# iam28th/fqcomp28

Measured on AMD Instinct MI355X. Metric: encode MB/s (raw FASTQ in), higher is better.
Workload: dtype u8; 1 GPU; BASELINE configs[1]: 1024 MiB synthetic 150 bp reads (uniform ACGT, Phred~N(34,5) clipped [2,41]), -R 256 blocks, tables from the first 128 MiB, inputs resident in HBM; layout=config1, job_blocks=4, blocks_this_gpu=4, records_this_gpu=3202273, bases_this_gpu=480340950

## Files before the change

fqcomp28_amd/binding.py:

```python
import ctypes as C
import os
import subprocess

import numpy as np

HERE = os.path.dirname(os.path.abspath(__file__))
ROOT = os.path.dirname(HERE)
LIB_PATH = os.environ.get("FQGPU_LIB") or os.path.join(HERE, "libfqgpu.so")

SEQ_MODELS, SEQ_ALPHA = 256, 4
QUAL_MODELS, QUAL_ALPHA = 8192, 64
REC_DTYPE = np.dtype([("seq_off", "<u4"), ("qual_off", "<u4"), ("len", "<u4")])
SEQ_FT_DTYPE = np.dtype(
    [("norm", "<i2", (SEQ_MODELS, SEQ_ALPHA)), ("logs", "<u4", (SEQ_MODELS,)), ("max_log", "<u4")]
)
QUAL_FT_DTYPE = np.dtype(
    [("norm", "<i2", (QUAL_MODELS, QUAL_ALPHA)), ("logs", "<u4", (QUAL_MODELS,)), ("max_log", "<u4")]
)
F_WRITE_BACK_N = 1
F_DECODE_INDEX = 2
DEC_FORM_BOTH, DEC_FORM_QUAL_RESIDENT, DEC_FORM_QUAL_COMPACT, DEC_FORM_SEQ = 0x001, 0x002, 0x004, 0x008
DEC_FORM_CHUNKS_QUAL_RESIDENT, DEC_FORM_CHUNKS_QUAL_COMPACT, DEC_FORM_CHUNKS_SEQ, DEC_FORM_SNAP = 0x010, 0x020, 0x040, 0x100

ERRORS = {0: "OK", -1: "OVERFLOW", -2: "SHORT_READ", -3: "CORRUPT", -4: "ARG", -5: "NO_DEVICE",
# ... 16 lines not shown
    return LIB_PATH


def build(verbose=False):
    cmd = ["make", "-C", os.path.join(HERE, "csrc"), "-j", "6"]
    subprocess.run(cmd, check=True, stdout=None if verbose else subprocess.DEVNULL)
    return LIB_PATH


_lib = None

_PROTOS = {
    "fqgpu_device_count": (C.c_int, []),
    "fqgpu_strerror": (C.c_char_p, [C.c_int]),
    "fqgpu_version": (C.c_char_p, []),
    "fqgpu_bound_seq": (C.c_size_t, [C.c_size_t]),
    "fqgpu_bound_qual": (C.c_size_t, [C.c_size_t]),
    "fqgpu_freq_tables": (C.c_int, [C.c_int, C.c_void_p, C.c_size_t, C.c_void_p, C.c_size_t,
                                    C.c_void_p, C.c_void_p, C.c_void_p, C.c_void_p]),
    "fqgpu_tables_from_counts": (C.c_int, [C.c_int, C.c_void_p, C.c_void_p, C.c_void_p, C.c_void_p]),
    "fqgpu_ctx_create": (C.c_int, [C.c_int, C.c_void_p, C.c_void_p, C.POINTER(C.c_void_p)]),
    "fqgpu_ctx_destroy": (None, [C.c_void_p]),
    "fqgpu_ctx_set_chain_params": (C.c_int, [C.c_void_p, C.c_uint, C.c_uint]),
    "fqgpu_ctx_dump_tables": (C.c_int, [C.c_void_p, C.c_int, C.c_uint, C.c_void_p, C.c_size_t,
                                        C.c_void_p, C.c_size_t]),
    "fqgpu_encode_block": (C.c_int, [C.c_void_p, C.c_void_p, C.c_size_t, C.c_void_p, C.c_size_t,
                                     C.c_void_p, C.c_size_t, C.POINTER(C.c_size_t),
                                     C.c_void_p, C.c_size_t, C.POINTER(C.c_size_t),
                                     C.c_void_p, C.c_void_p, C.c_void_p, C.c_size_t,
                                     C.POINTER(C.c_size_t), C.c_uint]),
    "fqgpu_encode_begin": (C.c_int, [C.c_void_p, C.c_void_p, C.c_size_t, C.c_void_p, C.c_size_t, C.c_uint,
                                     C.POINTER(C.c_size_t), C.POINTER(C.c_size_t), C.POINTER(C.c_size_t)]),
    "fqgpu_encode_records": (C.c_int, [C.c_void_p, C.c_void_p, C.c_size_t]),
    "fqgpu_encode_wait": (C.c_int, [C.c_void_p, C.POINTER(C.c_size_t), C.POINTER(C.c_size_t), C.POINTER(C.c_size_t)]),
    "fqgpu_encode_cancel": (C.c_int, [C.c_void_p]),
    "fqgpu_encode_headers_begin": (C.c_int, [C.c_void_p, C.c_void_p, C.c_char_p, C.c_uint, C.c_void_p, C.c_size_t]),
    "fqgpu_encode_headers_wait": (C.c_int, [C.c_void_p, C.c_void_p, C.POINTER(C.c_size_t), C.POINTER(C.c_size_t)]),
    "fqgpu_encode_headers_end": (C.c_int, [C.c_void_p, C.c_void_p, C.c_size_t]),
    "fqgpu_encode_end": (C.c_int, [C.c_void_p, C.c_void_p, C.c_void_p, C.c_size_t, C.POINTER(C.c_size_t),
                                   C.c_void_p, C.c_size_t, C.POINTER(C.c_size_t), C.c_void_p, C.c_void_p, C.c_void_p,
                                   C.c_size_t, C.POINTER(C.c_size_t)]),
    "fqgpu_decode_block": (C.c_int, [C.c_void_p, C.c_void_p, C.c_size_t, C.c_void_p, C.c_size_t,
                                     C.c_void_p, C.c_size_t, C.c_void_p, C.c_size_t, C.c_void_p,
                                     C.c_size_t, C.c_void_p, C.c_size_t]),
    "fqgpu_encode_index": (C.c_int, [C.c_void_p, C.c_int, C.c_void_p, C.c_size_t, C.POINTER(C.c_size_t)]),
    "fqgpu_decode_block_indexed": (C.c_int, [C.c_void_p, C.c_void_p, C.c_size_t, C.c_void_p, C.c_size_t,
                                             C.c_void_p, C.c_size_t, C.c_void_p, C.c_size_t, C.c_void_p,
                                             C.c_size_t, C.c_void_p, C.c_size_t, C.c_void_p, C.c_size_t, C.c_void_p, C.c_size_t]),
    "fqgpu_decode_chunk": (C.c_int, [C.c_void_p, C.c_void_p, C.c_void_p, C.c_size_t, C.c_void_p, C.c_size_t,
                                     C.c_void_p, C.c_size_t, C.c_void_p, C.c_size_t, C.c_void_p, C.c_size_t,
                                     C.c_void_p, C.c_size_t, C.c_void_p, C.c_size_t, C.c_void_p, C.c_size_t,
                                     C.c_void_p, C.POINTER(C.c_size_t), C.POINTER(C.c_size_t)]),
    "fqgpu_decode_chunk_indexing": (C.c_int, [C.c_void_p, C.c_void_p, C.c_void_p, C.c_size_t, C.c_void_p, C.c_size_t,
                                              C.c_void_p, C.c_size_t, C.c_void_p, C.c_size_t, C.c_void_p, C.c_size_t,
                                              C.c_void_p, C.c_size_t, C.c_void_p, C.POINTER(C.c_size_t), C.POINTER(C.c_size_t)]),
    "fqgpu_decode_index": (C.c_int, [C.c_void_p, C.c_int, C.c_void_p, C.c_size_t, C.POINTER(C.c_size_t)]),
    "fqgpu_decode_chunk_range": (C.c_int, [C.c_void_p, C.c_void_p, C.c_void_p, C.c_size_t, C.c_void_p, C.c_size_t,
                                           C.c_void_p, C.c_size_t, C.c_void_p, C.c_size_t, C.c_void_p, C.c_size_t,
                                           C.c_void_p, C.c_size_t, C.c_void_p, C.c_size_t, C.c_size_t, C.c_size_t, C.c_size_t,
                                           C.c_void_p, C.c_size_t, C.POINTER(C.c_size_t), C.c_void_p,
                                           C.POINTER(C.c_size_t)]),
    "fqgpu_decode_chunk_fasta": (C.c_int, [C.c_void_p, C.c_void_p, C.c_void_p, C.c_size_t, C.c_void_p, C.c_size_t,
                                           C.c_void_p, C.c_size_t, C.c_void_p, C.c_size_t, C.c_void_p, C.c_size_t,
                                           C.c_size_t, C.c_size_t, C.c_size_t,
                                           C.c_void_p, C.c_size_t, C.POINTER(C.c_size_t), C.c_void_p,
                                           C.POINTER(C.c_size_t)]),
    "fqgpu_dblock_create": (C.c_int, [C.c_void_p, C.c_void_p, C.c_size_t, C.c_void_p, C.c_size_t,
                                      C.POINTER(C.c_void_p)]),
    "fqgpu_dblock_create_from_raw": (C.c_int, [C.c_void_p, C.c_void_p, C.c_size_t, C.POINTER(C.c_void_p)]),
    "fqgpu_dblock_records": (C.c_int, [C.c_void_p, C.c_void_p, C.c_void_p, C.c_size_t, C.POINTER(C.c_size_t),
                                       C.POINTER(C.c_size_t)]),
    "fqgpu_dblock_destroy": (None, [C.c_void_p]),
    "fqgpu_dblock_encode": (C.c_int, [C.c_void_p, C.c_void_p, C.c_uint]),
    "fqgpu_dblock_wipe": (C.c_int, [C.c_void_p, C.c_void_p]),
    "fqgpu_dblocks_decode": (C.c_int, [C.c_void_p, C.POINTER(C.c_void_p), C.c_size_t]),
    "fqgpu_dblocks_decode_indexing": (C.c_int, [C.c_void_p, C.POINTER(C.c_void_p), C.c_size_t]),
    "fqgpu_sync": (C.c_int, [C.c_void_p]),
    "fqgpu_dblock_status": (C.c_int, [C.c_void_p, C.POINTER(C.c_size_t), C.POINTER(C.c_size_t),
                                      C.POINTER(C.c_size_t), C.POINTER(C.c_size_t)]),
    "fqgpu_dblock_longest_chain": (C.c_int, [C.c_void_p, C.POINTER(C.c_uint), C.POINTER(C.c_uint)]),
    "fqgpu_dblock_qual_segment_classes": (C.c_int, [C.c_void_p, C.c_void_p, C.POINTER(C.c_size_t)]),
    "fqgpu_dblock_qual_segments": (C.c_int, [C.c_void_p, C.c_void_p, C.c_void_p, C.c_void_p, C.c_void_p, C.c_size_t,
                                             C.POINTER(C.c_size_t)]),
    "fqgpu_ctx_set_index_stride": (C.c_int, [C.c_void_p, C.c_uint]),
    "fqgpu_dblock_index_bytes": (C.c_int, [C.c_void_p, C.c_int, C.POINTER(C.c_size_t)]),
    "fqgpu_dblock_fetch_index": (C.c_int, [C.c_void_p, C.c_void_p, C.c_int, C.c_void_p, C.c_size_t]),
    "fqgpu_dblock_load_index": (C.c_int, [C.c_void_p, C.c_void_p, C.c_int, C.c_void_p, C.c_size_t]),
    "fqgpu_ctx_set_lanes": (C.c_int, [C.c_void_p, C.c_uint]),
    "fqgpu_ctx_fill_scratch": (C.c_int, [C.c_void_p, C.c_ubyte, C.POINTER(C.c_size_t), C.POINTER(C.c_size_t)]),
    "fqgpu_ctx_reserve": (C.c_int, [C.c_void_p, C.c_size_t, C.c_size_t, C.c_size_t]),
    "fqgpu_ctx_set_seq_segment": (C.c_int, [C.c_void_p, C.c_uint]),
    "fqgpu_ctx_set_seq_group": (C.c_int, [C.c_void_p, C.c_uint, C.c_uint]),
    "fqgpu_ctx_decode_forms": (C.c_int, [C.c_void_p] + [C.POINTER(C.c_uint)] * 4),
    "fqgpu_ctx_set_seq_handover": (C.c_int, [C.c_void_p, C.c_uint, C.c_uint]),
    "fqgpu_dblock_seq_handover": (C.c_int, [C.c_void_p, C.POINTER(C.c_uint), C.POINTER(C.c_uint)]),
    "fqgpu_dblock_fetch": (C.c_int, [C.c_void_p, C.c_void_p, C.c_void_p, C.c_void_p, C.c_void_p,
                                     C.c_void_p, C.c_void_p, C.c_void_p]),
    "fqgpu_dblock_load_streams": (C.c_int, [C.c_void_p, C.c_void_p, C.c_void_p, C.c_size_t,
                                            C.c_void_p, C.c_size_t, C.c_void_p, C.c_void_p, C.c_size_t]),
    "fqgpu_ctx_enable_timing": (C.c_int, [C.c_void_p, C.c_int]),
    "fqgpu_ctx_last_timing": (C.c_int, [C.c_void_p, C.POINTER(Timing)]),
    "fqgpu_ctx_timing_only": (C.c_int, [C.c_void_p, C.c_char_p]),
    "fqgpu_chunk_crc32": (C.c_int, [C.c_void_p, C.POINTER(C.c_uint32), C.POINTER(C.c_size_t)]),
    "fqgpu_dblock_crc32": (C.c_int, [C.c_void_p, C.c_void_p, C.POINTER(C.c_uint32), C.POINTER(C.c_size_t)]),
    "fqgpu_crc32_combine": (C.c_uint32, [C.c_uint32, C.c_uint32, C.c_uint64]),
    "fqgpu_ctx_set_check_only": (C.c_int, [C.c_void_p, C.c_int]),
    "fqgpu_stats_words": (C.c_size_t, [C.c_uint]),
    "fqgpu_chunk_stats": (C.c_int, [C.c_void_p, C.c_uint, C.c_void_p, C.c_size_t]),
    "fqgpu_dblock_stats": (C.c_int, [C.c_void_p, C.c_void_p, C.c_uint, C.c_void_p, C.c_size_t]),
    "fqgpu_stats_merge": (C.c_int, [C.c_void_p, C.c_size_t, C.c_void_p, C.c_size_t]),
    "fqgpu_filter_check": (C.c_int, [C.c_void_p]),
    "fqgpu_chunk_filter": (C.c_int, [C.c_void_p, C.c_void_p, C.c_void_p, C.c_size_t, C.POINTER(C.c_size_t), C.c_void_p, C.c_void_p]),
    "fqgpu_dblock_filter": (C.c_int, [C.c_void_p, C.c_void_p, C.c_void_p, C.c_void_p, C.c_size_t, C.POINTER(C.c_size_t),
                                      C.c_void_p, C.c_void_p]),
    "fqgpu_trim_check": (C.c_int, [C.c_void_p]),
    "fqgpu_chunk_trim": (C.c_int, [C.c_void_p, C.c_void_p, C.c_void_p, C.c_void_p, C.c_size_t, C.POINTER(C.c_size_t), C.c_void_p,
                                   C.c_void_p, C.c_void_p]),
    "fqgpu_dblock_trim": (C.c_int, [C.c_void_p, C.c_void_p, C.c_void_p, C.c_void_p, C.c_void_p, C.c_size_t, C.POINTER(C.c_size_t),
                                    C.c_void_p, C.c_void_p, C.c_void_p]),
    "fqgpu_adapter_check": (C.c_int, [C.c_void_p]),
    "fqgpu_chunk_clip": (C.c_int, [C.c_void_p, C.c_void_p, C.c_void_p, C.c_void_p, C.c_void_p, C.c_size_t, C.POINTER(C.c_size_t),
                                   C.c_void_p, C.c_void_p, C.c_void_p]),
    "fqgpu_dblock_clip": (C.c_int, [C.c_void_p, C.c_void_p, C.c_void_p, C.c_void_p, C.c_void_p, C.c_void_p, C.c_size_t,
                                    C.POINTER(C.c_size_t), C.c_void_p, C.c_void_p, C.c_void_p]),
    "fqgpu_tail_check": (C.c_int, [C.c_void_p]),
    "fqgpu_chunk_tailtrim": (C.c_int, [C.c_void_p, C.c_void_p, C.c_void_p, C.c_void_p, C.c_void_p, C.c_void_p, C.c_size_t,
                                       C.POINTER(C.c_size_t), C.c_void_p, C.c_void_p, C.c_void_p, C.c_void_p]),
    "fqgpu_dblock_tailtrim": (C.c_int, [C.c_void_p, C.c_void_p, C.c_void_p, C.c_void_p, C.c_void_p, C.c_void_p, C.c_void_p, C.c_size_t,
                                        C.POINTER(C.c_size_t), C.c_void_p, C.c_void_p, C.c_void_p, C.c_void_p]),
    "fqgpu_chunk_select_marked": (C.c_int, [C.c_void_p, C.c_void_p, C.c_void_p, C.c_void_p, C.c_void_p, C.c_size_t, C.c_size_t, C.c_void_p,
                                            C.c_void_p, C.c_size_t, C.POINTER(C.c_size_t), C.c_void_p, C.c_void_p, C.c_void_p, C.c_void_p]),
    "fqgpu_dblock_select_marked": (C.c_int, [C.c_void_p, C.c_void_p, C.c_void_p, C.c_void_p, C.c_void_p, C.c_void_p, C.c_size_t, C.c_size_t,
                                             C.c_void_p, C.c_void_p, C.c_size_t, C.POINTER(C.c_size_t), C.c_void_p, C.c_void_p, C.c_void_p,
                                             C.c_void_p]),
    "fqgpu_chunk_select_limited": (C.c_int, [C.c_void_p, C.c_void_p, C.c_void_p, C.c_void_p, C.c_void_p, C.c_size_t, C.c_size_t, C.c_void_p, C.c_void_p,
                                             C.c_void_p, C.c_size_t, C.POINTER(C.c_size_t), C.c_void_p, C.c_void_p, C.c_void_p, C.c_void_p]),
    "fqgpu_dblock_select_limited": (C.c_int, [C.c_void_p, C.c_void_p, C.c_void_p, C.c_void_p, C.c_void_p, C.c_void_p, C.c_size_t, C.c_size_t,
                                              C.c_void_p, C.c_void_p, C.c_void_p, C.c_size_t, C.POINTER(C.c_size_t), C.c_void_p, C.c_void_p,
                                              C.c_void_p, C.c_void_p]),
    "fqgpu_overlap_check": (C.c_int, [C.c_void_p]),
    "fqgpu_overlap_merge": (C.c_int, [C.c_void_p, C.c_size_t, C.c_void_p, C.c_size_t]),
    "fqgpu_chunk_pair_overlap": (C.c_int, [C.c_void_p, C.c_size_t, C.c_void_p, C.c_size_t, C.c_size_t, C.c_void_p, C.c_void_p, C.c_size_t,
                                           C.c_void_p, C.c_void_p, C.c_void_p]),
    "fqgpu_dblock_pair_overlap": (C.c_int, [C.c_void_p, C.c_void_p, C.c_size_t, C.c_void_p, C.c_size_t, C.c_size_t, C.c_void_p, C.c_void_p,
                                            C.c_size_t, C.c_void_p, C.c_void_p, C.c_void_p]),
    "fqgpu_correct_check": (C.c_int, [C.c_void_p]),
    "fqgpu_chunk_pair_correct": (C.c_int, [C.c_void_p, C.c_size_t, C.c_void_p, C.c_size_t, C.c_size_t, C.c_void_p, C.c_void_p, C.c_void_p,
                                           C.c_void_p, C.c_void_p]),
    "fqgpu_dblock_pair_correct": (C.c_int, [C.c_void_p, C.c_void_p, C.c_size_t, C.c_void_p, C.c_size_t, C.c_size_t, C.c_void_p, C.c_void_p,
                                            C.c_void_p, C.c_void_p, C.c_void_p]),
    "fqgpu_merge_check": (C.c_int, [C.c_void_p]),
    "fqgpu_chunk_pair_merge": (C.c_int, [C.c_void_p, C.c_size_t, C.c_void_p, C.c_size_t, C.c_size_t, C.c_void_p, C.c_void_p, C.c_void_p,
                                         C.c_void_p, C.c_size_t, C.c_void_p, C.c_void_p, C.c_void_p]),
    "fqgpu_dblock_pair_merge": (C.c_int, [C.c_void_p, C.c_void_p, C.c_size_t, C.c_void_p, C.c_size_t, C.c_size_t, C.c_void_p, C.c_void_p,
                                          C.c_void_p, C.c_void_p, C.c_size_t, C.c_void_p, C.c_void_p, C.c_void_p]),
    "fqgpu_chunk_pair_names": (C.c_int, [C.c_void_p, C.c_size_t, C.c_void_p, C.c_size_t, C.c_size_t, C.POINTER(C.c_size_t)]),
    "fqgpu_dblock_pair_names": (C.c_int, [C.c_void_p, C.c_void_p, C.c_size_t, C.c_void_p, C.c_size_t, C.c_size_t, C.POINTER(C.c_size_t)]),
    "fqgpu_read_id_len": (C.c_size_t, [C.c_void_p, C.c_size_t]),
    "fqgpu_probe_words": (C.c_size_t, [C.c_uint, C.c_uint]),
    "fqgpu_probes_check": (C.c_int, [C.c_void_p]),
    "fqgpu_chunk_probe": (C.c_int, [C.c_void_p, C.c_void_p, C.c_uint, C.c_void_p, C.c_size_t, C.c_void_p]),
    "fqgpu_dblock_probe": (C.c_int, [C.c_void_p, C.c_void_p, C.c_void_p, C.c_uint, C.c_void_p, C.c_size_t, C.c_void_p]),
    "fqgpu_probe_merge": (C.c_int, [C.c_void_p, C.c_size_t, C.c_void_p, C.c_size_t]),
    "fqgpu_host_alloc": (C.c_void_p, [C.c_size_t]),
    "fqgpu_host_free": (None, [C.c_void_p]),
    "fqgpu_host_trim": (C.c_size_t, []),
# ... 462 lines not shown
    def wipe(self):
        _check(lib().fqgpu_dblock_wipe(self.ctx.h, self.h), "dblock_wipe")

    def crc32(self, want_len=False):
        crc, n = C.c_uint32(0), C.c_size_t(0)
        _check(lib().fqgpu_dblock_crc32(self.ctx.h, self.h, C.byref(crc), C.byref(n)), "dblock_crc32")
        return (crc.value, n.value) if want_len else crc.value

    def stats(self, positions):
        rc, out = _stats_call(lib().fqgpu_dblock_stats, positions, self.ctx.h, self.h)
        _check(rc, "dblock_stats")
        return out

    def probe(self, probes, positions, want_places=True, **kw):
        return _probe_call(lib().fqgpu_dblock_probe, (self.ctx.h, self.h), probes, positions, self.n_recs, want_places, **kw)

    def filter(self, flt, **kw):
        return _select_call(lib().fqgpu_dblock_filter, (self.ctx.h, self.h), (flt,), self.n_recs, **kw)

    def trim(self, trim, flt=None, **kw):
        return _select_call(lib().fqgpu_dblock_trim, (self.ctx.h, self.h), (trim, flt), self.n_recs, more=("win",), **kw)

    def clip(self, adapter, trim=None, flt=None, **kw):
        return _select_call(lib().fqgpu_dblock_clip, (self.ctx.h, self.h), (adapter, trim, flt), self.n_recs, more=("win",), **kw)

    def tailtrim(self, adapter=None, tail=None, trim=None, flt=None, **kw):
        return _select_call(lib().fqgpu_dblock_tailtrim, (self.ctx.h, self.h), (adapter, tail, trim, flt), self.n_recs, more=("win", "places"),
                            report_words=TAIL_REPORT_WORDS, **kw)

    def select_marked(self, first, end, mark=None, adapter=None, tail=None, trim=None, flt=None, **kw):
        return _range_call(lib().fqgpu_dblock_select_marked, (self.ctx.h, self.h), (adapter, tail, trim, flt), first, end, mark, **kw)

    def select_limited(self, first, end, mark=None, limit=None, adapter=None, tail=None, trim=None, flt=None, **kw):
        return _range_call(lib().fqgpu_dblock_select_limited, (self.ctx.h, self.h), (adapter, tail, trim, flt), first, end, mark, limit, **kw)

    def pair_correct(self, first, other, other_first, count, insert, spec, **kw):
        return _correct_call(lib().fqgpu_dblock_pair_correct, (self.ctx.h, self.h, first, other.h if other is not None else None, other_first),
                             count, insert, spec, **kw)

    def pair_merge(self, first, other, other_first, count, insert, mark, spec, **kw):
        return _merge_call(lib().fqgpu_dblock_pair_merge, (self.ctx.h, self.h, first, other.h if other is not None else None, other_first),
                           count, insert, mark, spec, **kw)

    def pair_overlap(self, first, other, other_first, count, spec, **kw):
        return _overlap_call(lib().fqgpu_dblock_pair_overlap, (self.ctx.h, self.h, first, other.h if other is not None else None, other_first),
                             count, spec, **kw)

    def pair_names(self, first, other, other_first, count):
        m = C.c_size_t(7)
        rc = lib().fqgpu_dblock_pair_names(self.ctx.h, self.h, first, other.h if other is not None else None, other_first, count, C.byref(m))
        return rc, None if m.value == NO_MISMATCH else m.value

    def status(self):
        a, b, c, d = C.c_size_t(), C.c_size_t(), C.c_size_t(), C.c_size_t()
        rc = lib().fqgpu_dblock_status(self.h, C.byref(a), C.byref(b), C.byref(c), C.byref(d))
        return rc, dict(seq_len=a.value, qual_len=b.value, n_pos_len=c.value, n_bases=d.value)

    def longest_chain(self):
        a, b = C.c_uint(), C.c_uint()
        _check(lib().fqgpu_dblock_longest_chain(self.h, C.byref(a), C.byref(b)), "dblock_longest_chain")
        return a.value, b.value

    def seq_handover(self):
        a, b = C.c_uint(), C.c_uint()
        _check(lib().fqgpu_dblock_seq_handover(self.h, C.byref(a), C.byref(b)), "dblock_seq_handover")
        return a.value, b.value

    def qual_segment_classes(self):
        c = (C.c_size_t * 4)()
        _check(lib().fqgpu_dblock_qual_segment_classes(self.ctx.h, self.h, c), "dblock_qual_segment_classes")
        return dict(transparent=c[0], anchored=c[1], uniform=c[2], opaque=c[3])

    def qual_segments(self):
        n = C.c_size_t(0)
        rc = lib().fqgpu_dblock_qual_segments(self.ctx.h, self.h, None, None, None, 0, C.byref(n))
        if rc != -1:
            _check(rc, "dblock_qual_segments")
        cls, anchor, ctx = np.zeros(n.value, dtype=np.uint8), np.zeros(n.value, dtype=np.uint32), np.zeros(n.value, dtype=np.uint32)
        if n.value:
            _check(lib().fqgpu_dblock_qual_segments(self.ctx.h, self.h, _p(cls), _p(anchor), _p(ctx), n.value, C.byref(n)),
                   "dblock_qual_segments")
        return dict(cls=cls, anchor=anchor, ctx=ctx)

    def fetch(self, raw=False):
        rc, st = self.status()
        _check(rc, "dblock_status")
        seq = np.zeros(st["seq_len"], dtype=np.uint8)
        qual = np.zeros(st["qual_len"], dtype=np.uint8)
        rl = np.zeros(self.n_recs, dtype=np.uint16)
        nc = np.zeros(self.n_recs, dtype=np.uint16)
        npos = np.zeros(st["n_pos_len"], dtype=np.uint16)
        rw = np.zeros(self.raw_len, dtype=np.uint8) if raw else None
        _check(lib().fqgpu_dblock_fetch(self.ctx.h, self.h, _p(seq), _p(qual), _p(rl), _p(nc), _p(npos),
                                        _p(rw)), "dblock_fetch")
        return dict(seq=seq, qual=qual, readlens=rl, n_count=nc, n_pos=npos, raw=rw)

    def fetch_raw(self):
        rw = np.zeros(self.raw_len, dtype=np.uint8)
        _check(lib().fqgpu_dblock_fetch(self.ctx.h, self.h, None, None, None, None, None, _p(rw)),
               "dblock_fetch")
        return rw

    def load_streams(self, seq, qual, n_count, n_pos):
        seq = np.ascontiguousarray(seq, dtype=np.uint8)
        qual = np.ascontiguousarray(qual, dtype=np.uint8)
        n_count = np.ascontiguousarray(n_count, dtype=np.uint16)
        n_pos = np.ascontiguousarray(n_pos, dtype=np.uint16)
        _check(lib().fqgpu_dblock_load_streams(self.ctx.h, self.h, _p(seq), seq.size, _p(qual), qual.size,
                                               _p(n_count), _p(n_pos), n_pos.size), "load_streams")


class _HeaderStreams(C.Structure):
    _fields_ = [("field_types", C.c_void_p), ("separators", C.c_char_p), ("n_fields", C.c_uint),
                ("first_header", C.c_void_p), ("first_header_len", C.c_size_t), ("sizes", C.c_void_p),
                ("streams", C.POINTER(C.c_void_p))]


class Context:

    def __init__(self, seq_ft, qual_ft, device=0):
        self.seq_ft = np.ascontiguousarray(seq_ft)
        self.qual_ft = np.ascontiguousarray(qual_ft)
        assert self.seq_ft.nbytes == SEQ_FT_DTYPE.itemsize and self.qual_ft.nbytes == QUAL_FT_DTYPE.itemsize
        h = C.c_void_p()
        _check(lib().fqgpu_ctx_create(device, _p(self.seq_ft), _p(self.qual_ft), C.byref(h)), "ctx_create")
        self.h = h
        self.device = device

    def close(self):
        if getattr(self, "h", None):
            lib().fqgpu_ctx_destroy(self.h)
            self.h = None

    __del__ = close

    def set_chain_params(self, segment=0, seq_generic=False, seq_segment=None, seq_group=None):
        flags = 1 if seq_generic else 0
        if seq_segment is not None:
            _check(lib().fqgpu_ctx_set_seq_segment(self.h, seq_segment), "set_seq_segment")
        if seq_group is not None:
            q, g = seq_group if isinstance(seq_group, tuple) else (seq_group, 0)
            _check(lib().fqgpu_ctx_set_seq_group(self.h, q, g), "set_seq_group")
        _check(lib().fqgpu_ctx_set_chain_params(self.h, segment, flags), "set_chain_params")

    def set_seq_handover(self, cap, prefix_segments=1):
        _check(lib().fqgpu_ctx_set_seq_handover(self.h, cap, prefix_segments), "set_seq_handover")

    def set_index_stride(self, symbols):
        _check(lib().fqgpu_ctx_set_index_stride(self.h, symbols), "set_index_stride")

    def set_lanes(self, lanes):
        _check(lib().fqgpu_ctx_set_lanes(self.h, lanes), "set_lanes")

    def sync(self):
        _check(lib().fqgpu_sync(self.h), "sync")

    def fill_scratch(self, byte):
        n, nb = C.c_size_t(0), C.c_size_t(0)
        _check(lib().fqgpu_ctx_fill_scratch(self.h, byte, C.byref(n), C.byref(nb)), "fill_scratch")
        return n.value, nb.value

    def decode_forms(self):
        f, c, s, n = C.c_uint(0), C.c_uint(0), C.c_uint(0), C.c_uint(0)
        _check(lib().fqgpu_ctx_decode_forms(self.h, C.byref(f), C.byref(c), C.byref(s), C.byref(n)), "decode_forms")
        return dict(forms=f.value, qual_chains=c.value, qual_strides=s.value, n_cus=n.value)

# ... 268 lines not shown
```

fqcomp28_amd/csrc/api.hip:

```cpp
#include "fqgpu_internal.h"

#include <algorithm>
#include <cstdio>
#include <cstdlib>
#include <cstring>
#include <initializer_list>
#include <new>
#include <string>
#include <map>
#include <memory>
#include <mutex>
#include <vector>

__attribute__((constructor)) static void fq_ask_for_hw_queues() {
  if (getenv("FQGPU_KEEP_HW_QUEUES")) return;
  if (const char *have = getenv("GPU_MAX_HW_QUEUES")) {
    char *end = nullptr;
    const long n = strtol(have, &end, 10);
    if (end == have || *end != 0 || n < 1 || n >= 16) return;
  }
  setenv("GPU_MAX_HW_QUEUES", "16", 1);
}

static thread_local char g_hip_msg[256] = "";

int fq_hip_error(hipError_t e, const char *file, int line) {
  snprintf(g_hip_msg, sizeof(g_hip_msg), "HIP error %d (%s) at %s:%d", (int)e, hipGetErrorString(e), file, line);
  if (getenv("FQGPU_VERBOSE")) fprintf(stderr, "fqgpu: %s\n", g_hip_msg);
  return (e == hipErrorOutOfMemory) ? FQGPU_E_NOMEM
         : (e == hipErrorNoDevice || e == hipErrorInvalidDevice) ? FQGPU_E_NO_DEVICE
                                                                 : FQGPU_E_HIP;
}

extern "C" const char *fqgpu_strerror(int code) {
  switch (code) {
  case FQGPU_OK: return "ok";
  case FQGPU_E_OVERFLOW: return "compressed stream exceeds the reference capacity bound";
  case FQGPU_E_SHORT_READ: return "read shorter than 3 bases (undefined in the reference coder)";
  case FQGPU_E_CORRUPT: return "corrupt stream (end mark / leftover bits / N table)";
  case FQGPU_E_ARG: return "bad argument or symbol outside the model alphabet";
  case FQGPU_E_NO_DEVICE: return "no usable MI355X / HIP device (there is no CPU fallback)";
  case FQGPU_E_NOMEM: return "out of device or host memory";
  case FQGPU_E_HIP: return g_hip_msg[0] ? g_hip_msg : "HIP runtime error";
  case FQGPU_E_HEADER: return "read header the field coder cannot code (numeric field not an int32 / string field of 255 or more bytes)";
  default: return "unknown fqgpu error";
  }
}

extern "C" const char *fqgpu_version(void) { return "fqgpu 0.1 (gfx950)"; }

extern "C" int fqgpu_device_count(void) {
  int n = 0;
  if (hipGetDeviceCount(&n) != hipSuccess) return 0;
  return n;
}

extern "C" size_t fqgpu_bound_seq(size_t n) {
  if (n < 1024) return (size_t)1024 * FQGPU_SEQ_MODELS;
  return n / 4 + 1024;
}
extern "C" size_t fqgpu_bound_qual(size_t n) {
  const size_t a = (size_t)1024 * FQGPU_QUAL_MODELS, b = n * 7 / 8 + 1024;
  return a > b ? a : b;
}

static int use_device(int device) {
  int n = 0;
  if (hipGetDeviceCount(&n) != hipSuccess || n <= 0) return FQGPU_E_NO_DEVICE;
  if (device < 0 || device >= n) return FQGPU_E_NO_DEVICE;
  FQ_HIP(hipSetDevice(device));
  return FQGPU_OK;
}

namespace {
struct HostHdr { uint64_t magic, pinned, size, pad[5]; };
constexpr uint64_t HOST_MAGIC = 0x46514850494E4E44ull;
constexpr size_t PIN_MIN = 64 << 10;
struct PinCache {
  std::mutex mutex;
  std::multimap<size_t, void *> blocks;
  size_t bytes = 0;
};
PinCache &pin_cache() {
// ... 262 lines not shown
  return l;
}

static int normalize_to_host(hipStream_t st, const uint32_t *counts_dev, int stream, void *ft_out) {
  const FtLayout l = ft_layout(stream);
  uint8_t *dev = fq_dev_alloc<uint8_t>(l.total + 8);
  if (!dev) return FQGPU_E_NOMEM;
  int rc = FQGPU_OK;
  uint32_t err = 0;
  do {
    if (hipMemsetAsync(dev, 0, l.total + 8, st) != hipSuccess) { rc = FQGPU_E_HIP; break; }
    uint32_t *err_dev = reinterpret_cast<uint32_t *>(dev + ((l.total + 3) & ~(size_t)3));
    rc = fq_normalize_counts(st, counts_dev, l.n_models, l.alpha, reinterpret_cast<int16_t *>(dev),
                             reinterpret_cast<uint32_t *>(dev + l.logs_off),
                             reinterpret_cast<uint32_t *>(dev + l.maxlog_off), err_dev);
    if (rc) break;
    if (hipMemcpyAsync(ft_out, dev, l.total, hipMemcpyDeviceToHost, st) != hipSuccess ||
        hipMemcpyAsync(&err, err_dev, 4, hipMemcpyDeviceToHost, st) != hipSuccess ||
        hipStreamSynchronize(st) != hipSuccess) { rc = FQGPU_E_HIP; break; }
    if (err) rc = FQGPU_E_ARG;
  } while (0);
  (void)hipFree(dev);
  return rc;
}

extern "C" int fqgpu_tables_from_counts(int device, const uint32_t *seq_counts, const uint32_t *qual_counts,
                                        void *seq_ft_out, void *qual_ft_out) {
  int rc = use_device(device);
  if (rc) return rc;
  if (!seq_counts || !qual_counts || !seq_ft_out || !qual_ft_out) return FQGPU_E_ARG;
  const size_t ns = (size_t)FQGPU_SEQ_MODELS * FQGPU_SEQ_ALPHA, nq = (size_t)FQGPU_QUAL_MODELS * FQGPU_QUAL_ALPHA;
  uint32_t *dev = fq_dev_alloc<uint32_t>(ns + nq);
  if (!dev) return FQGPU_E_NOMEM;
  hipStream_t st = nullptr;
  if (hipMemcpy(dev, seq_counts, ns * 4, hipMemcpyHostToDevice) != hipSuccess ||
      hipMemcpy(dev + ns, qual_counts, nq * 4, hipMemcpyHostToDevice) != hipSuccess) rc = FQGPU_E_HIP;
  if (!rc) rc = normalize_to_host(st, dev, 0, seq_ft_out);
  if (!rc) rc = normalize_to_host(st, dev + ns, 1, qual_ft_out);
  (void)hipFree(dev);
  return rc;
}

extern "C" int fqgpu_freq_tables(int device, const uint8_t *raw, size_t raw_len, const fqgpu_rec *recs,
                                 size_t n_recs, void *seq_ft_out, void *qual_ft_out,
                                 uint32_t *seq_counts_out, uint32_t *qual_counts_out) {
  int rc = use_device(device);
  if (rc) return rc;
  if (!raw || !recs || !seq_ft_out || !qual_ft_out) return FQGPU_E_ARG;
  size_t n_bases = 0;
  unsigned min_len = 0xFFFFFFFFu;
  for (size_t i = 0; i < n_recs; i++) {
    if ((size_t)recs[i].seq_off + recs[i].len > raw_len || (size_t)recs[i].qual_off + recs[i].len > raw_len)
      return FQGPU_E_ARG;
    n_bases += recs[i].len;
    if (recs[i].len < min_len || recs[i].len > 65535u) min_len = recs[i].len > 65535u ? 0u : recs[i].len;
  }
  const size_t ns = (size_t)FQGPU_SEQ_MODELS * FQGPU_SEQ_ALPHA, nq = (size_t)FQGPU_QUAL_MODELS * FQGPU_QUAL_ALPHA;
  uint8_t *raw_dev = fq_dev_alloc<uint8_t>(raw_len + 64);
  fqgpu_rec *recs_dev = fq_dev_alloc<fqgpu_rec>(n_recs + 1);
  uint32_t *cnt = fq_dev_alloc<uint32_t>(ns + nq + 1);
  hipStream_t st = nullptr;
  uint32_t err = 0;
  if (!raw_dev || !recs_dev || !cnt) rc = FQGPU_E_NOMEM;
  do {
    if (rc) break;
    if (hipMemcpy(raw_dev, raw, raw_len, hipMemcpyHostToDevice) != hipSuccess ||
        hipMemcpy(recs_dev, recs, n_recs * sizeof(fqgpu_rec), hipMemcpyHostToDevice) != hipSuccess ||
        hipMemset(cnt + ns + nq, 0, 4) != hipSuccess) { rc = FQGPU_E_HIP; break; }
    if ((rc = fq_build_freq_tables(device, st, raw_dev, recs_dev, n_recs, cnt, cnt + ns, n_bases, min_len))) break;
    if (hipMemcpy(&err, cnt + ns + nq, 4, hipMemcpyDeviceToHost) != hipSuccess) { rc = FQGPU_E_HIP; break; }
    if (err) { rc = FQGPU_E_ARG; break; }
    if (seq_counts_out && hipMemcpy(seq_counts_out, cnt, ns * 4, hipMemcpyDeviceToHost) != hipSuccess) { rc = FQGPU_E_HIP; break; }
    if (qual_counts_out && hipMemcpy(qual_counts_out, cnt + ns, nq * 4, hipMemcpyDeviceToHost) != hipSuccess) { rc = FQGPU_E_HIP; break; }
    if ((rc = normalize_to_host(st, cnt, 0, seq_ft_out))) break;
    if ((rc = normalize_to_host(st, cnt + ns, 1, qual_ft_out))) break;
  } while (0);
  if (raw_dev) (void)hipFree(raw_dev);
  if (recs_dev) (void)hipFree(recs_dev);
  if (cnt) (void)hipFree(cnt);
  return rc;
}

static void free_tables(DevTables &t) {
  void *ps[] = {t.norm, t.logs, t.log_prefix, t.ct, t.ct_off, t.dt, t.dt_off, t.next1, t.next2, t.reset_mask,
                t.seq_pow[0], t.seq_pow[1], t.seq_pow[2], t.seq_pow[3]};
  for (void *p : ps) if (p) (void)hipFree(p);
  t = DevTables();
}

static int upload_tables(fqgpu_ctx *ctx, int stream, const void *ft) {
  const FtLayout l = ft_layout(stream);
  DevTables &t = ctx->tab[stream];
  const uint8_t *p = static_cast<const uint8_t *>(ft);
  const uint32_t *logs = reinterpret_cast<const uint32_t *>(p + l.logs_off);
  const int16_t *norm = reinterpret_cast<const int16_t *>(p);
  uint32_t max_log = 0;
  for (int i = 0; i < l.n_models; i++) {
    if (logs[i] < 5 || logs[i] > 12) return FQGPU_E_ARG;
    if (logs[i] > max_log) max_log = logs[i];
    uint32_t sum = 0;
    for (int s = 0; s < l.alpha; s++) {
      const int n = norm[(size_t)i * l.alpha + s];
      if (n < -1) return FQGPU_E_ARG;
      sum += n == -1 ? 1u : (uint32_t)n;
    }
    if (sum != (1u << logs[i])) return FQGPU_E_ARG;
  }
  t.max_log = max_log;
  t.norm = fq_dev_alloc<int16_t>((size_t)l.n_models * l.alpha);
  t.logs = fq_dev_alloc<uint32_t>(l.n_models);
  uint32_t *err_dev = fq_dev_alloc<uint32_t>(1);
  if (!t.norm || !t.logs || !err_dev) return FQGPU_E_NOMEM;
  FQ_HIP(hipMemcpyAsync(t.norm, p, l.norm_bytes, hipMemcpyHostToDevice, ctx->stream));
  FQ_HIP(hipMemcpyAsync(t.logs, logs, (size_t)l.n_models * 4, hipMemcpyHostToDevice, ctx->stream));
  FQ_HIP(hipMemsetAsync(err_dev, 0, 4, ctx->stream));
  int rc = fq_build_tables(ctx->stream, t, l.n_models, l.alpha, err_dev);
  uint32_t err = 0;
  if (!rc) {
    FQ_HIP(hipMemcpyAsync(&err, err_dev, 4, hipMemcpyDeviceToHost, ctx->stream));
    FQ_HIP(hipStreamSynchronize(ctx->stream));
    if (err) rc = FQGPU_E_ARG;
  }
  (void)hipFree(err_dev);
  return rc;
}

extern "C" int fqgpu_ctx_create(int device, const void *seq_ft, const void *qual_ft, fqgpu_ctx **out) {
  if (!out) return FQGPU_E_ARG;
  *out = nullptr;
  int rc = use_device(device);
  if (rc) return rc;
  if (!seq_ft || !qual_ft) return FQGPU_E_ARG;
  fqgpu_ctx *ctx = new (std::nothrow) fqgpu_ctx();
  if (!ctx) return FQGPU_E_NOMEM;
  ctx->device = device;
  {
    int cus = 0;
    if (hipDeviceGetAttribute(&cus, hipDeviceAttributeMultiprocessorCount, device) == hipSuccess && cus > 0) ctx->n_cus = (unsigned)cus;
  }
  if (hipStreamCreateWithFlags(&ctx->stream, hipStreamNonBlocking) != hipSuccess) {
    delete ctx;
    return FQGPU_E_HIP;
  }
  rc = fq_probe_lds_atomic_order(ctx->stream, &ctx->lds_atomics_ordered);
  if (!rc) rc = fq_encode_init_device();
  if (getenv("FQGPU_NO_LDS_ATOMIC_RANK")) ctx->lds_atomics_ordered = false;
  if (getenv("FQGPU_SLOT_PARTITION")) ctx->tile_sorted = false;
  if (const char *e = getenv("FQGPU_SETFUNC_WGS")) ctx->setfunc_wgs = (unsigned)atoi(e);
  if (const char *e = getenv("FQGPU_SEQ_GROUP")) ctx->seq_group = (unsigned)atoi(e);
  if (const char *e = getenv("FQGPU_SEQ_GROUP_MIN")) ctx->seq_group_min = (unsigned)atoi(e);
  if (const char *e = getenv("FQGPU_SEQ_CAND_CAP")) ctx->seq_cand_cap = std::min((unsigned)atoi(e), 64u);
  if (const char *e = getenv("FQGPU_SEQ_CAND_PREFIX")) ctx->seq_cand_prefix = std::max((unsigned)atoi(e), 1u);
  if (!rc) rc = upload_tables(ctx, 0, seq_ft);
  if (!rc) rc = upload_tables(ctx, 1, qual_ft);
  if (rc) { fqgpu_ctx_destroy(ctx); return rc; }
  *out = ctx;
  return FQGPU_OK;
}

#ifdef FQGPU_EXPERIMENTS
void fq_ts_prof_dump();
#endif

extern "C" void fqgpu_ctx_destroy(fqgpu_ctx *ctx) {
  if (!ctx) return;
  (void)hipSetDevice(ctx->device);
  (void)fqgpu_sync(ctx);
// ... 293 lines not shown
  return rc;
}

extern "C" int fqgpu_dblock_longest_chain(const fqgpu_dblock *b, unsigned *seq_segments, unsigned *qual_segments) {
  if (!b) return FQGPU_E_ARG;
  (void)hipSetDevice(b->device);
  BlockResult tmp;
  FQ_HIP(hipMemcpy(&tmp, b->result, sizeof(tmp), hipMemcpyDeviceToHost));
  if (seq_segments) *seq_segments = tmp.s[0].refixed;
  if (qual_segments) *qual_segments = tmp.s[1].refixed;
  return FQGPU_OK;
}

extern "C" int fqgpu_dblock_seq_handover(const fqgpu_dblock *b, unsigned *handed_over, unsigned *kept) {
  if (!b) return FQGPU_E_ARG;
  (void)hipSetDevice(b->device);
  if (b->last_op && !b->result_pulled && b->owner) {
    const int rc = fqgpu_sync(b->owner);
    if (rc) return rc;
  }
  BlockResult tmp;
  FQ_HIP(hipMemcpy(&tmp, b->result, sizeof(tmp), hipMemcpyDeviceToHost));
  if (handed_over) *handed_over = tmp.seq_groups_handed;
  if (kept) *kept = tmp.seq_groups_kept;
  return FQGPU_OK;
}

extern "C" int fqgpu_ctx_decode_forms(const fqgpu_ctx *ctx, unsigned *forms, unsigned *qual_chains, unsigned *qual_strides, unsigned *n_cus) {
  if (!ctx) return FQGPU_E_ARG;
  if (forms) *forms = ctx->dec_forms;
  if (qual_chains) *qual_chains = ctx->dec_qual_chains;
  if (qual_strides) *qual_strides = ctx->dec_qual_strides;
  if (n_cus) *n_cus = ctx->n_cus;
  return FQGPU_OK;
}

static int diag_lane(fqgpu_ctx *ctx, const fqgpu_dblock *b, const EncLane **lane_out, uint32_t *n_out) {
  if (int rc = fqgpu_sync(ctx)) return rc;
  if (b->owner != ctx || !b->diag_stamp || b->home_lane < 0 || b->home_lane >= FQ_MAX_LANES) return FQGPU_E_ARG;
  const EncLane &lane = ctx->lanes[b->home_lane];
  if (lane.diag_stamp != b->diag_stamp || !lane.diag_cls || !lane.diag_anchor || !lane.diag_n_segs) return FQGPU_E_ARG;
  FQ_HIP(hipMemcpy(n_out, lane.diag_n_segs, 4, hipMemcpyDeviceToHost));
  *lane_out = &lane;
  return FQGPU_OK;
}

extern "C" int fqgpu_dblock_qual_segment_classes(fqgpu_ctx *ctx, const fqgpu_dblock *b, size_t counts[4]) {
  if (!ctx || !b || !counts) return FQGPU_E_ARG;
  counts[0] = counts[1] = counts[2] = counts[3] = 0;
  const EncLane *lane = nullptr;
  uint32_t n = 0;
  if (int rc = diag_lane(ctx, b, &lane, &n)) return rc;
  if (!n) return FQGPU_OK;
  uint8_t *cls = static_cast<uint8_t *>(malloc(n));
  if (!cls) return FQGPU_E_NOMEM;
  const hipError_t he = hipMemcpy(cls, lane->diag_cls, n, hipMemcpyDeviceToHost);
  if (he == hipSuccess)
    for (uint32_t i = 0; i < n; i++) counts[cls[i] == 1 ? 0 : cls[i] == 0xFF ? 2 : cls[i] == 0 ? 3 : 1]++;
  free(cls);
  return he == hipSuccess ? FQGPU_OK : fq_hip_error(he, __FILE__, __LINE__);
}

extern "C" int fqgpu_dblock_qual_segments(fqgpu_ctx *ctx, const fqgpu_dblock *b, uint8_t *cls_out, uint32_t *anchor_out,
                                          uint32_t *ctx_out, size_t cap, size_t *n_out) {
  if (!ctx || !b || !n_out || (cap && (!cls_out || !anchor_out || !ctx_out))) return FQGPU_E_ARG;
  *n_out = 0;
  const EncLane *lane = nullptr;
  uint32_t n = 0;
  if (int rc = diag_lane(ctx, b, &lane, &n)) return rc;
  *n_out = n;
  if (n > cap) return FQGPU_E_OVERFLOW;
  if (!n) return FQGPU_OK;
  constexpr unsigned B = FQGPU_QUAL_MODELS;
  uint32_t *seg_base = static_cast<uint32_t *>(malloc((size_t)(B + 1) * 4));
  if (!seg_base) return FQGPU_E_NOMEM;
  hipError_t he = hipMemcpy(seg_base, lane->diag_n_segs - B, (size_t)(B + 1) * 4, hipMemcpyDeviceToHost);
  if (he == hipSuccess) he = hipMemcpy(cls_out, lane->diag_cls, n, hipMemcpyDeviceToHost);
  if (he == hipSuccess) he = hipMemcpy(anchor_out, lane->diag_anchor, (size_t)n * 4, hipMemcpyDeviceToHost);
  if (he == hipSuccess)
    for (unsigned c = 0; c < B; c++)
      for (uint32_t s = seg_base[c]; s < seg_base[c + 1] && s < n; s++) ctx_out[s] = c;
  free(seg_base);
  return he == hipSuccess ? FQGPU_OK : fq_hip_error(he, __FILE__, __LINE__);
}

extern "C" int fqgpu_dblock_fetch(fqgpu_ctx *ctx, const fqgpu_dblock *b, uint8_t *seq_out, uint8_t *qual_out,
                                  uint16_t *readlens_out, uint16_t *n_count_out, uint16_t *n_pos_out,
                                  uint8_t *raw_out) {
  if (!ctx || !b) return FQGPU_E_ARG;
  int rc = fqgpu_sync(ctx);
  if (rc) return rc;
  if (b->last_op && !b->result_pulled && (rc = pull_result(const_cast<fqgpu_dblock *>(b), b->last_op == 1))) return rc;
  if (seq_out && b->seq_len) FQ_HIP(hipMemcpy(seq_out, b->seq, b->seq_len, hipMemcpyDeviceToHost));
  if (qual_out && b->qual_len) FQ_HIP(hipMemcpy(qual_out, b->qual, b->qual_len, hipMemcpyDeviceToHost));
  if (readlens_out) FQ_HIP(hipMemcpy(readlens_out, b->readlens, b->n_recs * 2, hipMemcpyDeviceToHost));
  if (n_count_out) FQ_HIP(hipMemcpy(n_count_out, b->n_count, b->n_recs * 2, hipMemcpyDeviceToHost));
  if (n_pos_out && b->n_pos_len) FQ_HIP(hipMemcpy(n_pos_out, b->n_pos, b->n_pos_len * 2, hipMemcpyDeviceToHost));
  if (raw_out) FQ_HIP(hipMemcpy(raw_out, b->raw, b->raw_len, hipMemcpyDeviceToHost));
  return FQGPU_OK;
}

extern "C" int fqgpu_dblock_load_streams(fqgpu_ctx *ctx, fqgpu_dblock *b, const uint8_t *seq, size_t seq_len,
                                         const uint8_t *qual, size_t qual_len, const uint16_t *n_count,
                                         const uint16_t *n_pos, size_t n_pos_len) {
  if (!ctx || !b || !seq || !qual || !n_count || (!n_pos && n_pos_len)) return FQGPU_E_ARG;
  int rc = fqgpu_sync(ctx);
  if (rc) return rc;
  if (b->seq.grow(seq_len + 64) || b->qual.grow(qual_len + 64) || b->n_pos.grow(n_pos_len + 16)) return FQGPU_E_NOMEM;
  if (n_pos_len > b->n_pos_cap) b->n_pos_cap = n_pos_len;
  FQ_HIP(hipMemset(b->seq + seq_len, 0, 16));
  FQ_HIP(hipMemset(b->qual + qual_len, 0, 16));
  FQ_HIP(hipMemcpy(b->seq, seq, seq_len, hipMemcpyHostToDevice));
  FQ_HIP(hipMemcpy(b->qual, qual, qual_len, hipMemcpyHostToDevice));
  FQ_HIP(hipMemcpy(b->n_count, n_count, b->n_recs * 2, hipMemcpyHostToDevice));
  if (n_pos_len) FQ_HIP(hipMemcpy(b->n_pos, n_pos, n_pos_len * 2, hipMemcpyHostToDevice));
  b->seq_len = seq_len; b->qual_len = qual_len; b->n_pos_len = n_pos_len;
  b->drop_results();
  return FQGPU_OK;
}

static int dblocks_decode(fqgpu_ctx *ctx, fqgpu_dblock *const *blocks, size_t n_blocks, bool build_index) {
  if (!ctx || (!blocks && n_blocks)) return FQGPU_E_ARG;
  int rc = use_device(ctx->device);
  if (rc) return rc;
  for (size_t i = 0; i < n_blocks; i++)
    if (!blocks[i] || blocks[i]->device != ctx->device) return FQGPU_E_ARG;
  bool synced = false;
  for (size_t i = 0; i < n_blocks; i++) {
    fqgpu_dblock *b = blocks[i];
    if (b->last_op == 1 && !b->result_pulled) {
      if (!synced && (rc = fqgpu_sync(ctx))) return rc;
      synced = true;
      if ((rc = pull_result(b, true))) return rc;
    }
    if (!b->seq_len || !b->qual_len) return FQGPU_E_ARG;
  }
  for (size_t i = 0; i < n_blocks; i++) blocks[i]->launched(2);
  return fq_decode_launch(ctx, blocks, n_blocks, nullptr, build_index);
}

extern "C" int fqgpu_dblocks_decode(fqgpu_ctx *ctx, fqgpu_dblock *const *blocks, size_t n_blocks) {
  return dblocks_decode(ctx, blocks, n_blocks, false);
}

extern "C" int fqgpu_dblocks_decode_indexing(fqgpu_ctx *ctx, fqgpu_dblock *const *blocks, size_t n_blocks) {
  int rc = dblocks_decode(ctx, blocks, n_blocks, true);
  if (rc) {
    for (size_t i = 0; blocks && i < n_blocks; i++)
      if (blocks[i]) blocks[i]->index_bytes[0] = blocks[i]->index_bytes[1] = 0;
    return rc;
  }
  if ((rc = fqgpu_sync(ctx))) return rc;
  for (size_t i = 0; i < n_blocks; i++) {
    const int brc = pull_result(blocks[i], false);
    if (brc) blocks[i]->index_bytes[0] = blocks[i]->index_bytes[1] = 0;
    if (brc && brc != FQGPU_E_CORRUPT && brc != FQGPU_E_ARG) return brc;
  }
  return FQGPU_OK;
}

template <class A> static bool hp_room(A &a, size_t need) { return a.grow(need, need / 8) == FQGPU_OK; }

static int hp_block_acquire(fqgpu_ctx *ctx, size_t raw_len, size_t n_recs, size_t n_bases, size_t seq_cap,
                            size_t qual_cap, size_t n_pos_cap, fqgpu_dblock **out) {
  if (!ctx->hp.block && !(ctx->hp.block = dblock_new(ctx).release())) return FQGPU_E_NOMEM;
  fqgpu_dblock *b = ctx->hp.block;
// ... 885 lines not shown
```

fqcomp28_amd/csrc/enc_chains_generic.h:

```cpp

constexpr unsigned SEG_NONE = 0xFFFFFFFFu;
constexpr unsigned SEG_CLS_OPAQUE = 0, SEG_CLS_UNIFORM = 0xFF;

struct SegArrays {
  uint32_t *anchor;
  uint32_t *usym;
  uint16_t *entry_state;
  uint16_t *cand_exit;
  uint8_t *cls;
};

template <class M>
__device__ __forceinline__ unsigned seg_ctx_of(const uint32_t *__restrict__ base, unsigned v) {
  unsigned lo = 0, hi = M::B - 1;
  while (lo < hi) {
    const unsigned mid = lo + ((hi - lo + 1) >> 1);
    if (base[mid] <= v) lo = mid; else hi = mid - 1;
  }
  return lo;
}

template <class M>
__global__ void __launch_bounds__(256)
k_seg_scan(const uint8_t *__restrict__ sorted_sym, const uint32_t *__restrict__ arrays,
// ... 78 lines not shown
__device__ __forceinline__ bool seg_wants_setfunc(const SegArrays &sa, unsigned seg, unsigned k, unsigned nseg) {
  if (k + 1 >= nseg) return false;
  const unsigned cls = sa.cls[seg];
  return cls == SEG_CLS_OPAQUE || (seg_is_cand(cls) && !seg_entry_known(k, k ? (unsigned)sa.cls[seg - 1] : 1u));
}

template <class M, unsigned PER0>
__device__ __forceinline__ void seg_pow_table(uint32_t *lds, const uint32_t *__restrict__ tbl, unsigned s, unsigned S,
                                              uint16_t *__restrict__ f) {
  const unsigned log = tbl[0] & 0xFFFFu, size = 1u << log, lane = fq_lane(), per = max(size >> 6, 1u);
  const uint16_t *st = reinterpret_cast<const uint16_t *>(tbl) + 2;
  const uint32_t *tt = tbl + 1 + (size >> 1);
  const int dfs = (int)tt[2 * s];
  const unsigned dnb = tt[2 * s + 1];
  uint16_t *base = reinterpret_cast<uint16_t *>(lds);
  unsigned acc[PER0], tmp[PER0];
#pragma unroll
  for (unsigned j = 0; j < PER0; j++) {
    const unsigned i = (lane + 64u * j) & (size - 1);
    acc[j] = i;
    if (j < per) {
      const unsigned x = size + i, nb = (x + dnb) >> 16;
      base[i] = (uint16_t)(st[(int)(x >> nb) + dfs] - size);
    }
  }
  fq_lds_wave_sync();
  for (unsigned e = S; e; e >>= 1) {
    if (e & 1u) {
#pragma unroll
      for (unsigned j = 0; j < PER0; j++)
        if (j < per) acc[j] = base[acc[j]];
    }
    if (e > 1u) {
#pragma unroll
      for (unsigned j = 0; j < PER0; j++)
        if (j < per) tmp[j] = base[base[(lane + 64u * j) & (size - 1)]];
      fq_lds_wave_sync();
#pragma unroll
      for (unsigned j = 0; j < PER0; j++)
        if (j < per) base[(lane + 64u * j) & (size - 1)] = (uint16_t)tmp[j];
      fq_lds_wave_sync();
    }
  }
#pragma unroll
  for (unsigned j = 0; j < PER0; j++) {
    const unsigned i = lane + 64u * j;
    if (j < per && i < size) f[i] = (uint16_t)(size + acc[j]);
  }
}

template <class M>
__device__ __forceinline__ unsigned seg_walk_range(const LdsCTable &t, const uint8_t *__restrict__ sym,
                                                   uint16_t *__restrict__ out, unsigned i, unsigned end, unsigned x) {
  while (i < end && (i & 15u)) {
    out[i] = (uint16_t)chain_step(t, x, sym[i] & (unsigned)(M::A - 1));
    i++;
  }
  if (i + 16 <= end) {
    const uint4 *sym16 = reinterpret_cast<const uint4 *>(sym);
    uint4 *out16v = reinterpret_cast<uint4 *>(out);
    uint4 cur = sym16[i >> 4];
    while (i + 16 <= end) {
      const uint4 nxt = i + 32 <= end ? sym16[(i >> 4) + 1] : cur;
      const unsigned w[4] = {cur.x, cur.y, cur.z, cur.w};
      unsigned o[8];
#pragma unroll
      for (int j = 0; j < 16; j++) {
        const unsigned v = chain_step(t, x, (w[j >> 2] >> (8 * (j & 3))) & (unsigned)(M::A - 1));
        if (j & 1) o[j >> 1] |= v << 16; else o[j >> 1] = v;
      }
      out16v[i >> 3] = make_uint4(o[0], o[1], o[2], o[3]);
      out16v[(i >> 3) + 1] = make_uint4(o[4], o[5], o[6], o[7]);
      i += 16;
      cur = nxt;
    }
  }
  while (i < end) {
    out[i] = (uint16_t)chain_step(t, x, sym[i] & (unsigned)(M::A - 1));
    i++;
  }
  return x;
}

template <class M, int PASS>
__device__ __forceinline__ void seg_walk_role(uint32_t *lds, unsigned item, const uint8_t *__restrict__ sorted_sym,
                                              uint16_t *__restrict__ out16, const uint32_t *__restrict__ arrays,
                                              const uint32_t *__restrict__ ct, const uint32_t *__restrict__ ct_off,
                                              uint16_t *__restrict__ final_state, unsigned S, const SegArrays &sa, StreamResult *res) {
  constexpr unsigned B = M::B;
  const uint32_t *ctx_count = arrays, *ctx_start = arrays + B, *seg_base = ctx_start + B + 1,
                 *item_base = seg_base + B + 1;
  if (item >= item_base[B]) return;
  const unsigned c = seg_ctx_of<M>(item_base, item);
  const unsigned n = ctx_count[c];
  const unsigned nseg = seg_base[c + 1] - seg_base[c];
  const unsigned k = (item - item_base[c]) * 64 + fq_lane();
  const LdsCTable t = stage_ctable<M>(lds, ct + ct_off[c]);
  if (k >= nseg) return;
  const unsigned seg = seg_base[c] + k;
  const uint8_t *sym = sorted_sym + ctx_start[c];
  uint16_t *out = out16 + ctx_start[c];
  const unsigned begin = k * S, end = min(n, begin + S);
  const bool reset = sa.cls[seg] == 1;
  const unsigned fr = sa.anchor[seg];
  unsigned x, i0, i1;
  if (PASS == 1) {
    if (!reset) return;
    i0 = begin + fr + 1; i1 = end;
    x = reset_state(t, sym[begin + fr] & (unsigned)(M::A - 1));
  } else {
    i0 = begin; i1 = reset ? begin + fr + 1 : end;
    x = sa.entry_state[seg];
  }
  x = seg_walk_range<M>(t, sym, out, i0, i1, x);
  if (PASS == 1 && k + 1 < nseg) sa.entry_state[seg + 1] = (uint16_t)x;
  if (k == nseg - 1 && (PASS == 1 || !reset)) final_state[c] = (uint16_t)x;
  if (PASS == 2 && fq_lane() == 0) atomicMax(&res->refixed, min(S, n));
}

template <class M, int PASS>
__global__ void __launch_bounds__(64)
k_seg_walk(const uint8_t *__restrict__ sorted_sym, uint16_t *__restrict__ out16,
           const uint32_t *__restrict__ arrays, const uint32_t *__restrict__ ct,
           const uint32_t *__restrict__ ct_off, uint16_t *__restrict__ final_state, unsigned S,
           SegArrays sa, StreamResult *res) {
  extern __shared__ uint32_t lds[];
  seg_walk_role<M, PASS>(lds, blockIdx.x, sorted_sym, out16, arrays, ct, ct_off, final_state, S, sa, res);
}

template <class M>
__device__ __forceinline__ unsigned seg_state_range(const LdsCTable &t, const uint8_t *__restrict__ sym, unsigned i,
                                                    unsigned end, unsigned x) {
  auto step = [&](unsigned s) {
    const int dfs = (int)t.tt[2 * s];
    const unsigned nb = (x + t.tt[2 * s + 1]) >> 16;
    x = t.state_table[(int)(x >> nb) + dfs];
  };
  while (i < end && (i & 15u)) { step(sym[i] & (unsigned)(M::A - 1)); i++; }
  if (i + 16 <= end) {
    const uint4 *sym16 = reinterpret_cast<const uint4 *>(sym);
    uint4 cur = sym16[i >> 4];
    while (i + 16 <= end) {
      const uint4 nxt = i + 32 <= end ? sym16[(i >> 4) + 1] : cur;
      const unsigned w[4] = {cur.x, cur.y, cur.z, cur.w};
#pragma unroll
      for (int j = 0; j < 16; j++) step((w[j >> 2] >> (8 * (j & 3))) & (unsigned)(M::A - 1));
      i += 16;
      cur = nxt;
    }
  }
  while (i < end) { step(sym[i] & (unsigned)(M::A - 1)); i++; }
  return x;
}

template <class M, bool HEADS>
__device__ __forceinline__ void seg_cand_role(uint32_t *lds, unsigned w_first, unsigned w_step, const uint8_t *__restrict__ sorted_sym,
                                              const uint32_t *__restrict__ arrays, const uint32_t *__restrict__ ct,
                                              const uint32_t *__restrict__ ct_off, unsigned S, unsigned fstride, const SegArrays &sa,
                                              uint16_t *__restrict__ fbuf) {
  constexpr unsigned B = M::B, PER = 64 / SEG_SLOT;
  const uint32_t *ctx_count = arrays, *ctx_start = arrays + B, *seg_base = ctx_start + B + 1;
  const unsigned n_segs = seg_base[B];
  const unsigned lane = fq_lane(), slot = lane / SEG_SLOT, j = lane % SEG_SLOT;
  for (unsigned w = w_first; w * PER < n_segs; w += w_step) {
    const unsigned seg = w * PER + slot;
    unsigned cls = 0, c = 0, k = 0, pred = 1;
    bool want = false;
    if (seg < n_segs) {
      cls = sa.cls[seg];
      if (seg_is_cand(cls)) {
        c = seg_ctx_of<M>(seg_base, seg);
        k = seg - seg_base[c];
        pred = k ? (unsigned)sa.cls[seg - 1] : 1u;
        want = k + 1 < seg_base[c + 1] - seg_base[c] && (!HEADS || seg_entry_known(k, pred));
      }
    }
    unsigned long long todo = __ballot(want);
    while (todo) {
      const unsigned cc = (unsigned)__shfl((int)c, __ffsll((long long)todo) - 1);
      const bool mine = want && c == cc;
      todo &= ~__ballot(mine);
      fq_lds_wave_sync();
      const LdsCTable t = stage_ctable<M>(lds, ct + ct_off[cc]);
      if (!mine) continue;
      const unsigned size = 1u << t.log;
      const unsigned n = ctx_count[c], begin = k * S, end = min(n, begin + S);
      const uint8_t *sym = sorted_sym + ctx_start[c];
      const unsigned r = begin + sa.anchor[seg];
      const unsigned s = sym[r] & (unsigned)(M::A - 1);
      const int dfs = (int)t.tt[2 * s];
      const unsigned n_cand = HEADS ? pred : cls;
      for (unsigned cand = j; cand < n_cand; cand += SEG_SLOT) {
        if (!HEADS) {
          unsigned x = t.state_table[dfs + (int)cls + (int)cand];
          x = seg_state_range<M>(t, sym, r + 1, end, x);
          sa.cand_exit[(size_t)seg * SEG_MAX_CAND + cand] = (uint16_t)x;
        } else {
          const unsigned entry = pred == 1 ? (unsigned)sa.entry_state[seg] : (unsigned)sa.cand_exit[(size_t)(seg - 1) * SEG_MAX_CAND + cand];
          const unsigned x = seg_state_range<M>(t, sym, begin, r, entry);
          const unsigned nb = (x + t.tt[2 * s + 1]) >> 16;
          const unsigned u = (x >> nb) - cls;
          fbuf[(size_t)seg * fstride + (entry - size)] = sa.cand_exit[(size_t)seg * SEG_MAX_CAND + u];
        }
      }
    }
  }
}

template <class M>
__global__ void __launch_bounds__(64)
// ... 61 lines not shown
  const LdsCTable t = stage_ctable<M>(lds, ct + ct_off[c]);
  const unsigned log = t.log, size = 1u << log, lane = fq_lane();
  const unsigned per = max(size >> 6, 1u), nw = max(size >> 5, 1u);
  const uint4 *gseg = reinterpret_cast<const uint4 *>(sorted_sym + ctx_start[c] + (size_t)k * S);
  const unsigned nblk = S / SETS_BLOCK, w_end = S / 4;

  unsigned x0[PER0];
#pragma unroll
  for (unsigned j = 0; j < PER0; j++) x0[j] = size + ((lane + 64u * j) & (size - 1));
  unsigned level = 0, n = size, n1 = 0;
  unsigned w = 0, stop = 1;
  uint4 cur = gseg[lane];
  for (unsigned blk = 0; blk < nblk; blk++) {
    const uint4 nxt = blk + 1 < nblk ? gseg[(size_t)(blk + 1) * 64 + lane] : cur;
    const unsigned wb_end = (blk + 1) * (SETS_BLOCK / 4);
    while (w < wb_end) {
      const unsigned w1 = min(stop, wb_end);
      if (level == 0) {
        for (; w < w1; w++) {
          const unsigned word = sets_word(cur, w);
#pragma unroll
          for (int i = 0; i < 4; i++) {
            const unsigned s = (word >> (8 * i)) & (unsigned)(M::A - 1);
            const int dfs = (int)t.tt[2 * s];
            const unsigned dnb = t.tt[2 * s + 1];
#pragma unroll
            for (unsigned j = 0; j < PER0; j++)
              if (j < per) { const unsigned nb = (x0[j] + dnb) >> 16; x0[j] = t.state_table[(int)(x0[j] >> nb) + dfs]; }
          }
        }
      } else {
        switch ((n + 63) / 64) {
          case 1: seg_sets_walk<M, 1>(L, n, t, cur, w, w1); break;
          case 2: seg_sets_walk<M, 2>(L, n, t, cur, w, w1); break;
          case 3: seg_sets_walk<M, 3>(L, n, t, cur, w, w1); break;
          case 4: seg_sets_walk<M, 4>(L, n, t, cur, w, w1); break;
          case 5: seg_sets_walk<M, 5>(L, n, t, cur, w, w1); break;
          case 6: seg_sets_walk<M, 6>(L, n, t, cur, w, w1); break;
          case 7: seg_sets_walk<M, 7>(L, n, t, cur, w, w1); break;
          default: seg_sets_walk<M, 8>(L, n, t, cur, w, w1); break;
        }
        w = w1;
      }
      if (w != stop || w >= w_end) continue;
      stop = stop == 1 ? 4 : stop == 4 ? 12 : stop == 12 ? 32 : stop * 4;
      if (level == 0) {
        sets_clear(L);
#pragma unroll
        for (unsigned j = 0; j < PER0; j++)
          if (j < per) { const unsigned xi = x0[j] - size; atomicOr(&L.bm[xi >> 5], 1u << (xi & 31u)); }
        fq_lds_wave_sync();
        const unsigned nn = sets_count(L, nw);
        if (nn <= SETS_MAX_CLASSES) {
#pragma unroll
          for (unsigned j = 0; j < PER0; j++)
            if (j < per) {
              const unsigned r = sets_rank(L, x0[j] - size);
              L.list[r] = (uint16_t)x0[j];
              x0[j] = r;
            }
          for (unsigned i = lane; i < nn; i += 64) L.m[i] = (uint16_t)i;
          fq_lds_wave_sync();
          level = 1; n = n1 = nn;
        }
      } else if (n > 64) {
        n = sets_merge<false>(L, n, n1, nw, size);
      }
    }
    cur = nxt;
  }
  uint16_t *f = fbuf + (size_t)seg * fstride;
#pragma unroll
  for (unsigned j = 0; j < PER0; j++) {
    const unsigned xi = lane + 64u * j;
    if (j < per && xi < size) f[xi] = level == 0 ? (uint16_t)x0[j] : L.list[L.m[x0[j]]];
  }
}

template <class M, unsigned PER0>
__global__ void __launch_bounds__(64)
k_seg_stage1(const uint8_t *__restrict__ sorted_sym, uint16_t *__restrict__ out16, const uint32_t *__restrict__ arrays,
             const uint32_t *__restrict__ ct, const uint32_t *__restrict__ ct_off, uint16_t *__restrict__ final_state,
             unsigned S, unsigned n_walk, unsigned n_cand, unsigned pbase, unsigned fstride, SegArrays sa,
             uint16_t *__restrict__ fbuf, StreamResult *res) {
  extern __shared__ uint32_t lds[];
  __shared__ SetsWaveLds L;
  if (blockIdx.x < n_walk)
    seg_walk_role<M, 1>(lds, blockIdx.x, sorted_sym, out16, arrays, ct, ct_off, final_state, S, sa, res);
  else if (blockIdx.x < n_walk + n_cand)
    seg_cand_role<M, false>(lds, blockIdx.x - n_walk, n_cand, sorted_sym, arrays, ct, ct_off, S, fstride, sa, fbuf);
  else
    seg_setfunc_role<M, PER0>(lds, L, blockIdx.x - n_walk - n_cand, sorted_sym, arrays, ct, ct_off, S, pbase, fstride, sa, fbuf);
}

struct ItemArrays {
  uint16_t *g;
  uint32_t *has_g;
  uint16_t *item_entry;
};

template <class M, unsigned PER0>
__global__ void __launch_bounds__(64)
k_seg_compose(const uint32_t *__restrict__ arrays, const uint32_t *__restrict__ logs,
              const uint16_t *__restrict__ fbuf, unsigned pbase, unsigned fstride, SegArrays sa, ItemArrays ia) {
  constexpr unsigned B = M::B;
  const uint32_t *seg_base = arrays + B + (B + 1), *item_base = seg_base + B + 1;
  const unsigned item = blockIdx.x, lane = fq_lane();
  if (item >= item_base[B]) return;
  const unsigned c = seg_ctx_of<M>(item_base, item);
  const unsigned nseg = seg_base[c + 1] - seg_base[c];
  const unsigned k0 = (item - item_base[c]) * 64, n_here = min(64u, nseg - k0);
  const unsigned seg0 = seg_base[c] + k0;
  const unsigned slot = lane < n_here ? seg_fslot(sa, seg0 + lane, k0 + lane, nseg, c, pbase) : SEG_NONE;
  const unsigned long long opaque = __ballot(slot != SEG_NONE);
  if (lane == 0) ia.has_g[item] = opaque != 0ull;
  if (!opaque) return;
  const unsigned exit_state = lane < n_here && slot == SEG_NONE && k0 + lane + 1 < nseg ? sa.entry_state[seg0 + lane + 1] : 0u;
  const unsigned size = 1u << logs[c], per = max(size >> 6, 1u);
  unsigned x[PER0];
#pragma unroll
  for (unsigned j = 0; j < PER0; j++) x[j] = size + ((lane + 64u * j) & (size - 1));
  for (unsigned t = 0; t < n_here; t++) {
    const unsigned sl = (unsigned)__shfl((int)slot, (int)t);
    if (sl == SEG_NONE) {
      if (k0 + t + 1 >= nseg) break;
      const unsigned e = (unsigned)__shfl((int)exit_state, (int)t);
#pragma unroll
      for (unsigned j = 0; j < PER0; j++) x[j] = e;
    } else {
      const uint16_t *f = fbuf + (size_t)sl * fstride;
#pragma unroll
      for (unsigned j = 0; j < PER0; j++)
        if (j < per) x[j] = size | ((unsigned)f[x[j] - size] & (size - 1));
    }
  }
  uint16_t *g = ia.g + (size_t)item * fstride;
#pragma unroll
  for (unsigned j = 0; j < PER0; j++) {
    const unsigned xi = lane + 64u * j;
    if (j < per && xi < size) g[xi] = (uint16_t)x[j];
  }
}

template <class M>
__global__ void __launch_bounds__(256)
k_seg_resolve2(const uint32_t *__restrict__ arrays, const uint32_t *__restrict__ logs, unsigned fstride,
               SegArrays sa, ItemArrays ia) {
  constexpr unsigned B = M::B;
  const unsigned c = blockIdx.x * blockDim.x + threadIdx.x;
  if (c >= B) return;
  const uint32_t *seg_base = arrays + B + (B + 1), *item_base = seg_base + B + 1;
  const unsigned i0 = item_base[c], ni = item_base[c + 1] - i0;
  const unsigned size = 1u << logs[c];
  unsigned x = size;
  for (unsigned i = 0; i < ni; i++) {
    ia.item_entry[i0 + i] = (uint16_t)x;
    if (i + 1 == ni) break;
    x = ia.has_g[i0 + i] ? ia.g[(size_t)(i0 + i) * fstride + (x - size)]
                         : sa.entry_state[seg_base[c] + (i + 1) * 64];
  }
}

template <class M>
__global__ void __launch_bounds__(256)
k_seg_resolve3(const uint32_t *__restrict__ arrays, const uint32_t *__restrict__ logs,
               const uint16_t *__restrict__ fbuf, unsigned pbase, unsigned fstride, SegArrays sa, ItemArrays ia) {
  constexpr unsigned B = M::B;
  const uint32_t *seg_base = arrays + B + (B + 1), *item_base = seg_base + B + 1;
  const unsigned item = blockIdx.x * blockDim.x + threadIdx.x;
  if (item >= item_base[B] || !ia.has_g[item]) return;
  const unsigned c = seg_ctx_of<M>(item_base, item);
// ... 14 lines not shown
```

fqcomp28_amd/csrc/enc_plan.h:

```cpp
#pragma once

#include <stddef.h>
#include <stdint.h>

#include <algorithm>

#include "../../include/fqgpu.h"

constexpr unsigned TILE_SEQ = 32768;
constexpr unsigned TILE_QUAL = 65536;
constexpr unsigned TS_TILE = 32768;
constexpr unsigned GROUP_TILES = 64;
constexpr unsigned PACK_TILE = 4096;
constexpr unsigned CTX_PAD = 16;
constexpr unsigned SC_BATCH_SEQ = 8192;
constexpr unsigned SETS_WAVES = 8;
constexpr unsigned SETS_WAVES2 = 16;
constexpr unsigned SETS_ROUNDS = 4;
constexpr unsigned SETS_MAX_GROUP = 16;
constexpr unsigned SETS_BLOCK = 1024;
constexpr unsigned SEQ_CAND_MAX = 64;
constexpr unsigned SEGPLAN_WORDS = 5 * (FQGPU_SEQ_MODELS + 1) + 4;
constexpr unsigned SEQ_ITEM_GROUPS = 64;
constexpr unsigned SEG_MAX_CAND = 64;
constexpr unsigned SEG_SLOT = 16;

struct EncSpan {
  size_t off = 0, bytes = 0;
};
struct EncCarve {
  size_t total = 0;
  EncSpan take(size_t bytes, size_t align = 1) {
    EncSpan s;
    s.off = (total + align - 1) & ~(align - 1);
    s.bytes = bytes;
    total = s.off + bytes;
    return s;
  }
};

struct EncBytes {
  size_t slot_of = 0;
  size_t keys = 0;
  size_t sorted_sym = 0;
  size_t out16 = 0;
  size_t tile_hist = 0;
  size_t tile_base = 0;
  size_t group_sum = 0;
  size_t ctx_arrays = 0;
  size_t seg_state = 0;
  size_t seg_arrays = 0;
  size_t seq_plan = 0;
  size_t seq_fbuf = 0;
  size_t seq_cbuf = 0;
  size_t seq_cand = 0;
  size_t seq_bdesc = 0;
  size_t tile_bits = 0;
  size_t tile_bit_base = 0;
  size_t tile_runs = 0;
  size_t tile_sync = 0;
};

struct EncShape {
  unsigned n_sym = 0, R = 0, B = 0, T = 0;
  unsigned n_tiles = 0, n_groups = 0, n_ptiles = 0;
  size_t n_pad = 0;
  size_t padded = 0;
  size_t lpos16_bytes = 0, tile_runs_bytes = 0;
  EncBytes bytes;
  EncSpan ckey, csym;
  EncSpan ctx_count, ctx_start, seg_base;

  EncShape() = default;
  EncShape(unsigned n_sym_, unsigned R_, unsigned B_, unsigned T_) : n_sym(n_sym_), R(R_), B(B_), T(T_) {
    n_tiles = (n_sym + T - 1) / T;
    n_groups = (n_tiles + GROUP_TILES - 1) / GROUP_TILES;
    n_ptiles = (n_sym + PACK_TILE - 1) / PACK_TILE;
    n_pad = ((size_t)n_sym + SC_BATCH_SEQ + 15) & ~(size_t)15;
    padded = (size_t)n_sym + (size_t)CTX_PAD * B + 64;
    lpos16_bytes = n_pad * 2;
    tile_runs_bytes = (size_t)n_tiles * std::min(B, TS_TILE) * 8;
    EncCarve k, a;
    ckey = k.take(n_pad * 2);
    csym = k.take(n_pad);
    bytes.keys = k.total;
    bytes.sorted_sym = padded;
    bytes.tile_hist = bytes.tile_base = (size_t)n_tiles * B * 4;
    bytes.group_sum = (size_t)n_groups * B * 4;
    ctx_count = a.take((size_t)B * 4);
    ctx_start = a.take((size_t)(B + 1) * 4);
    seg_base = a.take((size_t)(B + 1) * 4);
    a.take((size_t)(B + 1) * 4);
    bytes.ctx_arrays = a.total;
  }
};

struct EncPlanIn {
  unsigned n_sym = 0, R = 0;
  int stream = 0;
  unsigned B = 0, A = 0, max_log = 0;
  bool two_sym = false;
  bool tile_path = false, serial_seq = false;
  unsigned seg_len = 0, seq_segment = 0, seq_group = 0, seq_group_min = 0, seq_cand_cap = 0, seq_cand_prefix = 0, n_cus = 0;
};

struct EncPlan : EncShape {
  bool tile_path = false, serial_seq = false, two_sym = false;
  unsigned max_log = 0;
  unsigned S = 0;
  unsigned seq_S = 0;
  unsigned max_items = 0, gen_max_segs = 0, seq_max_segs = 0;
  unsigned fstride = 0;
  unsigned next_stride = 0;
  unsigned gen_pbase = 0;
  unsigned cand_grid = 0;
  unsigned cand_cap = 0, cand_W = 0, cand_P = 0;
  unsigned wpg = 0, Q = 0, gmin = 0, rounds = 0;
  unsigned max_fitems = 0, max_eitems = 0, max_citems = 0;
  unsigned lds_ct = 0;

  EncSpan sa_anchor, sa_usym, sa_entry, sa_cand, sa_cls;
  EncSpan ia_has_g, ia_entry, ia_g;
  EncSpan sp_fitem, sp_seg, sp_work, sp_entry;
  EncSpan cb_func, cb_item_entry;
  EncSpan cand0, cand;
  EncSpan bd_start, bd_pre;
  EncSpan ts_status, ts_counter, ts_run_count, ts_edges;

  EncPlan() = default;
  explicit EncPlan(const EncPlanIn &in)
      : EncShape(in.n_sym, in.R, in.B, in.tile_path ? TS_TILE : in.stream == 0 ? TILE_SEQ : TILE_QUAL),
        tile_path(in.tile_path), serial_seq(in.serial_seq), two_sym(in.two_sym), max_log(in.max_log) {
    const auto whole_blocks = [](unsigned s) { return (unsigned)std::min(((size_t)s + SETS_BLOCK - 1) / SETS_BLOCK * SETS_BLOCK, (size_t)1 << 30); };
    S = whole_blocks(in.seg_len ? in.seg_len : n_sym >= (24u << 20) ? 4096u : n_sym >= (4u << 20) ? 2048u : 1024u);
    seq_S = whole_blocks(in.seq_segment ? in.seq_segment : n_sym >= (48u << 20) ? 4096u : n_sym >= (4u << 20) ? 2048u : 1024u);
    max_items = (unsigned)((size_t)n_sym / ((size_t)S * 64) + B + 1);
    gen_max_segs = n_sym / S + B + 1;
    seq_max_segs = n_sym / seq_S + B + 1;
    fstride = 1u << max_log;
    next_stride = 4u << max_log;
    gen_pbase = gen_max_segs;
    cand_grid = std::min(gen_max_segs / (64 / SEG_SLOT) + 1, 32u * in.n_cus);
    cand_cap = serial_seq && two_sym ? std::min(in.seq_cand_cap, SEQ_CAND_MAX) : 0u;
    cand_W = cand_cap == 0 ? 0u : cand_cap <= 16 ? 16u : cand_cap <= 32 ? 32u : 64u;
    cand_P = std::min(std::max(in.seq_cand_prefix, 1u), SETS_MAX_GROUP);
    wpg = two_sym ? SETS_WAVES2 : SETS_WAVES;
    Q = std::min(std::max(in.seq_group, 1u), SETS_MAX_GROUP);
    gmin = std::max(in.seq_group_min, 1u);
    rounds = std::max(SETS_ROUNDS / Q, 1u);
    max_fitems = seq_max_segs / (wpg * rounds) + B + 1;
    max_eitems = seq_max_segs / 64 + B + 1;
    max_citems = seq_max_segs / SEQ_ITEM_GROUPS + B + 1;
    lds_ct = (1u + (1u << (max_log - 1)) + 2u * in.A) * 4u;

    bytes.slot_of = tile_path ? lpos16_bytes : n_pad * 4;
    bytes.out16 = padded * 2;
    bytes.seg_state = (size_t)B * 2 + (size_t)B * 8;
    bytes.tile_bits = (size_t)n_ptiles * 4;
    bytes.tile_bit_base = (size_t)(n_ptiles + 1) * 8;

    const size_t gs = gen_max_segs;
    EncCarve g;
    sa_anchor = g.take(gs * 4, 16);
    sa_usym = g.take((size_t)B * 4, 16);
    sa_entry = g.take(gs * 2, 16);
    sa_cand = g.take(gs * SEG_MAX_CAND * 2, 16);
    sa_cls = g.take(gs, 16);
    ia_has_g = g.take((size_t)max_items * 4, 16);
    ia_entry = g.take((size_t)max_items * 2, 16);
    ia_g = g.take((size_t)max_items * fstride * 2, 16);
    g.take(64);
    EncCarve sp, cb, cd, bd, ts;
    const size_t base_bytes = (size_t)(FQGPU_SEQ_MODELS + 1) * 4;
    sp_fitem = sp.take(2 * base_bytes);
    sp_seg = sp.take(3 * base_bytes);
    sp_work = sp.take(16);
    sp_entry = sp.take((size_t)seq_max_segs * 2);
    sp.take(64);
    cb_func = cb.take((size_t)max_citems * fstride * 2);
    cb_item_entry = cb.take((size_t)max_citems * 2);
    cb.take(64);
    cand0 = cd.take((size_t)seq_max_segs * cand_W * 2);
    cand = cd.take((size_t)seq_max_segs * cand_W * 2);
    cd.take(64);
    bd_start = bd.take((size_t)(n_ptiles + 1) * FQGPU_SEQ_MODELS * 4);
    bd_pre = bd.take((size_t)(n_ptiles + 1) * FQGPU_SEQ_MODELS * 2);
    bd.take(64);
    ts_status = ts.take((size_t)n_tiles * 8);
    ts_counter = ts.take(16);
    ts_run_count = ts.take((size_t)n_tiles * 4);
    ts_edges = ts.take((size_t)n_tiles * 16, 16);
    if (serial_seq) {
      bytes.seq_plan = sp.total;
      bytes.seq_fbuf = (size_t)seq_max_segs * fstride * 2 + 64;
      bytes.seq_cand = cand_W ? cd.total : 0;
      bytes.seq_cbuf = cb.total;
      bytes.seq_bdesc = bd.total;
    } else {
      bytes.seg_arrays = g.total;
      bytes.seq_fbuf = ((size_t)gen_max_segs + B) * fstride * 2 + 64;
    }
    if (tile_path) {
      bytes.tile_runs = tile_runs_bytes;
      bytes.tile_sync = ts.total;
    }
  }
};

struct EncLanePlan {
  size_t rec_start = 0;
  size_t n_cnt32 = 0;
  size_t n_off = 0;
  size_t first_sym = 0;
  size_t tile_first = 0;
  size_t scan_tmp = 0;
  EncSpan n_cnt, lens;
  EncSpan first_sym_of[2];

  EncLanePlan(unsigned R, size_t n_bases) {
    EncCarve c, f;
    rec_start = n_off = (size_t)(R + 1) * 4;
    n_cnt = c.take((size_t)R * 4);
    lens = c.take((size_t)R * 4);
    n_cnt32 = c.total;
    first_sym_of[0] = f.take(R);
    first_sym_of[1] = f.take(R);
    f.take(16);
    first_sym = f.total;
    tile_first = (n_bases + TS_TILE - 1) / TS_TILE * 4;
    scan_tmp = ((size_t)R / 1024 + 64) * 16;
  }
};
```

fqcomp28_amd/csrc/enc_records_hist.h:

```cpp


struct __attribute__((packed)) FqBytes16 { uint32_t w[4]; };
__global__ void __launch_bounds__(256)
k_readlens_ncount(const uint8_t *__restrict__ raw, const fqgpu_rec *__restrict__ recs, unsigned R,
                  uint16_t *__restrict__ readlens, uint16_t *__restrict__ n_count,
                  uint32_t *__restrict__ n_cnt32, uint32_t *__restrict__ lens32, BlockResult *res) {
  if (res != nullptr && blockIdx.x == 0 && threadIdx.x < sizeof(BlockResult) / 4) reinterpret_cast<uint32_t *>(res)[threadIdx.x] = 0u;
  const unsigned waves = (gridDim.x * blockDim.x) >> 6;
  const unsigned lane = fq_lane(), sub = lane >> 4, l = lane & 15u;
  for (unsigned r0 = ((blockIdx.x * blockDim.x + threadIdx.x) >> 6) * 4; r0 < R; r0 += waves * 4) {
    const unsigned r = r0 + sub;
    const bool on = r < R;
    const fqgpu_rec rec = recs[on ? r : R - 1];
    const unsigned len = on ? rec.len : 0u;
    const uint8_t *s = raw + rec.seq_off;
    unsigned cnt = 0;
    for (unsigned off = l * 16; off < len; off += 256) {
      const FqBytes16 v = *reinterpret_cast<const FqBytes16 *>(s + off);
      const unsigned live = min(16u, len - off);
#pragma unroll
      for (unsigned i = 0; i < 16; i++)
        cnt += (i < live && ((v.w[i >> 2] >> (8 * (i & 3))) & 0xFFu) == 'N') ? 1u : 0u;
    }
#pragma unroll
// ... 448 lines not shown
        }
        if (n & 1u) {
          const unsigned o = n & 2u;
          ckey_seq[e_first + o] = (uint8_t)(o ? kb >> 16 : kb);
          ckey_qual[e_first + o] = (uint16_t)(o ? cq23 : cq01);
        }
        if (cut) {
#pragma unroll
          for (unsigned i = 0; i < 4; i++)
            if ((valid >> i) & 1u) {
              ckey_seq[e_first + i] = (uint8_t)k16[i];
              ckey_qual[e_first + i] = (uint16_t)cq[i];
            }
        }
#pragma unroll
        for (unsigned i = 0; i < 4; i++) {
          const unsigned one = (valid >> i) & 1u;
          atomicAdd(&hist_s[k16[i] & 0xFFu], one);
          atomicAdd(&hist_q[cq[i] >> 1], one << (16u * (cq[i] & 1u)));
        }
      };
#pragma unroll
      for (int d = 0; d < K1Q_DEPTH - 1; d++)
        if ((unsigned)d < nch) fetch(d, (unsigned)d);
      unsigned c = 0;
      for (; c + 2u * (K1Q_DEPTH - 1) < nch; c += K1Q_DEPTH) {
#pragma unroll
        for (int d = 0; d < K1Q_DEPTH; d++) {
          fetch((d + K1Q_DEPTH - 1) % K1Q_DEPTH, c + d + (K1Q_DEPTH - 1));
          consume(d);
        }
      }
      for (; c < nch; c += K1Q_DEPTH) {
#pragma unroll
        for (int d = 0; d < K1Q_DEPTH; d++) {
          const unsigned cur = c + d;
          if (cur < nch) {
            if (cur + (K1Q_DEPTH - 1) < nch) fetch((d + K1Q_DEPTH - 1) % K1Q_DEPTH, cur + (K1Q_DEPTH - 1));
            consume(d);
          }
        }
      }
      if (covered >= we || r0 + 64u >= R) break;
      r0 += 64u;
    }
  }
  if (bad_s) atomicOr(&res->s[0].bad_symbol, 1u);
  if (bad_q) atomicOr(&res->s[1].bad_symbol, 1u);
  __syncthreads();
  for (unsigned c = threadIdx.x; c < BS; c += blockDim.x) tile_hist_seq[(size_t)tile * BS + c] = (uint16_t)hist_s[c];
  uint32_t *rowq = reinterpret_cast<uint32_t *>(tile_hist_qual + (size_t)tile * BQ);
  for (unsigned c = threadIdx.x; c < BQ / 2; c += blockDim.x) rowq[c] = hist_q[c];
}

template <class HT>
__global__ void __launch_bounds__(256)
k_group_sum(const HT *__restrict__ tile_hist, unsigned n_tiles, unsigned B,
            uint32_t *__restrict__ group_sum) {
  const unsigned c = blockIdx.x * blockDim.x + threadIdx.x;
  const unsigned g = blockIdx.y;
  if (c >= B) return;
  const unsigned t0 = g * GROUP_TILES, t1 = min(t0 + GROUP_TILES, n_tiles);
  uint32_t acc = 0;
  for (unsigned t = t0; t < t1; t++) acc += tile_hist[(size_t)t * B + c];
  group_sum[(size_t)g * B + c] = acc;
}

__global__ void __launch_bounds__(256)
k_group_prefix(uint32_t *__restrict__ group_sum, unsigned n_groups, unsigned B, uint32_t *__restrict__ ctx_count) {
  const unsigned c = blockIdx.x * blockDim.x + threadIdx.x;
  if (c >= B) return;
  uint32_t acc = 0;
  for (unsigned g0 = 0; g0 < n_groups; g0 += 8) {
    uint32_t v[8];
#pragma unroll
    for (unsigned k = 0; k < 8; k++) v[k] = g0 + k < n_groups ? group_sum[(size_t)(g0 + k) * B + c] : 0u;
#pragma unroll
    for (unsigned k = 0; k < 8; k++)
      if (g0 + k < n_groups) { group_sum[(size_t)(g0 + k) * B + c] = acc; acc += v[k]; }
  }
  ctx_count[c] = acc;
}

__global__ void __launch_bounds__(1024)
k_ctx_layout(unsigned B, unsigned S, uint32_t *__restrict__ arrays, uint32_t *__restrict__ fill_none) {
  if (fill_none)
    for (unsigned c = threadIdx.x; c < B; c += blockDim.x) fill_none[c] = 0xFFFFFFFFu;
  __shared__ unsigned part[3][1024];
  uint32_t *ctx_count = arrays, *ctx_start = arrays + B, *seg_base = ctx_start + B + 1,
           *item_base = seg_base + B + 1;
  const unsigned per = (B + blockDim.x - 1) / blockDim.x;
  const unsigned c0 = threadIdx.x * per, c1 = min(c0 + per, B);
  unsigned a0 = 0, a1 = 0, a2 = 0;
  for (unsigned c = c0; c < c1; c++) {
    const unsigned n = ctx_count[c];
    const unsigned nseg = (n + S - 1) / S;
    a0 += (n + CTX_PAD - 1) & ~(CTX_PAD - 1);
    a1 += nseg;
    a2 += (nseg + 63) >> 6;
  }
  part[0][threadIdx.x] = a0; part[1][threadIdx.x] = a1; part[2][threadIdx.x] = a2;
  __syncthreads();
  if (threadIdx.x < 3) {
    unsigned run = 0;
    for (unsigned i = 0; i < blockDim.x; i++) {
      const unsigned v = part[threadIdx.x][i];
      part[threadIdx.x][i] = run;
      run += v;
    }
  }
  __syncthreads();
  a0 = part[0][threadIdx.x]; a1 = part[1][threadIdx.x]; a2 = part[2][threadIdx.x];
  for (unsigned c = c0; c < c1; c++) {
    const unsigned n = ctx_count[c];
    const unsigned nseg = (n + S - 1) / S;
    ctx_start[c] = a0; seg_base[c] = a1; item_base[c] = a2;
    a0 += (n + CTX_PAD - 1) & ~(CTX_PAD - 1);
    a1 += nseg;
    a2 += (nseg + 63) >> 6;
  }
  if (c1 == B && c0 < B) { ctx_start[B] = a0; seg_base[B] = a1; item_base[B] = a2; }
}

template <class HT>
__global__ void __launch_bounds__(256)
k_tile_base(const HT *__restrict__ tile_hist, const uint32_t *__restrict__ group_sum,
            const uint32_t *__restrict__ ctx_start, unsigned n_tiles, unsigned B,
            uint32_t *__restrict__ tile_base) {
  const unsigned c = blockIdx.x * blockDim.x + threadIdx.x;
  const unsigned g = blockIdx.y;
  if (c >= B) return;
  const unsigned t0 = g * GROUP_TILES, t1 = min(t0 + GROUP_TILES, n_tiles);
  uint32_t acc = ctx_start[c] + group_sum[(size_t)g * B + c];
  for (unsigned t = t0; t < t1; t++) {
    tile_base[(size_t)t * B + c] = acc;
    acc += tile_hist[(size_t)t * B + c];
  }
}
```

fqcomp28_amd/csrc/encode.hip:

```cpp
#include "fqgpu_internal.h"
#include "enc_plan.h"

#include <cstdio>
#include <cstdlib>
#include <cstring>
#include <type_traits>

#ifdef FQGPU_EXPERIMENTS
__device__ unsigned long long g_ts_prof[48];
void fq_ts_prof_dump() {
  unsigned long long h[48];
  if (hipMemcpyFromSymbol(h, HIP_SYMBOL(g_ts_prof), sizeof(h)) != hipSuccess) return;
  const char *names[4] = {"partition<Qual>", "partition<Seq>", "gather_pack<Qual>", "gather_pack<Seq>"};
  for (int k = 0; k < 4; k++)
    fprintf(stderr, "ts_prof %-18s phase ticks (100 MHz, summed over workgroups): %llu %llu %llu %llu | ranker alone %llu | K3: store wait %llu patch %llu run map %llu\n",
            names[k], h[8 * k], h[8 * k + 1], h[8 * k + 2], h[8 * k + 3], h[8 * k + 4], h[8 * k + 5], h[8 * k + 6], h[8 * k + 7]);
  for (int k = 0; k < 2; k++)
    fprintf(stderr, "ts_prof %-18s loader thread 64, ticks summed over workgroups: wait for the requested batch (taken in front of finish) %llu | finish %llu | deposit %llu | request %llu | barrier %llu\n",
            names[k], h[32 + 8 * k], h[33 + 8 * k], h[34 + 8 * k], h[35 + 8 * k], h[36 + 8 * k]);
}
#endif

namespace {

// ... 43 lines not shown
  return ctx->lds_atomics_ordered && ctx->tile_sorted && !ctx->seq_generic && !fq_debug_skip() && !fq_debug_k1();
}
static bool dbg_no_alias() {
  static const bool on = fq_debug_flag("FQGPU_DEBUG_NO_ALIAS");
  return on;
}

struct EncStage {
  fqgpu_ctx *ctx;
  hipStream_t st;
  bool off;
  EncStage(fqgpu_ctx *c, hipStream_t s, const char *span, unsigned mask = 0, unsigned bit = 0, const char *skipk = nullptr)
      : ctx(c), st(s), off((mask & bit) != 0 || (skipk && fq_debug_skipk(skipk))) { fq_timer_span_begin(ctx, span, st); }
  ~EncStage() { fq_timer_span_end(ctx, st); }
  EncStage(const EncStage &) = delete;
};
#define FQ_SPAN(x) (M::STREAM ? "qual." x : "seq." x)

template <class M>
EncPlan make_plan(const fqgpu_ctx *ctx, const fqgpu_dblock *b) {
  const DevTables &tab = ctx->tab[M::STREAM];
  EncPlanIn in;
  in.n_sym = (unsigned)b->n_bases;
  in.R = (unsigned)b->n_recs;
  in.stream = M::STREAM; in.B = M::B; in.A = M::A;
  in.max_log = tab.max_log;
  in.two_sym = tab.next2 != nullptr;
  in.serial_seq = M::STREAM == 0 && !ctx->seq_generic;
  in.tile_path = ctx->lds_atomics_ordered && ctx->tile_sorted && (M::STREAM == 1 || in.serial_seq);
  in.seg_len = ctx->seg_len; in.seq_segment = ctx->seq_segment;
  in.seq_group = ctx->seq_group; in.seq_group_min = ctx->seq_group_min;
  in.seq_cand_cap = ctx->seq_cand_cap; in.seq_cand_prefix = ctx->seq_cand_prefix;
  in.n_cus = ctx->n_cus;
  return EncPlan(in);
}
static_assert(TILE_SEQ % SEQ_BATCH == 0 && SEQ_BATCH % PACK_TILE == 0 && TILE_QUAL % PACK_TILE == 0, "a packing tile lies inside one partition tile");
static_assert(ts_run_stride<SeqModel>() == (unsigned)SeqModel::B && ts_run_stride<QualModel>() == (unsigned)QualModel::B, "EncPlan sizes tile_runs by min(B, TS_TILE)");

static int reserve_k1(EncScratch &sc, const EncShape &sh) {
  int rc;
  if ((rc = sc.keys.reserve(sh.bytes.keys))) return rc;
  return sc.tile_hist.reserve(sh.bytes.tile_hist);
}
static int reserve(EncScratch &sc, const EncPlan &p) {
  const EncBytes &n = p.bytes;
  const struct { DevBuf &buf; size_t bytes; } want[] = {
      {sc.slot_of, n.slot_of}, {sc.keys, n.keys}, {sc.sorted_sym, n.sorted_sym}, {sc.out16, n.out16}, {sc.tile_hist, n.tile_hist},
      {sc.tile_base, n.tile_base}, {sc.group_sum, n.group_sum}, {sc.ctx_arrays, n.ctx_arrays}, {sc.seg_state, n.seg_state},
      {sc.seg_arrays, n.seg_arrays}, {sc.seq_plan, n.seq_plan}, {sc.seq_fbuf, n.seq_fbuf}, {sc.seq_cand, n.seq_cand},
      {sc.seq_cbuf, n.seq_cbuf}, {sc.seq_bdesc, n.seq_bdesc}, {sc.tile_bits, n.tile_bits}, {sc.tile_bit_base, n.tile_bit_base},
      {sc.tile_runs, n.tile_runs}, {sc.tile_sync, n.tile_sync}, {sc.dbg_enc16, dbg_no_alias() ? p.n_pad * 2 : 0}};
  for (const auto &w : want)
    if (int rc = w.bytes ? w.buf.reserve(w.bytes) : FQGPU_OK) return rc;
  return FQGPU_OK;
}
static int reserve(EncLane &lane, const EncLanePlan &lp) {
  int rc;
  if ((rc = lane.rec_start.reserve(lp.rec_start)) || (rc = lane.n_cnt32.reserve(lp.n_cnt32)) || (rc = lane.n_off.reserve(lp.n_off)) ||
      (rc = lane.first_sym.reserve(lp.first_sym)))
    return rc;
  return lane.tile_first.reserve(lp.tile_first);
}

template <class T> T *at(const DevBuf &b, const EncSpan &s) { return b.p ? reinterpret_cast<T *>(b.as<uint8_t>() + s.off) : nullptr; }

struct EncViews {
  const uint32_t *rec_start;
  StreamResult *res;
  uint16_t *ckey;
  uint8_t *csym;
  uint16_t *enc16;
  uint32_t *arrays, *ctx_start, *seg_base;
  uint16_t *final_state;
  uint16_t *lpos16;
  SeqBatchDesc bd;
  unsigned long long *ts_status;
  unsigned *ts_counter;
  uint32_t *ts_run_count;
  uint4 *ts_edges;
  const uint8_t *first_sym;
  const uint32_t *tile_first;
  SegArrays sa;
  ItemArrays ia;
  uint32_t *plan, *plan_work, *plan_seg_base;
  uint16_t *entry, *fbuf, *cbuf, *item_entry;
  SeqHandover hand;
};

template <class M>
EncViews make_views(EncLane &lane, const EncPlan &p, const EncLanePlan &lp, fqgpu_dblock *b, bool fused) {
  EncScratch &sc = lane.enc[M::STREAM];
  EncViews v{};
  v.rec_start = lane.rec_start.as<uint32_t>();
  v.res = &b->result->s[M::STREAM];
  v.ckey = at<uint16_t>(sc.keys, p.ckey);
  v.csym = at<uint8_t>(sc.keys, p.csym);
  v.enc16 = dbg_no_alias() ? sc.dbg_enc16.as<uint16_t>() : v.ckey;
  v.arrays = at<uint32_t>(sc.ctx_arrays, p.ctx_count);
  v.ctx_start = at<uint32_t>(sc.ctx_arrays, p.ctx_start);
  v.seg_base = at<uint32_t>(sc.ctx_arrays, p.seg_base);
  v.final_state = sc.seg_state.as<uint16_t>();
  v.lpos16 = sc.slot_of.as<uint16_t>();
  v.bd.start = at<uint32_t>(sc.seq_bdesc, p.bd_start);
  v.bd.pre = at<uint16_t>(sc.seq_bdesc, p.bd_pre);
  v.ts_status = at<unsigned long long>(sc.tile_sync, p.ts_status);
  v.ts_counter = at<unsigned>(sc.tile_sync, p.ts_counter);
  v.ts_run_count = at<uint32_t>(sc.tile_sync, p.ts_run_count);
  v.ts_edges = at<uint4>(sc.tile_sync, p.ts_edges);
  if (fused) {
    v.first_sym = at<uint8_t>(lane.first_sym, lp.first_sym_of[M::STREAM]);
    v.tile_first = lane.tile_first.as<uint32_t>();
  }
  v.fbuf = sc.seq_fbuf.as<uint16_t>();
  if (p.serial_seq) {
    v.plan = at<uint32_t>(sc.seq_plan, p.sp_fitem);
    v.plan_work = at<uint32_t>(sc.seq_plan, p.sp_work);
    v.plan_seg_base = at<uint32_t>(sc.seq_plan, p.sp_seg);
    v.entry = at<uint16_t>(sc.seq_plan, p.sp_entry);
    v.cbuf = at<uint16_t>(sc.seq_cbuf, p.cb_func);
    v.item_entry = at<uint16_t>(sc.seq_cbuf, p.cb_item_entry);
    v.hand.W = p.cand_W; v.hand.cap = p.cand_cap; v.hand.P = p.cand_P;
    if (p.cand_W) {
      v.hand.cand0 = at<uint16_t>(sc.seq_cand, p.cand0);
      v.hand.cand = at<uint16_t>(sc.seq_cand, p.cand);
      v.hand.counts = &b->result->seq_groups_handed;
    }
  } else {
    v.sa.anchor = at<uint32_t>(sc.seg_arrays, p.sa_anchor);
    v.sa.usym = at<uint32_t>(sc.seg_arrays, p.sa_usym);
    v.sa.entry_state = at<uint16_t>(sc.seg_arrays, p.sa_entry);
    v.sa.cand_exit = at<uint16_t>(sc.seg_arrays, p.sa_cand);
    v.sa.cls = at<uint8_t>(sc.seg_arrays, p.sa_cls);
    v.ia.has_g = at<uint32_t>(sc.seg_arrays, p.ia_has_g);
    v.ia.item_entry = at<uint16_t>(sc.seg_arrays, p.ia_entry);
    v.ia.g = at<uint16_t>(sc.seg_arrays, p.ia_g);
  }
  return v;
}

template <class F> void with_hist_type(bool tile_path, F &&f) {
  if (tile_path) f((uint16_t *)nullptr); else f((uint32_t *)nullptr);
}
#define FQ_HIST_TYPE(h) std::remove_pointer_t<decltype(h)>
template <class F> void with_log_width(unsigned max_log, F &&f) {
  if (max_log <= 11) f(std::integral_constant<unsigned, 32>()); else f(std::integral_constant<unsigned, 64>());
}
template <class F> void with_cand_width(unsigned W, F &&f) {
  if (W == 16) f(std::integral_constant<unsigned, 16>());
  else if (W == 32) f(std::integral_constant<unsigned, 32>());
  else f(std::integral_constant<unsigned, 64>());
}

template <class M>
void launch_hist(EncScratch &sc, const EncPlan &p, const EncViews &v, hipStream_t st, const fqgpu_dblock *b) {
  with_hist_type(p.tile_path, [&](auto *h) {
    using H = FQ_HIST_TYPE(h);
    hipLaunchKernelGGL((k_tile_hist<M, H>), dim3(p.n_tiles), dim3(256), 0, st, b->raw, b->recs, v.rec_start, p.R, p.n_sym, p.T,
                       sc.tile_hist.as<H>(), v.ckey, v.csym, v.res, fq_debug_k1());
  });
}

static void launch_layout(EncScratch &sc, const EncShape &sh, bool tile_path, unsigned S, uint32_t *usym, hipStream_t st) {
  const unsigned B = sh.B;
  const dim3 grid((B + 255) / 256, sh.n_groups);
  uint32_t *arrays = at<uint32_t>(sc.ctx_arrays, sh.ctx_count), *group_sum = sc.group_sum.as<uint32_t>();
  with_hist_type(tile_path, [&](auto *h) {
    using H = FQ_HIST_TYPE(h);
    hipLaunchKernelGGL(k_group_sum<H>, grid, dim3(256), 0, st, sc.tile_hist.as<H>(), sh.n_tiles, B, group_sum);
    hipLaunchKernelGGL(k_group_prefix, dim3((B + 255) / 256), dim3(256), 0, st, group_sum, sh.n_groups, B, arrays);
    hipLaunchKernelGGL(k_ctx_layout, dim3(1), dim3(1024), 0, st, B, S, arrays, usym);
    hipLaunchKernelGGL(k_tile_base<H>, grid, dim3(256), 0, st, sc.tile_hist.as<H>(), group_sum, at<uint32_t>(sc.ctx_arrays, sh.ctx_start),
                       sh.n_tiles, B, sc.tile_base.as<uint32_t>());
  });
}

template <class M, bool FUSED>
void launch_tile_partition(EncScratch &sc, const EncShape &sh, hipStream_t st, const uint16_t *ckey, const uint8_t *csym, uint32_t *run_count,
                           unsigned long long *status, unsigned *counter, const uint32_t *rec_start, const uint8_t *first_sym, const uint32_t *tile_first) {
  hipLaunchKernelGGL((k_tile_partition<M, FUSED>), dim3(sh.n_tiles), dim3(TS_THREADS), 0, st, ckey, csym, sh.n_sym, sc.tile_hist.as<uint16_t>(),
                     sc.tile_base.as<uint32_t>(), sc.sorted_sym.as<uint8_t>(), sc.slot_of.as<uint16_t>(), sc.tile_runs.as<uint2>(), run_count, status, counter,
                     rec_start, sh.R, first_sym, tile_first);
}

template <class M>
void launch_partition(const fqgpu_ctx *ctx, EncScratch &sc, const EncPlan &p, const EncViews &v, hipStream_t st, bool fused) {
  const bool ordered = ctx->lds_atomics_ordered;
  if (p.tile_path) {
    if (fused) launch_tile_partition<M, true>(sc, p, st, v.ckey, v.csym, v.ts_run_count, v.ts_status, v.ts_counter, v.rec_start, v.first_sym, v.tile_first);
    else launch_tile_partition<M, false>(sc, p, st, v.ckey, v.csym, v.ts_run_count, v.ts_status, v.ts_counter, v.rec_start, v.first_sym, v.tile_first);
  } else if (p.serial_seq) {
    if (ordered)
      hipLaunchKernelGGL(k_scatter_seq<true>, dim3(p.n_tiles), dim3(64), 0, st, v.ckey, p.n_sym, p.T, sc.tile_base.as<uint32_t>(),
                         sc.sorted_sym.as<uint8_t>(), v.lpos16, v.bd, fq_debug_no_sym(0));
    else
      hipLaunchKernelGGL(k_scatter_seq<false>, dim3(p.n_tiles), dim3(64), 0, st, v.ckey, p.n_sym, p.T, sc.tile_base.as<uint32_t>(),
                         sc.sorted_sym.as<uint8_t>(), v.lpos16, v.bd, fq_debug_no_sym(0));
  } else if (ordered) {
    hipLaunchKernelGGL((k_scatter<M, true>), dim3(p.n_tiles), dim3(64), 0, st, v.ckey, v.csym, p.n_sym, p.T, sc.tile_base.as<uint32_t>(),
                       sc.sorted_sym.as<uint8_t>(), sc.slot_of.as<uint32_t>(), fq_debug_no_sym(M::STREAM));
  } else {
    hipLaunchKernelGGL((k_scatter<M, false>), dim3(p.n_tiles), dim3(64), 0, st, v.ckey, v.csym, p.n_sym, p.T, sc.tile_base.as<uint32_t>(),
                       sc.sorted_sym.as<uint8_t>(), sc.slot_of.as<uint32_t>(), fq_debug_no_sym(M::STREAM));
  }
}

static void launch_seq_chains(fqgpu_ctx *ctx, EncScratch &sc, const EncPlan &p, const EncViews &v, hipStream_t st, unsigned mask) {
  const DevTables &tab = ctx->tab[0];
  const uint8_t *sym = sc.sorted_sym.as<uint8_t>();
  const uint16_t *pow = nullptr;
  for (unsigned i = 0; i < FQ_SEQ_POW_SETS; i++)
    if (tab.seq_pow[i] && tab.seq_pow_S[i] == p.seq_S) pow = tab.seq_pow[i];
  const SeqHandover no_hand{};
  const unsigned log_size = 1u << tab.max_log;
  if (EncStage s{ctx, st, "seq.plan", mask, 8u}; !s.off)
    hipLaunchKernelGGL(k_seq_segplan, dim3(1), dim3(256), 0, st, v.arrays, p.seq_S, p.Q, p.gmin, p.wpg * p.rounds, v.plan);
  const bool dbg_skip = fq_debug_flag("FQGPU_DEBUG_SKIP_SEQ_CHAIN");
  if (EncStage s{ctx, st, "seq.setfunc", mask, 8u, "setfunc"}; s.off || dbg_skip) {
  } else if (p.two_sym) {
    hipLaunchKernelGGL((k_seq_setfunc<32, true>), dim3(min(p.max_fitems, ctx->setfunc_wgs ? ctx->setfunc_wgs : ctx->n_cus)), dim3(SETS_WAVES2 * 64),
                       32 * log_size + SETS_WAVES2 * sizeof(SetsWaveLds11) + 16, st, sym, v.arrays, v.plan, tab.logs, tab.next2,
                       4 * p.next_stride, pow, p.next_stride, p.seq_S, p.Q, p.gmin, p.rounds, p.fstride, v.fbuf, v.plan_work, 32 * log_size, v.hand);
  } else {
    hipLaunchKernelGGL((k_seq_setfunc<64, false>), dim3(min(p.max_fitems, 2 * ctx->n_cus)), dim3(SETS_WAVES * 64),
                       8 * log_size + SETS_WAVES * sizeof(SetsWaveLds) + 16, st, sym, v.arrays, v.plan, tab.logs, tab.next1,
                       p.next_stride, pow, p.next_stride, p.seq_S, p.Q, p.gmin, p.rounds, p.fstride, v.fbuf, v.plan_work, 8 * log_size, no_hand);
  }
  if (dbg_skip) return;
  if (p.cand_W) {
    const unsigned clds = 32u << tab.max_log;
    if (EncStage s{ctx, st, "seq.candwalk", mask, 8u, "candwalk"}; !s.off)
      with_cand_width(p.cand_W, [&](auto w) {
        hipLaunchKernelGGL(k_seq_candwalk<decltype(w)::value>, dim3(p.max_fitems), dim3(CANDW_WAVES * 64), clds, st, sym, v.arrays, v.plan, tab.logs,
                           tab.next2, 4 * p.next_stride, p.seq_S, p.Q, p.gmin, p.rounds, v.hand);
      });
  }
  if (EncStage s{ctx, st, "seq.resolve", mask, 8u, "resolve"}; !s.off)
    with_log_width(tab.max_log, [&](auto w) {
      constexpr unsigned W = decltype(w)::value;
      hipLaunchKernelGGL(k_seq_resolve<W>, dim3(1), dim3(SEQ_RESOLVE_THREADS), 0, st, v.plan, tab.logs, v.fbuf, p.fstride, p.Q, p.gmin, v.cbuf,
                         v.item_entry, v.entry, W == 32 ? v.hand : no_hand);
    });
  if (EncStage s{ctx, st, "seq.chains", mask, 8u, "emit"}; !s.off)
    hipLaunchKernelGGL(k_seq_emit, dim3(p.max_eitems), dim3(64), 8 * log_size, st, sym, sc.out16.as<uint16_t>(), v.arrays, v.plan, tab.ct, tab.ct_off,
                       tab.next1, p.next_stride, p.seq_S, v.entry, v.final_state, v.res);
}

template <class M>
void launch_generic_chains(fqgpu_ctx *ctx, EncScratch &sc, const EncPlan &p, const EncViews &v, hipStream_t st, unsigned mask) {
  const DevTables &tab = ctx->tab[M::STREAM];
  constexpr unsigned B = M::B;
  const uint8_t *sym = sc.sorted_sym.as<uint8_t>();
  uint16_t *out16 = sc.out16.as<uint16_t>();
  if (EncStage s{ctx, st, FQ_SPAN("scan"), mask, 8u, "scan"}; !s.off)
    hipLaunchKernelGGL(k_seg_scan<M>, dim3((p.gen_max_segs + 3) / 4), dim3(256), 0, st, sym, v.arrays, tab.reset_mask, tab.norm, tab.logs, p.S, v.sa);
  if (EncStage s{ctx, st, FQ_SPAN("stage1"), mask, 8u, "stage1"}; !s.off)
    with_log_width(tab.max_log, [&](auto w) {
      hipLaunchKernelGGL((k_seg_stage1<M, decltype(w)::value>), dim3(p.max_items + p.cand_grid + p.gen_pbase + B), dim3(64), p.lds_ct, st, sym, out16,
                         v.arrays, tab.ct, tab.ct_off, v.final_state, p.S, p.max_items, p.cand_grid, p.gen_pbase, p.fstride, v.sa, v.fbuf, v.res);
    });
  if (EncStage s{ctx, st, FQ_SPAN("heads"), mask, 8u, "heads"}; !s.off)
    hipLaunchKernelGGL(k_seg_heads<M>, dim3(p.cand_grid), dim3(64), p.lds_ct, st, sym, v.arrays, tab.ct, tab.ct_off, p.S, p.fstride, v.sa, v.fbuf);
  if (EncStage s{ctx, st, FQ_SPAN("resolve"), mask, 8u, "qresolve"}; !s.off) {
    with_log_width(tab.max_log, [&](auto w) {
      hipLaunchKernelGGL((k_seg_compose<M, decltype(w)::value>), dim3(p.max_items), dim3(64), 0, st, v.arrays, tab.logs, v.fbuf, p.gen_pbase, p.fstride, v.sa, v.ia);
    });
    hipLaunchKernelGGL(k_seg_resolve2<M>, dim3((B + 255) / 256), dim3(256), 0, st, v.arrays, tab.logs, p.fstride, v.sa, v.ia);
    hipLaunchKernelGGL(k_seg_resolve3<M>, dim3((p.max_items + 255) / 256), dim3(256), 0, st, v.arrays, tab.logs, v.fbuf, p.gen_pbase, p.fstride, v.sa, v.ia);
  }
  if (EncStage s{ctx, st, FQ_SPAN("walk2"), mask, 8u, "walk2"}; !s.off)
    hipLaunchKernelGGL((k_seg_walk<M, 2>), dim3(p.max_items), dim3(64), p.lds_ct, st, sym, out16, v.arrays, tab.ct, tab.ct_off, v.final_state, p.S, v.sa, v.res);
}

template <class M>
void launch_pack(fqgpu_ctx *ctx, EncScratch &sc, const EncPlan &p, const EncViews &v, hipStream_t st, unsigned mask, uint8_t *out_dev, size_t cap) {
  const DevTables &tab = ctx->tab[M::STREAM];
  uint16_t *out16 = sc.out16.as<uint16_t>();
  uint32_t *out = reinterpret_cast<uint32_t *>(out_dev);
  unsigned long long *bit_base = sc.tile_bit_base.as<unsigned long long>();
  if (p.tile_path) {
    if (EncStage s{ctx, st, FQ_SPAN("gatherpack"), mask, 16u, M::STREAM ? "k6q" : "k6s"}; !s.off)
      hipLaunchKernelGGL(k_tile_gather_pack<M>, dim3(p.n_tiles), dim3(TS_GP_THREADS), 0, st, v.lpos16, sc.tile_runs.as<uint2>(), v.ts_run_count, out16,
                         p.n_sym, p.n_tiles, v.ts_status, v.ts_counter, tab.log_prefix, (unsigned long long)cap, out, v.res, bit_base, v.ts_edges);
    return;
  }
  if (EncStage s{ctx, st, FQ_SPAN("bitcount"), mask, 16u}; s.off) {
  } else if (p.serial_seq) {
    hipLaunchKernelGGL(k_bitcount_seq, dim3((p.n_sym + SEQ_BATCH - 1) / SEQ_BATCH), dim3(PACK_THREADS), 0, st, v.lpos16, v.bd, out16, p.n_sym,
                       sc.tile_bits.as<uint32_t>(), v.enc16);
  } else {
    hipLaunchKernelGGL(k_bitcount, dim3(p.n_ptiles), dim3(PACK_THREADS), 0, st, sc.slot_of.as<uint32_t>(), out16, p.n_sym, sc.tile_bits.as<uint32_t>(), v.enc16);
  }
  if (EncStage s{ctx, st, FQ_SPAN("bitscan"), mask, 32u}; !s.off)
    hipLaunchKernelGGL(k_bitscan, dim3(1), dim3(1024), 0, st, sc.tile_bits.as<uint32_t>(), p.n_ptiles, bit_base, tab.log_prefix, p.B, (unsigned long long)cap, out, v.res);
  if (EncStage s{ctx, st, FQ_SPAN("pack"), mask, 64u}; !s.off)
    hipLaunchKernelGGL(k_pack, dim3(p.n_ptiles), dim3(PACK_THREADS), 0, st, v.enc16, p.n_sym, bit_base, out, v.res);
}

template <class M>
int launch_index(fqgpu_ctx *ctx, EncScratch &sc, const EncPlan &p, const EncViews &v, hipStream_t st, fqgpu_dblock *b) {
  const DevTables &tab = ctx->tab[M::STREAM];
  const unsigned stride = ctx->index_stride;
  const unsigned n_snap = fq_index_n_snap(p.n_sym, stride);
  const size_t bytes = fq_index_bytes(n_snap, M::B);
  if (int rc = b->index[M::STREAM].grow(bytes + 64, 0, true)) return rc;
  {
    EncStage s{ctx, st, FQ_SPAN("index")};
    hipLaunchKernelGGL(k_index_meta<M>, dim3(n_snap / 256 + 1), dim3(256), 0, st, b->raw, b->recs, v.rec_start, p.R, p.n_sym, stride,
                       sc.tile_bit_base.as<unsigned long long>(), p.tile_path ? TS_TILE : PACK_TILE, b->index[M::STREAM]);
    if (n_snap)
      hipLaunchKernelGGL(k_index_states<M>, dim3(M::B, (n_snap + 63) / 64), dim3(64), p.lds_ct, st, sc.sorted_sym.as<uint8_t>(), v.arrays,
                         sc.tile_base.as<uint32_t>(), p.T, p.n_sym, stride, p.serial_seq ? v.plan_seg_base : v.seg_base,
                         p.serial_seq ? v.entry : v.sa.entry_state, p.serial_seq ? 1 : 0, p.serial_seq ? p.seq_S : p.S, tab.ct, tab.ct_off,
                         v.final_state, b->index[M::STREAM]);
  }
  b->index_bytes[M::STREAM] = bytes;
  return FQGPU_OK;
}

template <class M>
int encode_stream(fqgpu_ctx *ctx, EncLane &lane, const EncPlan &p, const EncLanePlan &lp, hipStream_t st, fqgpu_dblock *b,
                  uint8_t *out_dev, size_t cap, unsigned flags) {
  EncScratch &sc = lane.enc[M::STREAM];
  const DevTables &tab = ctx->tab[M::STREAM];
  unsigned mask = fq_debug_skip();
  if ((mask & 256u) && M::STREAM == 1) mask = 0;
  if ((mask & 512u) && M::STREAM == 0) mask = 0;
  const bool fused = fused_k1(ctx);
  if (int rc = reserve(sc, p)) return rc;
  const EncViews v = make_views<M>(lane, p, lp, b, fused);
  if (M::STREAM == 1) {
    lane.diag_cls = v.sa.cls;
    lane.diag_anchor = v.sa.anchor;
    lane.diag_n_segs = v.seg_base + M::B;
  }

  if (EncStage s{ctx, st, FQ_SPAN("tile_hist"), mask, 1u}; !s.off && !fused) launch_hist<M>(sc, p, v, st, b);
  if (EncStage s{ctx, st, FQ_SPAN("layout"), mask, 2u, M::STREAM ? "k2q" : "k2s"}; !s.off) launch_layout(sc, p, p.tile_path, p.S, v.sa.usym, st);
  if (EncStage s{ctx, st, FQ_SPAN("scatter"), mask, 4u, M::STREAM ? "k3q" : "k3s"}; !s.off) launch_partition<M>(ctx, sc, p, v, st, fused);
  if (p.serial_seq) launch_seq_chains(ctx, sc, p, v, st, mask);
  else launch_generic_chains<M>(ctx, sc, p, v, st, mask);
  launch_pack<M>(ctx, sc, p, v, st, mask, out_dev, cap);
  if (EncStage s{ctx, st, FQ_SPAN("epilogue"), mask, 128u}; !s.off)
    hipLaunchKernelGGL(k_epilogue<M>, dim3(1), dim3(256), 0, st, v.arrays, v.final_state, tab.logs, tab.log_prefix, reinterpret_cast<uint32_t *>(out_dev),
                       v.res, p.tile_path ? v.ts_edges : (const uint4 *)nullptr, p.n_tiles);
  b->index_bytes[M::STREAM] = 0;
  if ((flags & FQGPU_F_DECODE_INDEX) && !mask)
    if (int rc = launch_index<M>(ctx, sc, p, v, st, b)) return rc;
  FQ_HIP(hipGetLastError());
  return FQGPU_OK;
}

#undef FQ_SPAN
#undef FQ_HIST_TYPE

}

int fq_encode_init_device() {
  FQ_HIP(hipFuncSetAttribute(reinterpret_cast<const void *>(&k_seq_setfunc<32, true>), hipFuncAttributeMaxDynamicSharedMemorySize, 160 * 1024));
  FQ_HIP(hipFuncSetAttribute(reinterpret_cast<const void *>(&k_seq_setfunc<64, false>), hipFuncAttributeMaxDynamicSharedMemorySize, 160 * 1024));
  return FQGPU_OK;
}

namespace {
__global__ void __launch_bounds__(256)
k_probe_lds_atomic_order(unsigned iters, unsigned *__restrict__ bad) {
  __shared__ unsigned cnt[4][1024];
  const unsigned wave = threadIdx.x >> 6, lane = fq_lane();
  unsigned s = (blockIdx.x * blockDim.x + threadIdx.x) * 40503u + 12345u;
  unsigned nbad = 0;
  for (unsigned it = 0; it < iters; it++) {
    for (unsigned c = lane; c < 1024; c += 64) cnt[wave][c] = 0;
    fq_lds_wave_sync();
    s ^= s << 13; s ^= s >> 17; s ^= s << 5;
    const unsigned range = 1u << ((it % 6) * 2);
    const unsigned key = (s >> 8) % range;
    const bool active = (s & 15u) != 0;
    const bool packed = (it & 1u) != 0;
    unsigned got = 0;
    if (active) {
      if (packed) got = (atomicAdd(&cnt[wave][key >> 1], 1u << (16 * (key & 1u))) >> (16 * (key & 1u))) & 0xFFFFu;
      else got = atomicAdd(&cnt[wave][key], 1u);
    }
    unsigned ref = 0;
    for (int l = 0; l < 64; l++) {
      const unsigned k2 = (unsigned)__shfl((int)key, l);
      const int a2 = __shfl((int)active, l);
      if ((unsigned)l < lane && a2 && k2 == key) ref++;
    }
    if (active && got != ref) nbad++;
    fq_lds_wave_sync();
  }
  if (nbad) atomicAdd(bad, nbad);
}

}

int fq_probe_lds_atomic_order(hipStream_t st, bool *ordered) {
  unsigned *bad = fq_dev_alloc<unsigned>(1);
  if (!bad) return FQGPU_E_NOMEM;
  unsigned h = 1;
  hipError_t e = hipMemsetAsync(bad, 0, 4, st);
  if (e == hipSuccess) {
    hipLaunchKernelGGL(k_probe_lds_atomic_order, dim3(512), dim3(256), 0, st, 96u, bad);
    e = hipMemcpyAsync(&h, bad, 4, hipMemcpyDeviceToHost, st);
  }
  if (e == hipSuccess) e = hipStreamSynchronize(st);
  (void)hipFree(bad);
  if (e != hipSuccess) return FQGPU_E_HIP;
  *ordered = h == 0;
  return FQGPU_OK;
}

namespace {
__global__ void __launch_bounds__(256)
k_hist_sorted_qual(const uint8_t *__restrict__ sorted_sym, const uint32_t *__restrict__ arrays, unsigned S,
                   uint32_t *__restrict__ counts) {
  constexpr unsigned B = QualModel::B, A = QualModel::A;
  __shared__ uint32_t s_bins[4][A];
  const uint32_t *ctx_count = arrays, *ctx_start = arrays + B, *seg_base = ctx_start + B + 1;
  const unsigned wave = threadIdx.x >> 6, lane = fq_lane(), seg = blockIdx.x * 4 + wave;
  if (seg >= seg_base[B]) return;
  const unsigned c = seg_ctx_of<QualModel>(seg_base, seg), k = seg - seg_base[c];
  const unsigned n = ctx_count[c], begin = k * S, end = min(n, begin + S);
  const uint8_t *sym = sorted_sym + ctx_start[c];
  uint32_t *bins = s_bins[wave];
  bins[lane] = 0;
  fq_lds_wave_sync();
  for (unsigned p0 = begin; p0 < end; p0 += 1024) {
    const unsigned p = p0 + 16 * lane;
    uint4 v = make_uint4(0, 0, 0, 0);
    if (p < end) v = *reinterpret_cast<const uint4 *>(sym + p);
    const unsigned w[4] = {v.x, v.y, v.z, v.w};
#pragma unroll
    for (int j = 0; j < 16; j++) {
      const unsigned s = (w[j >> 2] >> (8 * (j & 3))) & (A - 1);
      bool on = p + j < end;
      const unsigned long long live = __ballot(on);
      if (!live) break;
      const unsigned lead = (unsigned)__ffsll((long long)live) - 1u;
      const unsigned s_lead = (unsigned)__shfl((int)s, (int)lead);
      const unsigned long long same = __ballot(on && s == s_lead);
      if (lane == lead) atomicAdd(&bins[s_lead], (unsigned)__popcll(same));
      if (on && s != s_lead) atomicAdd(&bins[s], 1u);
    }
  }
  fq_lds_wave_sync();
  if (bins[lane]) atomicAdd(&counts[(size_t)c * A + lane], bins[lane]);
}
}

namespace {
void launch_hist2(EncLane &lane, const EncLanePlan &lp, hipStream_t st, const uint8_t *raw, const fqgpu_rec *recs, unsigned R, unsigned n_sym,
                  BlockResult *res) {
  hipLaunchKernelGGL(k_tile_hist2, dim3((n_sym + TS_TILE - 1) / TS_TILE), dim3(256), 0, st, raw, recs, lane.rec_start.as<uint32_t>(), R, n_sym, TS_TILE,
                     lane.enc[0].tile_hist.as<uint16_t>(), lane.enc[0].keys.as<uint8_t>(), lane.enc[1].tile_hist.as<uint16_t>(),
                     lane.enc[1].keys.as<uint16_t>(), at<uint8_t>(lane.first_sym, lp.first_sym_of[0]), at<uint8_t>(lane.first_sym, lp.first_sym_of[1]),
                     lane.tile_first.as<uint32_t>(), at<uint32_t>(lane.n_cnt32, lp.n_cnt), res);
}
}

int fq_qual_counts_sorted(hipStream_t st, const uint8_t *raw_dev, const fqgpu_rec *recs_dev, size_t n_recs, size_t n_bases,
                          uint32_t *counts_dev, uint32_t *err_dev) {
  constexpr unsigned S = 4096;
  const unsigned R = (unsigned)n_recs, n_sym = (unsigned)n_bases;
  const EncShape shq(n_sym, R, QualModel::B, TS_TILE), shs(n_sym, R, SeqModel::B, TS_TILE);
  const EncLanePlan lp(R, n_bases);
  const unsigned max_segs = n_sym / S + shq.B + 1;
  EncLane lane;
  EncScratch &sq = lane.enc[1], &ss = lane.enc[0];
  DevBuf readlens, result;
  int rc = FQGPU_OK;
  do {
    if ((rc = lane.rec_start.reserve(lp.rec_start)) || (rc = lane.n_cnt32.reserve(lp.n_cnt32)) ||
        (rc = readlens.reserve((size_t)R * 2)) || (rc = result.reserve(sizeof(BlockResult))) || (rc = lane.first_sym.reserve(lp.first_sym)) ||
        (rc = lane.tile_first.reserve(lp.tile_first)) || (rc = reserve_k1(ss, shs)) || (rc = reserve_k1(sq, shq)) ||
        (rc = sq.slot_of.reserve(shq.lpos16_bytes)) || (rc = sq.sorted_sym.reserve(shq.bytes.sorted_sym)) || (rc = sq.tile_base.reserve(shq.bytes.tile_base)) ||
        (rc = sq.group_sum.reserve(shq.bytes.group_sum)) || (rc = sq.ctx_arrays.reserve(shq.bytes.ctx_arrays)) ||
        (rc = sq.tile_runs.reserve(shq.tile_runs_bytes)) || (rc = sq.tile_sync.reserve((size_t)shq.n_tiles * 4 + 64)))
      break;
    uint32_t *n_cnt32 = at<uint32_t>(lane.n_cnt32, lp.n_cnt), *lens32 = at<uint32_t>(lane.n_cnt32, lp.lens), *rec_start = lane.rec_start.as<uint32_t>();
    BlockResult *res = result.as<BlockResult>();
    if (hipMemsetAsync(res, 0, sizeof(BlockResult), st) != hipSuccess) { rc = FQGPU_E_HIP; break; }
    hipLaunchKernelGGL(k_readlens, dim3((unsigned)min((size_t)(R + 255) / 256, (size_t)2048)), dim3(256), 0, st, recs_dev, R,
                       readlens.as<uint16_t>(), n_cnt32, lens32, (BlockResult *)nullptr);
    if ((rc = fq_scan_u32_to_u32(st, lens32, R, rec_start, lane.scan_tmp))) break;
    launch_hist2(lane, lp, st, raw_dev, recs_dev, R, n_sym, res);
    launch_layout(sq, shq, true, S, nullptr, st);
    launch_tile_partition<QualModel, true>(sq, shq, st, sq.keys.as<uint16_t>(), nullptr, sq.tile_sync.as<uint32_t>(), nullptr, nullptr, rec_start,
                                           at<uint8_t>(lane.first_sym, lp.first_sym_of[1]), lane.tile_first.as<uint32_t>());
    hipLaunchKernelGGL(k_hist_sorted_qual, dim3((max_segs + 3) / 4), dim3(256), 0, st, sq.sorted_sym.as<uint8_t>(), sq.ctx_arrays.as<uint32_t>(), S, counts_dev);
    BlockResult h;
    if (hipMemcpyAsync(&h, res, sizeof(h), hipMemcpyDeviceToHost, st) != hipSuccess || hipStreamSynchronize(st) != hipSuccess ||
        hipGetLastError() != hipSuccess) { rc = FQGPU_E_HIP; break; }
    if (h.s[0].bad_symbol || h.s[1].bad_symbol) {
      uint32_t one = 1;
      if (hipMemcpy(err_dev, &one, 4, hipMemcpyHostToDevice) != hipSuccess) rc = FQGPU_E_HIP;
    }
  } while (0);
  (void)hipStreamSynchronize(st);
  readlens.release();
  result.release();
  fq_release_bufs(lane);
  fq_release_bufs(ss);
  fq_release_bufs(sq);
  return rc;
}

namespace {
int launch_record_scan(EncLane &lane, const EncLanePlan &lp, hipStream_t st, const fqgpu_dblock *b, int mode) {
  const unsigned R = (unsigned)b->n_recs, rscan_chunks = (R + RSCAN_CHUNK - 1) / RSCAN_CHUNK;
  const size_t need = (size_t)rscan_chunks * 8 + 16;
  if (need > lane.rscan.cap) {
    int rr = lane.rscan.reserve(need);
    if (rr) return rr;
    FQ_HIP(hipMemsetAsync(lane.rscan.p, 0, lane.rscan.cap, st));
    lane.rscan_tickets = 0;
  }
  lane.rscan_epoch = (lane.rscan_epoch + 1u) & 0xFFFFFFu;
  if (lane.rscan_epoch == 0u) {
    FQ_HIP(hipMemsetAsync(lane.rscan.p, 0, lane.rscan.cap, st));
    lane.rscan_tickets = 0;
    lane.rscan_epoch = 1u;
  }
  unsigned *ticket = lane.rscan.as<unsigned>();
  unsigned long long *status = reinterpret_cast<unsigned long long *>(lane.rscan.as<uint8_t>() + 16);
  uint32_t *n_cnt32 = at<uint32_t>(lane.n_cnt32, lp.n_cnt);
  if (mode == 0)
    hipLaunchKernelGGL(k_record_scan<0>, dim3(rscan_chunks), dim3(RSCAN_THREADS), 0, st, b->recs, n_cnt32, R, b->readlens, lane.rec_start.as<uint32_t>(),
                       status, ticket, lane.rscan_tickets, lane.rscan_epoch, b->result);
  else
    hipLaunchKernelGGL(k_record_scan<1>, dim3(rscan_chunks), dim3(RSCAN_THREADS), 0, st, b->recs, n_cnt32, R, b->n_count, lane.n_off.as<uint32_t>(),
                       status, ticket, lane.rscan_tickets, lane.rscan_epoch, b->result);
  lane.rscan_tickets += rscan_chunks;
  return FQGPU_OK;
}
}

int fq_encode_reserve(fqgpu_ctx *ctx, const fqgpu_dblock *b) {
  if (b->n_recs == 0 || b->n_bases == 0) return FQGPU_E_ARG;
  EncLane *lane = fq_next_lane(ctx, b->n_bases);
  if (!lane) return FQGPU_E_NOMEM;
  const EncLanePlan lp((unsigned)b->n_recs, b->n_bases);
  const EncPlan seq = make_plan<SeqModel>(ctx, b), qual = make_plan<QualModel>(ctx, b);
  lane->forget_diag();
  int rc;
  if ((rc = reserve(*lane, lp))) return rc;
  if (fused_k1(ctx) && ((rc = reserve_k1(lane->enc[0], seq)) || (rc = reserve_k1(lane->enc[1], qual)))) return rc;
  if ((rc = lane->scan_tmp.reserve(lp.scan_tmp)) || (rc = reserve(lane->enc[1], qual))) return rc;
  return reserve(lane->enc[0], seq);
}

int fq_encode_launch(fqgpu_ctx *ctx, fqgpu_dblock *b, unsigned flags, hipEvent_t wait, hipStream_t *done) {
  const unsigned R = (unsigned)b->n_recs, n_sym = (unsigned)b->n_bases;
  if (R == 0 || b->n_bases == 0) return FQGPU_E_ARG;
  EncLane *lanep = fq_next_lane(ctx, b->n_bases, b);
  if (!lanep) return FQGPU_E_NOMEM;
  EncLane &lane = *lanep;
  hipStream_t st = lane.st_seq;
  if (done) *done = st;
  int rc;
  if (wait) FQ_HIP(hipStreamWaitEvent(st, wait, 0));
  if (b->ev_encoded) FQ_HIP(hipStreamWaitEvent(st, b->ev_encoded, 0));
  lane.forget_diag();
  lane.diag_stamp = ++ctx->encodes;
  b->diag_stamp = b->owner == ctx ? lane.diag_stamp : 0;
  const bool fused = fused_k1(ctx);
  const EncLanePlan lp(R, b->n_bases);
  const EncPlan seq = make_plan<SeqModel>(ctx, b), qual = make_plan<QualModel>(ctx, b);
  if ((rc = reserve(lane, lp))) return rc;
  uint32_t *n_cnt32 = at<uint32_t>(lane.n_cnt32, lp.n_cnt), *lens32 = at<uint32_t>(lane.n_cnt32, lp.lens);
// ... 34 lines not shown
```

fqcomp28_amd/csrc/fqgpu_internal.h:

```cpp
#pragma once

#include <hip/hip_runtime.h>
#include <stdint.h>
#include <stddef.h>

#include <new>

#include "../../include/fqgpu.h"

#define FQ_WAVE 64

struct SeqModel {
  static constexpr int B = FQGPU_SEQ_MODELS;
  static constexpr int A = FQGPU_SEQ_ALPHA;
  static constexpr int KEYBITS = 8;
  static constexpr int STREAM = 0;
};
struct QualModel {
  static constexpr int B = FQGPU_QUAL_MODELS;
  static constexpr int A = FQGPU_QUAL_ALPHA;
  static constexpr int KEYBITS = 13;
  static constexpr int STREAM = 1;
};

#define FQ_DENTRY(new_state, sym, nb) ((((uint32_t)(new_state)) << 18) | ((uint32_t)(nb) << 9) | ((uint32_t)(sym) << 3))
#define FQ_DENTRY_TO_ZSTD(w) ((((uint32_t)(w)) >> 18) | (((((uint32_t)(w)) >> 3) & 63u) << 16) | (((((uint32_t)(w)) >> 9) & 15u) << 24))

struct DevTables {
  int16_t *norm = nullptr;
  uint32_t *logs = nullptr;
  uint32_t *log_prefix = nullptr;
  uint32_t *ct = nullptr;
  uint32_t *ct_off = nullptr;
  uint32_t *dt = nullptr;
  uint32_t *dt_off = nullptr;
  unsigned long long *reset_mask = nullptr;
  uint16_t *next1 = nullptr;
  uint16_t *next2 = nullptr;
  uint16_t *seq_pow[4] = {nullptr, nullptr, nullptr, nullptr};
  unsigned seq_pow_S[4] = {0, 0, 0, 0};
  uint32_t max_log = 0;
  size_t ct_words = 0, dt_words = 0;
};
#define FQ_SEQ_POW_SETS 4
#ifndef FQ_SEQ_CAND_CAP_DEFAULT
#define FQ_SEQ_CAND_CAP_DEFAULT 32u
#endif
#ifndef FQ_SEQ_CAND_PREFIX_DEFAULT
#define FQ_SEQ_CAND_PREFIX_DEFAULT 1u
#endif

struct StreamResult {
  unsigned long long total_bits;
  unsigned long long len;
  unsigned int overflow;
  unsigned int bad_symbol;
  unsigned int refixed;
  unsigned int corrupt;
};

struct BlockResult {
  StreamResult s[2];
  unsigned long long n_pos_len;
  unsigned int seq_groups_handed;
  unsigned int seq_groups_kept;
};

#define FQ_HIP(call)                                                 \
  do {                                                               \
    hipError_t e_ = (call);                                          \
    if (e_ != hipSuccess) return fq_hip_error(e_, __FILE__, __LINE__); \
  } while (0)

int fq_hip_error(hipError_t e, const char *file, int line);

template <class T> static inline T *fq_dev_alloc(size_t n) {
  void *p = nullptr;
  if (hipMalloc(&p, (n ? n : 1) * sizeof(T)) != hipSuccess) return nullptr;
  return reinterpret_cast<T *>(p);
}

template <class T> struct DevArray {
  T *p = nullptr;
  size_t n = 0;
  operator T *() const { return p; }
  T *operator->() const { return p; }
  size_t bytes() const { return n * sizeof(T); }
  int grow(size_t need, size_t slack = 0, bool check_free = false) {
    if (p && need <= n) return FQGPU_OK;
    const hipError_t e = release();
    if (check_free) FQ_HIP(e);
    if (!(p = fq_dev_alloc<T>(need + slack))) return FQGPU_E_NOMEM;
    n = need + slack;
    return FQGPU_OK;
  }
  hipError_t release() {
    const hipError_t e = p ? hipFree(p) : hipSuccess;
    p = nullptr;
    n = 0;
    return e;
  }
};

struct DevBuf {
  void *p = nullptr;
  size_t cap = 0;
  int reserve(size_t bytes) {
    if (bytes <= cap) return FQGPU_OK;
    if (p) (void)hipFree(p);
    p = nullptr;
    cap = 0;
    const size_t want = bytes + bytes / 8 + 256;
    if (hipMalloc(&p, want) != hipSuccess) { p = nullptr; return FQGPU_E_NOMEM; }
    cap = want;
    return FQGPU_OK;
  }
  void release() { if (p) (void)hipFree(p); p = nullptr; cap = 0; }
  template <class T> T *as() const { return reinterpret_cast<T *>(p); }
};

template <class T> struct FqBufOf { const char *name; DevBuf T::*m; };
#define FQ_B(T, m) {#m, &T::m}
#define FQ_SCRATCH_BUFS(T, ...)                                                      \
  inline constexpr FqBufOf<T> fq_bufs_##T[] = {__VA_ARGS__};                         \
  template <class F> static inline void fq_each_buf(T &s, F &&f) {                   \
    for (const FqBufOf<T> &e : fq_bufs_##T) f(e.name, s.*(e.m));                     \
  }
template <class T> static inline void fq_release_bufs(T &s) { fq_each_buf(s, [](const char *, DevBuf &b) { b.release(); }); }

struct KernelTimer;

struct ParseScratch {
  DevBuf cnt, base, sum, nl_pos, scan_tmp;
  size_t total_nl = 0;
};
FQ_SCRATCH_BUFS(ParseScratch, FQ_B(ParseScratch, cnt), FQ_B(ParseScratch, base), FQ_B(ParseScratch, sum), FQ_B(ParseScratch, nl_pos),
                FQ_B(ParseScratch, scan_tmp))

struct HdrResult {
  unsigned long long first_error;
  unsigned long long total;
  unsigned long long off[3 * FQGPU_HDR_MAX_FIELDS];
  uint32_t size[3 * FQGPU_HDR_MAX_FIELDS];
};
struct HdrScratch {
  DevBuf wg_sum, wg_base, out, first, res;
  HdrResult *host_res = nullptr;
  uint8_t *host_first = nullptr;
  unsigned n_fields = 0;
  size_t bound = 0;
  bool pending = false;
  bool collected = false;
  void release_host() {
    if (host_res) (void)hipHostFree(host_res);
    if (host_first) (void)hipHostFree(host_first);
    host_res = nullptr; host_first = nullptr; pending = collected = false;
  }
};
FQ_SCRATCH_BUFS(HdrScratch, FQ_B(HdrScratch, wg_sum), FQ_B(HdrScratch, wg_base), FQ_B(HdrScratch, out), FQ_B(HdrScratch, first),
                FQ_B(HdrScratch, res))

struct EncScratch {
  DevBuf slot_of, keys, sorted_sym, out16, tile_hist, tile_base, group_sum, ctx_arrays, seg_state, seg_arrays;
  DevBuf seq_bdesc, seq_plan, seq_fbuf, seq_cbuf, seq_cand, tile_bits, tile_bit_base, tile_runs, tile_sync;
  DevBuf dbg_enc16;
};
FQ_SCRATCH_BUFS(EncScratch, FQ_B(EncScratch, slot_of), FQ_B(EncScratch, keys), FQ_B(EncScratch, sorted_sym), FQ_B(EncScratch, out16),
                FQ_B(EncScratch, tile_hist), FQ_B(EncScratch, tile_base), FQ_B(EncScratch, group_sum), FQ_B(EncScratch, ctx_arrays),
                FQ_B(EncScratch, seg_state), FQ_B(EncScratch, seg_arrays), FQ_B(EncScratch, seq_bdesc), FQ_B(EncScratch, seq_plan),
                FQ_B(EncScratch, seq_fbuf), FQ_B(EncScratch, seq_cbuf), FQ_B(EncScratch, seq_cand), FQ_B(EncScratch, tile_bits),
                FQ_B(EncScratch, tile_bit_base), FQ_B(EncScratch, dbg_enc16), FQ_B(EncScratch, tile_runs), FQ_B(EncScratch, tile_sync))

struct EncLane {
  hipStream_t st_seq = nullptr, st_qual = nullptr;
  hipEvent_t ev_fork = nullptr, ev_join = nullptr;
  DevBuf rec_start;
  DevBuf n_cnt32;
  DevBuf n_off;
  DevBuf first_sym;
  DevBuf tile_first;
  DevBuf rscan;
  unsigned rscan_epoch = 0, rscan_tickets = 0;
  DevBuf scan_tmp;
  EncScratch enc[2];
  const uint8_t *diag_cls = nullptr;
  const uint32_t *diag_anchor = nullptr;
  const uint32_t *diag_n_segs = nullptr;
  unsigned long long diag_stamp = 0;
  void forget_diag() { diag_cls = nullptr; diag_anchor = nullptr; diag_n_segs = nullptr; diag_stamp = 0; }
};
FQ_SCRATCH_BUFS(EncLane, FQ_B(EncLane, rec_start), FQ_B(EncLane, n_cnt32), FQ_B(EncLane, n_off), FQ_B(EncLane, first_sym),
                FQ_B(EncLane, tile_first), FQ_B(EncLane, rscan), FQ_B(EncLane, scan_tmp))

struct FqChunkField {
  unsigned long long flags, content, lengths;
  uint32_t n_flags, n_content, n_lengths;
  uint32_t first_off, first_len;
  int32_t first_val;
  uint32_t type;
  uint32_t sep;
};
struct FqChunkFmt {
  uint32_t n_fields, n_recs, n_tiles, pad;
  unsigned long long raw_len, stage_len, readlens, first;
  FqChunkField f[FQGPU_HDR_MAX_FIELDS];
};
struct FqChunkResult {
  unsigned long long bad;
  unsigned long long total;
};
struct ChunkScratch {
  DevBuf stage, agg, cls, clp, hlen, tlen, toff, res, scan_tmp;
  DevBuf pick;
  uint8_t *host = nullptr;
  size_t host_cap = 0, stage_len = 0;
  unsigned n_fields = 0, n_tiles = 0;
  bool host_grow(size_t n) {
    if (n <= host_cap) return true;
    delete[] host;
    host = new (std::nothrow) uint8_t[n + n / 8];
    host_cap = host ? n + n / 8 : 0;
    return host != nullptr;
  }
  void release_host() {
    delete[] host;
    host = nullptr;
    host_cap = 0;
  }
};
FQ_SCRATCH_BUFS(ChunkScratch, FQ_B(ChunkScratch, stage), FQ_B(ChunkScratch, agg), FQ_B(ChunkScratch, cls), FQ_B(ChunkScratch, clp),
                FQ_B(ChunkScratch, hlen), FQ_B(ChunkScratch, tlen), FQ_B(ChunkScratch, toff), FQ_B(ChunkScratch, res),
                FQ_B(ChunkScratch, scan_tmp), FQ_B(ChunkScratch, pick))

struct CrcScratch {
  DevBuf tab, rem, res, chk, clen, coff, flat, scan_tmp;
  uint32_t *host = nullptr;
  bool tab_built = false;
  void release_host();
};
FQ_SCRATCH_BUFS(CrcScratch, FQ_B(CrcScratch, tab), FQ_B(CrcScratch, rem), FQ_B(CrcScratch, res), FQ_B(CrcScratch, chk),
                FQ_B(CrcScratch, clen), FQ_B(CrcScratch, coff), FQ_B(CrcScratch, flat), FQ_B(CrcScratch, scan_tmp))

struct StatsScratch {
  DevBuf out, slabs, bad;
  unsigned *host_bad = nullptr;
  bool attr_set = false;
  void release_host();
};
FQ_SCRATCH_BUFS(StatsScratch, FQ_B(StatsScratch, out), FQ_B(StatsScratch, slabs), FQ_B(StatsScratch, bad))

struct SelectResult;
struct SelectScratch {
  DevBuf ksize, hstart, win, clip, places, keep, koff, dst, res, scan_tmp;
  DevBuf probe_out, probe_places;
  DevBuf mark, limit;
  DevBuf overlap_out, overlap_pairs;
  DevBuf correct_in, correct_fixed;
  DevBuf merge_in, merge_size, merge_bits, merge_out;
  void *host = nullptr;
  void release_host();
  int begin(hipStream_t st);
  int finish(hipStream_t st, const SelectResult *&result);
};
FQ_SCRATCH_BUFS(SelectScratch, FQ_B(SelectScratch, ksize), FQ_B(SelectScratch, hstart), FQ_B(SelectScratch, win), FQ_B(SelectScratch, clip),
                FQ_B(SelectScratch, places), FQ_B(SelectScratch, keep), FQ_B(SelectScratch, koff), FQ_B(SelectScratch, dst),
                FQ_B(SelectScratch, res), FQ_B(SelectScratch, scan_tmp), FQ_B(SelectScratch, probe_out), FQ_B(SelectScratch, probe_places),
                FQ_B(SelectScratch, mark), FQ_B(SelectScratch, limit), FQ_B(SelectScratch, overlap_out), FQ_B(SelectScratch, overlap_pairs),
                FQ_B(SelectScratch, correct_in), FQ_B(SelectScratch, correct_fixed), FQ_B(SelectScratch, merge_in),
                FQ_B(SelectScratch, merge_size), FQ_B(SelectScratch, merge_bits), FQ_B(SelectScratch, merge_out))

#define FQ_MAX_LANES 8
#define FQ_RECENT_BLOCKS 8
// ... 345 lines not shown
```

fqcomp28_amd/csrc/tables.hip:

```cpp
#include "fqgpu_internal.h"

namespace {

__global__ void __launch_bounds__(256)
k_hist_seq(const uint8_t *__restrict__ raw, const fqgpu_rec *__restrict__ recs, unsigned R,
           uint32_t *__restrict__ counts, uint32_t *__restrict__ err) {
  __shared__ uint32_t hist[FQGPU_SEQ_MODELS * FQGPU_SEQ_ALPHA];
  for (unsigned i = threadIdx.x; i < FQGPU_SEQ_MODELS * FQGPU_SEQ_ALPHA; i += blockDim.x) hist[i] = 0;
  __syncthreads();
  const unsigned waves = (gridDim.x * blockDim.x) >> 6;
  const unsigned lane = fq_lane();
  bool bad = false;
  for (unsigned r = (blockIdx.x * blockDim.x + threadIdx.x) >> 6; r < R; r += waves) {
    const fqgpu_rec rec = recs[r];
    const uint8_t *s = raw + rec.seq_off;
    unsigned carry = 0xD7u;
    for (unsigned base = 0; base < rec.len; base += 64) {
      const unsigned i = base + lane;
      const unsigned ch = i < rec.len ? s[i] : 'N';
      const bool keep = i < rec.len && ch != 'N';
      const unsigned code = fq_base_code(ch);
      bad |= fq_base_sym(ch) > 3u;
      const unsigned long long km = __ballot(keep);
      unsigned long long m = km & ((1ull << lane) - 1ull);
      const unsigned avail = (unsigned)__popcll(m);
      unsigned ctx = 0;
#pragma unroll
      for (int k = 1; k <= 4; k++) {
        const int src = m ? 63 - __clzll(m) : 0;
        const unsigned from_wave = (unsigned)__shfl((int)code, src);
        const unsigned back = (unsigned)k > avail ? (unsigned)k - avail : 1u;
        const unsigned from_carry = (carry >> (2 * (4 - back))) & 3u;
        const unsigned c = (unsigned)k <= avail ? from_wave : from_carry;
        ctx |= c << (2 * (4 - k));
        if (m) m &= ~(1ull << src);
      }
      if (keep) atomicAdd(&hist[ctx * 4 + code], 1u);
      const unsigned kept = (unsigned)__popcll(km);
      if (kept) {
        const int lastl = 63 - __clzll(km);
        const unsigned ctx_last = (unsigned)__shfl((int)ctx, lastl);
        const unsigned code_last = (unsigned)__shfl((int)code, lastl);
        carry = (ctx_last >> 2) + (code_last << 6);
      }
    }
  }
  if (bad) atomicOr(err, 1u);
  __syncthreads();
  for (unsigned i = threadIdx.x; i < FQGPU_SEQ_MODELS * FQGPU_SEQ_ALPHA; i += blockDim.x)
    if (hist[i]) atomicAdd(&counts[i], hist[i]);
}

__global__ void __launch_bounds__(256)
k_hist_qual(const uint8_t *__restrict__ raw, const fqgpu_rec *__restrict__ recs, unsigned R,
            uint32_t *__restrict__ counts, uint32_t *__restrict__ err) {
  const unsigned waves = (gridDim.x * blockDim.x) >> 6;
  const unsigned lane = fq_lane();
  bool bad = false;
  for (unsigned r = (blockIdx.x * blockDim.x + threadIdx.x) >> 6; r < R; r += waves) {
    const fqgpu_rec rec = recs[r];
    const uint8_t *qs = raw + rec.qual_off;
    for (unsigned base = 0; base < rec.len; base += 64) {
      const unsigned i = base + lane;
      bool active = i < rec.len;
      unsigned cell = 0;
      if (active) {
        const unsigned q = (unsigned)qs[i] - 33u;
        const unsigned a = i >= 1 ? (unsigned)qs[i - 1] - 33u : 0u;
        const unsigned b = i >= 2 ? (unsigned)qs[i - 2] - 33u : 0u;
        const unsigned c = i >= 3 ? (unsigned)qs[i - 3] - 33u : 0u;
        if (q >= FQGPU_QUAL_ALPHA) { bad = true; active = false; }
        cell = fq_qual_ctx(a & 63u, b & 63u, c & 63u) * FQGPU_QUAL_ALPHA + (q & 63u);
      }
      for (int round = 0; round < 2; round++) {
        const unsigned long long am = __ballot(active);
        if (!am) break;
        const int lead = __ffsll((long long)am) - 1;
        const unsigned lead_cell = (unsigned)__shfl((int)cell, lead);
        const bool same = active && cell == lead_cell;
        const unsigned long long sm = __ballot(same);
        if ((int)lane == lead) atomicAdd(&counts[lead_cell], (unsigned)__popcll(sm));
        if (same) active = false;
      }
// ... 84 lines not shown
  unsigned long long total = cnt;
#pragma unroll
  for (int d = 32; d > 0; d >>= 1) total += __shfl_xor(total, d);
  if (total == 0 || total > 0xFFFFFFFFull) { if (lane == 0) atomicOr(err, 2u); return; }
  const unsigned t = optimal_table_log(total, A - 1);
  const unsigned long long scale = 62 - t;
  const unsigned long long step = (1ull << 62) / (unsigned)total;
  const unsigned long long vstep = 1ull << (scale - 20);
  const unsigned low_thr = (unsigned)(total >> t);
  int p = 0;
  if (__ballot(on && (unsigned long long)cnt == total)) {
    if (lane == 0) atomicOr(err, 4u);
    return;
  }
  if (on && cnt != 0) {
    if (cnt <= low_thr) {
      p = -1;
    } else {
      p = (int)(short)(((unsigned long long)cnt * step) >> scale);
      if (p < 8) {
        const unsigned long long to_beat = vstep * rtb[p];
        p += (((unsigned long long)cnt * step) - ((unsigned long long)p << scale)) > to_beat;
      }
    }
  }
  int used = p == -1 ? 1 : p;
#pragma unroll
  for (int d = 32; d > 0; d >>= 1) used += __shfl_xor(used, d);
  const int still = (1 << (int)t) - used;
  int best = p > 0 ? p : 0;
#pragma unroll
  for (int d = 32; d > 0; d >>= 1) { const int o = __shfl_xor(best, d); best = o > best ? o : best; }
  const unsigned long long at_best = __ballot(on && p > 0 && p == best);
  const unsigned largest = at_best ? (unsigned)__ffsll((long long)at_best) - 1u : 0u;
  const int norm_largest = __shfl(p, (int)largest);
  if (-still >= (norm_largest >> 1)) {
    s_cnt[lane] = cnt;
    __syncthreads();
    if (lane == 0 && normalize_m2(s_norm, t, s_cnt, total, A - 1) != 0) atomicOr(err, 8u);
    __syncthreads();
    p = s_norm[lane];
  } else if (lane == largest) {
    p += still;
  }
  if (on) norm_out[(size_t)ctx * A + lane] = (int16_t)p;
  if (lane == 0) { logs[ctx] = t; atomicMax(max_log, t); }
}

__global__ void __launch_bounds__(1024)
k_log_prefix(const uint32_t *__restrict__ logs, unsigned B, uint32_t *__restrict__ prefix,
             uint32_t *__restrict__ ct_off, uint32_t *__restrict__ dt_off, unsigned A,
             uint32_t *__restrict__ totals) {
  __shared__ unsigned part[3][1024];
  const unsigned per = (B + blockDim.x - 1) / blockDim.x;
  const unsigned c0 = threadIdx.x * per, c1 = min(c0 + per, B);
  unsigned a = 0, b = 0, d = 0;
  for (unsigned c = c0; c < c1; c++) {
    const unsigned t = logs[c];
    a += t;
    b += 1u + (1u << (t - 1)) + 2u * A;
    d += 1u + (1u << t);
  }
  part[0][threadIdx.x] = a; part[1][threadIdx.x] = b; part[2][threadIdx.x] = d;
  __syncthreads();
  if (threadIdx.x < 3) {
    unsigned run = 0;
    for (unsigned i = 0; i < blockDim.x; i++) {
      const unsigned v = part[threadIdx.x][i];
      part[threadIdx.x][i] = run;
      run += v;
    }
    totals[threadIdx.x] = run;
  }
  __syncthreads();
  a = part[0][threadIdx.x]; b = part[1][threadIdx.x]; d = part[2][threadIdx.x];
  for (unsigned c = c0; c < c1; c++) {
    const unsigned t = logs[c];
    prefix[c] = a; ct_off[c] = b; dt_off[c] = d;
    a += t; b += 1u + (1u << (t - 1)) + 2u * A; d += 1u + (1u << t);
  }
  if (c1 == B && c0 < B) prefix[B] = a;
}

template <int A, int ABITS>
__global__ void __launch_bounds__(64)
k_build_tables(const int16_t *__restrict__ norm, const uint32_t *__restrict__ logs,
               const uint32_t *__restrict__ ct_off, const uint32_t *__restrict__ dt_off,
               uint32_t *__restrict__ ct_pool, uint32_t *__restrict__ dt_pool,
               uint32_t *__restrict__ err) {
  __shared__ uint8_t cell[1 << 12];
  __shared__ uint32_t cum_pos[65];
  __shared__ uint32_t cumul[65];
  __shared__ uint32_t next_rank[64];
  const unsigned ctx = blockIdx.x, lane = threadIdx.x;
  const unsigned t = logs[ctx];
  if (t < 5 || t > 12) { if (lane == 0) atomicOr(err, 16u); return; }
  const unsigned size = 1u << t, mask = size - 1;
  const unsigned step = (size >> 1) + (size >> 3) + 3;
  const bool on = lane < (unsigned)A;
  const int n = on ? (int)norm[(size_t)ctx * A + lane] : 0;
  uint32_t *ct = ct_pool + ct_off[ctx];
  uint32_t *dt = dt_pool + dt_off[ctx];

  const unsigned pos_n = n > 0 ? (unsigned)n : 0u;
  const unsigned any_n = n == -1 ? 1u : pos_n;
  unsigned inc_pos = pos_n, inc_any = any_n;
#pragma unroll
  for (int d = 1; d < 64; d <<= 1) {
    const unsigned o1 = __shfl_up(inc_pos, d), o2 = __shfl_up(inc_any, d);
    if (lane >= (unsigned)d) { inc_pos += o1; inc_any += o2; }
  }
  const unsigned sum_any = __shfl(inc_any, 63);
  if (sum_any != size) { if (lane == 0) atomicOr(err, 32u); return; }
  cum_pos[lane + 1] = inc_pos;
  cumul[lane + 1] = inc_any;
  if (lane == 0) { cum_pos[0] = 0; cumul[0] = 0; }
  next_rank[lane] = 0;
  const unsigned long long low_mask = __ballot(n == -1);
  const unsigned n_low = (unsigned)__popcll(low_mask);
  const unsigned high = size - 1 - n_low;
  if (n == -1) cell[size - 1 - fq_mbcnt(low_mask)] = (uint8_t)lane;
  __syncthreads();

  unsigned seen = 0;
  for (unsigned jb = 0; jb < size; jb += 64) {
    const unsigned j = jb + lane;
    const unsigned pos = (j * step) & mask;
    const bool ok = j < size && pos <= high;
    const unsigned long long okm = __ballot(ok);
    if (ok) {
      const unsigned k = seen + fq_mbcnt(okm);
      unsigned lo = 0, hi = A - 1;
      while (lo < hi) {
        const unsigned mid = lo + ((hi - lo + 1) >> 1);
        if (cum_pos[mid] <= k) lo = mid; else hi = mid - 1;
      }
      cell[pos] = (uint8_t)lo;
    }
    seen += (unsigned)__popcll(okm);
  }
  __syncthreads();

  if (lane == 0) {
    ct[0] = t | ((unsigned)(A - 1) << 16);
    unsigned fast = 1;
    for (int s = 0; s < A; s++) if ((int)norm[(size_t)ctx * A + s] >= (int)(size >> 1)) fast = 0;
    dt[0] = t | (fast << 16);
  }
  uint16_t *state_table = reinterpret_cast<uint16_t *>(ct) + 2;
  for (unsigned ub = 0; ub < size; ub += 64) {
    const unsigned u = ub + lane;
    const bool valid = u < size;
    const unsigned s = valid ? cell[u] : 0u;
    const unsigned long long grp = fq_match_any<ABITS>(s, valid);
    const unsigned r = next_rank[s] + fq_mbcnt(grp);
    __syncthreads();
    if (valid) {
      if (fq_mbcnt(grp) == 0) next_rank[s] = r + (unsigned)__popcll(grp);
      state_table[cumul[s] + r] = (uint16_t)(size + u);
      const unsigned ns = cumul[s + 1] - cumul[s];
      const unsigned x = ns + r;
      const unsigned nb = t - hb32(x);
      dt[1 + u] = FQ_DENTRY(((x << nb) - size) & 0x3FFFu, s, nb);
    }
    __syncthreads();
  }
// ... 62 lines not shown
  uint16_t *next = next1 + (size_t)blockIdx.x * stride;
  for (unsigned e = threadIdx.x; e < 4 * size; e += 256) {
    const unsigned s = e >> log, x = size + (e & (size - 1));
    const unsigned nb = (x + tt[2 * s + 1]) >> 16;
    next[e] = (uint16_t)(((unsigned)st[(int)(x >> nb) + (int)tt[2 * s]] - size) * 2u);
  }
}

__global__ void __launch_bounds__(256)
k_build_seq_next2(const uint32_t *__restrict__ logs, const uint16_t *__restrict__ next1, unsigned stride1,
                  unsigned stride2, uint16_t *__restrict__ next2) {
  const unsigned log = logs[blockIdx.x], size = 1u << log;
  const uint16_t *n1 = next1 + (size_t)blockIdx.x * stride1;
  uint16_t *n2 = next2 + (size_t)blockIdx.x * stride2;
  for (unsigned e = threadIdx.x; e < 16 * size; e += 256) {
    const unsigned xi = e & (size - 1), pc = e >> log, s1 = pc & 3u, s2 = pc >> 2;
    n2[e] = n1[(s2 << log) + ((unsigned)n1[(s1 << log) + xi] >> 1)];
  }
}

__global__ void __launch_bounds__(256)
k_build_seq_pow(const uint32_t *__restrict__ logs, const uint16_t *__restrict__ next1, unsigned stride, unsigned S,
                uint16_t *__restrict__ pow) {
  __shared__ uint16_t base[1 << 12], acc[1 << 12], tmp[1 << 12];
  const unsigned c = blockIdx.x, s = blockIdx.y;
  const unsigned log = logs[c], size = 1u << log;
  const uint16_t *n1 = next1 + (size_t)c * stride + ((size_t)s << log);
  for (unsigned i = threadIdx.x; i < size; i += blockDim.x) { base[i] = (uint16_t)(n1[i] >> 1); acc[i] = (uint16_t)i; }
  __syncthreads();
  for (unsigned e = S; e; e >>= 1) {
    if (e & 1u) {
      for (unsigned i = threadIdx.x; i < size; i += blockDim.x) tmp[i] = base[acc[i]];
      __syncthreads();
      for (unsigned i = threadIdx.x; i < size; i += blockDim.x) acc[i] = tmp[i];
      __syncthreads();
    }
    if (e > 1u) {
      for (unsigned i = threadIdx.x; i < size; i += blockDim.x) tmp[i] = base[base[i]];
      __syncthreads();
      for (unsigned i = threadIdx.x; i < size; i += blockDim.x) base[i] = tmp[i];
      __syncthreads();
    }
  }
  uint16_t *o = pow + (size_t)c * stride + ((size_t)s << log);
  for (unsigned i = threadIdx.x; i < size; i += blockDim.x) o[i] = (uint16_t)(acc[i] * 2u);
}

__global__ void __launch_bounds__(256)
k_reset_masks(const int16_t *__restrict__ norm, unsigned B, unsigned A, unsigned long long *__restrict__ mask) {
  const unsigned c = blockIdx.x * blockDim.x + threadIdx.x;
  if (c >= B) return;
  unsigned long long m = 0;
  for (unsigned s = 0; s < A; s++) {
    const int v = norm[(size_t)c * A + s];
    if (v == 1 || v == -1) m |= 1ull << s;
  }
  mask[c] = m;
}

int fq_seq_pow_ensure(hipStream_t st, DevTables &t, unsigned n_models, unsigned S) {
  if (!t.next1 || S == 0) return FQGPU_OK;
  for (unsigned i = 0; i < FQ_SEQ_POW_SETS; i++)
    if (t.seq_pow[i] && t.seq_pow_S[i] == S) return FQGPU_OK;
  unsigned slot = FQ_SEQ_POW_SETS - 1;
  for (unsigned i = 0; i < FQ_SEQ_POW_SETS; i++)
    if (!t.seq_pow[i]) { slot = i; break; }
  const unsigned stride = 4u << t.max_log;
  if (!t.seq_pow[slot]) {
    t.seq_pow[slot] = fq_dev_alloc<uint16_t>((size_t)n_models * stride + 64);
    if (!t.seq_pow[slot]) return FQGPU_E_NOMEM;
  }
  t.seq_pow_S[slot] = S;
  hipLaunchKernelGGL(k_build_seq_pow, dim3(n_models, 4), dim3(256), 0, st, t.logs, t.next1, stride, S, t.seq_pow[slot]);
  FQ_HIP(hipGetLastError());
  return FQGPU_OK;
}

int fq_build_tables(hipStream_t st, DevTables &t, int n_models, int alpha, uint32_t *err_dev) {
  const unsigned B = (unsigned)n_models;
  t.log_prefix = fq_dev_alloc<uint32_t>(B + 1);
  t.ct_off = fq_dev_alloc<uint32_t>(B);
  t.dt_off = fq_dev_alloc<uint32_t>(B);
  uint32_t *totals = fq_dev_alloc<uint32_t>(4);
  if (!t.log_prefix || !t.ct_off || !t.dt_off || !totals) return FQGPU_E_NOMEM;
  hipLaunchKernelGGL(k_log_prefix, dim3(1), dim3(1024), 0, st, t.logs, B, t.log_prefix, t.ct_off, t.dt_off,
                     (unsigned)alpha, totals);
  uint32_t h_tot[3];
  FQ_HIP(hipMemcpyAsync(h_tot, totals, sizeof(h_tot), hipMemcpyDeviceToHost, st));
  FQ_HIP(hipStreamSynchronize(st));
  (void)hipFree(totals);
  t.ct_words = h_tot[1];
  t.dt_words = h_tot[2];
  t.ct = fq_dev_alloc<uint32_t>(t.ct_words + 16);
  t.dt = fq_dev_alloc<uint32_t>(t.dt_words + 16);
  if (!t.ct || !t.dt) return FQGPU_E_NOMEM;
  FQ_HIP(hipMemsetAsync(t.ct, 0, (t.ct_words + 16) * 4, st));
  FQ_HIP(hipMemsetAsync(t.dt, 0, (t.dt_words + 16) * 4, st));
  if (alpha == FQGPU_SEQ_ALPHA)
    hipLaunchKernelGGL((k_build_tables<FQGPU_SEQ_ALPHA, 2>), dim3(B), dim3(64), 0, st, t.norm, t.logs, t.ct_off,
                       t.dt_off, t.ct, t.dt, err_dev);
  else
    hipLaunchKernelGGL((k_build_tables<FQGPU_QUAL_ALPHA, 6>), dim3(B), dim3(64), 0, st, t.norm, t.logs, t.ct_off,
                       t.dt_off, t.ct, t.dt, err_dev);
  t.reset_mask = fq_dev_alloc<unsigned long long>(B);
  if (!t.reset_mask) return FQGPU_E_NOMEM;
  hipLaunchKernelGGL(k_reset_masks, dim3((B + 255) / 256), dim3(256), 0, st, t.norm, B, (unsigned)alpha, t.reset_mask);
  if (alpha == FQGPU_SEQ_ALPHA) {
    const unsigned stride = 4u << t.max_log;
    t.next1 = fq_dev_alloc<uint16_t>((size_t)B * stride + 64);
    if (!t.next1) return FQGPU_E_NOMEM;
    hipLaunchKernelGGL(k_build_seq_next, dim3(B), dim3(256), 0, st, t.ct, t.ct_off, stride, t.next1);
    if (t.max_log <= 11) {
      t.next2 = fq_dev_alloc<uint16_t>((size_t)B * 4 * stride + 64);
      if (!t.next2) return FQGPU_E_NOMEM;
      hipLaunchKernelGGL(k_build_seq_next2, dim3(B), dim3(256), 0, st, t.logs, t.next1, stride, 4 * stride, t.next2);
    }
    for (unsigned S : {1024u, 2048u, 4096u}) {
      const int rc = fq_seq_pow_ensure(st, t, B, S);
      if (rc) return rc;
    }
  }
  FQ_HIP(hipGetLastError());
  return FQGPU_OK;
}
```

include/fqgpu.h:

```cpp
#ifndef FQGPU_H
#define FQGPU_H

#include <stddef.h>
#include <stdint.h>

#ifdef __cplusplus
extern "C" {
#endif

#define FQGPU_SEQ_MODELS 256
#define FQGPU_SEQ_ALPHA 4
#define FQGPU_QUAL_MODELS 8192
#define FQGPU_QUAL_ALPHA 64
#define FQGPU_SEQ_FT_BYTES 3076
#define FQGPU_QUAL_FT_BYTES 1081348

enum {
  FQGPU_OK = 0,
  FQGPU_E_OVERFLOW = -1,
  FQGPU_E_SHORT_READ = -2,
  FQGPU_E_CORRUPT = -3,
  FQGPU_E_ARG = -4,
  FQGPU_E_NO_DEVICE = -5,
  FQGPU_E_NOMEM = -6,
// ... 7 lines not shown

typedef struct fqgpu_ctx fqgpu_ctx;

int fqgpu_device_count(void);
const char *fqgpu_strerror(int code);
const char *fqgpu_version(void);

size_t fqgpu_bound_seq(size_t total_bases);
size_t fqgpu_bound_qual(size_t total_bases);

int fqgpu_freq_tables(int device, const uint8_t *raw, size_t raw_len, const fqgpu_rec *recs,
                      size_t n_recs, void *seq_ft_out, void *qual_ft_out,
                      uint32_t *seq_counts_out, uint32_t *qual_counts_out);
int fqgpu_tables_from_counts(int device, const uint32_t *seq_counts, const uint32_t *qual_counts,
                             void *seq_ft_out, void *qual_ft_out);

int fqgpu_ctx_create(int device, const void *seq_ft, const void *qual_ft, fqgpu_ctx **out);
void fqgpu_ctx_destroy(fqgpu_ctx *ctx);
#define FQGPU_CHAIN_SEQ_GENERIC 1u
int fqgpu_ctx_set_chain_params(fqgpu_ctx *ctx, unsigned segment, unsigned flags);
int fqgpu_ctx_set_seq_segment(fqgpu_ctx *ctx, unsigned symbols);
int fqgpu_ctx_set_seq_group(fqgpu_ctx *ctx, unsigned max_segments, unsigned min_groups);
int fqgpu_ctx_set_seq_handover(fqgpu_ctx *ctx, unsigned cap, unsigned prefix_segments);
int fqgpu_ctx_reserve(fqgpu_ctx *ctx, size_t raw_len, size_t n_recs, size_t n_bases);
int fqgpu_ctx_set_lanes(fqgpu_ctx *ctx, unsigned lanes);
int fqgpu_ctx_dump_tables(fqgpu_ctx *ctx, int stream, unsigned model, uint32_t *ctable_out,
                          size_t ctable_cap_words, uint32_t *dtable_out, size_t dtable_cap_words);

#define FQGPU_F_WRITE_BACK_N 1u
#define FQGPU_F_DECODE_INDEX 2u
int fqgpu_encode_block(fqgpu_ctx *ctx, uint8_t *raw, size_t raw_len, const fqgpu_rec *recs,
                       size_t n_recs, uint8_t *seq_out, size_t seq_cap, size_t *seq_len,
                       uint8_t *qual_out, size_t qual_cap, size_t *qual_len,
                       uint16_t *readlens_out, uint16_t *n_count_out, uint16_t *n_pos_out,
                       size_t n_pos_cap, size_t *n_pos_len, unsigned flags);

int fqgpu_encode_begin(fqgpu_ctx *ctx, const uint8_t *raw, size_t raw_len, const fqgpu_rec *recs, size_t n_recs,
                       unsigned flags, size_t *n_recs_out, size_t *n_bases_out, size_t *used_len);
int fqgpu_encode_records(fqgpu_ctx *ctx, fqgpu_rec *recs_out, size_t cap);
int fqgpu_encode_wait(fqgpu_ctx *ctx, size_t *seq_len, size_t *qual_len, size_t *n_pos_len);
int fqgpu_encode_cancel(fqgpu_ctx *ctx);
int fqgpu_encode_end(fqgpu_ctx *ctx, uint8_t *raw, uint8_t *seq_out, size_t seq_cap, size_t *seq_len,
                     uint8_t *qual_out, size_t qual_cap, size_t *qual_len, uint16_t *readlens_out,
                     uint16_t *n_count_out, uint16_t *n_pos_out, size_t n_pos_cap, size_t *n_pos_len);

#define FQGPU_HDR_MAX_FIELDS 64
typedef struct {
  uint32_t isDifferentFlag, content, contentLength;
} fqgpu_field_sizes;
int fqgpu_encode_headers_begin(fqgpu_ctx *ctx, const uint8_t *field_types, const char *separators, unsigned n_fields,
                               const uint8_t *first_header, size_t first_header_len);
int fqgpu_encode_headers_wait(fqgpu_ctx *ctx, fqgpu_field_sizes *sizes, size_t *total_bytes, size_t *bad_record);
int fqgpu_encode_headers_end(fqgpu_ctx *ctx, uint8_t *out, size_t out_cap);

int fqgpu_decode_block(fqgpu_ctx *ctx, const uint8_t *seq, size_t seq_len, const uint8_t *qual,
                       size_t qual_len, const uint16_t *n_count, size_t n_count_len,
                       const uint16_t *n_pos, size_t n_pos_len, const fqgpu_rec *recs,
                       size_t n_recs, uint8_t *raw_out, size_t raw_len);
int fqgpu_encode_index(fqgpu_ctx *ctx, int stream, uint8_t *out, size_t cap, size_t *len);
int fqgpu_decode_block_indexed(fqgpu_ctx *ctx, const uint8_t *seq, size_t seq_len, const uint8_t *qual, size_t qual_len,
                               const uint16_t *n_count, size_t n_count_len, const uint16_t *n_pos, size_t n_pos_len,
                               const fqgpu_rec *recs, size_t n_recs, uint8_t *raw_out, size_t raw_len,
                               const uint8_t *seq_index, size_t seq_index_len, const uint8_t *qual_index, size_t qual_index_len);

typedef struct fqgpu_dblock fqgpu_dblock;
int fqgpu_dblock_create(fqgpu_ctx *ctx, const uint8_t *raw, size_t raw_len, const fqgpu_rec *recs,
                        size_t n_recs, fqgpu_dblock **out);
int fqgpu_dblock_create_from_raw(fqgpu_ctx *ctx, const uint8_t *raw, size_t raw_len, fqgpu_dblock **out);
int fqgpu_dblock_records(fqgpu_ctx *ctx, const fqgpu_dblock *b, fqgpu_rec *recs_out, size_t cap,
                         size_t *n_recs, size_t *raw_len);
void fqgpu_dblock_destroy(fqgpu_dblock *b);
int fqgpu_dblock_encode(fqgpu_ctx *ctx, fqgpu_dblock *b, unsigned flags);
int fqgpu_dblock_wipe(fqgpu_ctx *ctx, fqgpu_dblock *b);
int fqgpu_dblocks_decode(fqgpu_ctx *ctx, fqgpu_dblock *const *blocks, size_t n_blocks);
int fqgpu_dblocks_decode_indexing(fqgpu_ctx *ctx, fqgpu_dblock *const *blocks, size_t n_blocks);
int fqgpu_sync(fqgpu_ctx *ctx);
int fqgpu_dblock_status(const fqgpu_dblock *b, size_t *seq_len, size_t *qual_len,
                        size_t *n_pos_len, size_t *n_bases);
int fqgpu_dblock_longest_chain(const fqgpu_dblock *b, unsigned *seq_steps, unsigned *qual_steps);
int fqgpu_dblock_seq_handover(const fqgpu_dblock *b, unsigned *handed_over, unsigned *kept);
int fqgpu_dblock_qual_segment_classes(fqgpu_ctx *ctx, const fqgpu_dblock *b, size_t counts[4]);
int fqgpu_dblock_qual_segments(fqgpu_ctx *ctx, const fqgpu_dblock *b, uint8_t *cls_out, uint32_t *anchor_out, uint32_t *ctx_out,
                               size_t cap, size_t *n_out);
int fqgpu_ctx_fill_scratch(fqgpu_ctx *ctx, unsigned char byte, size_t *n_buffers, size_t *n_bytes);
#define FQGPU_DEC_FORM_BOTH 0x001u
#define FQGPU_DEC_FORM_QUAL_RESIDENT 0x002u
#define FQGPU_DEC_FORM_QUAL_COMPACT 0x004u
#define FQGPU_DEC_FORM_SEQ 0x008u
#define FQGPU_DEC_FORM_CHUNKS_QUAL_RESIDENT 0x010u
#define FQGPU_DEC_FORM_CHUNKS_QUAL_COMPACT 0x020u
#define FQGPU_DEC_FORM_CHUNKS_SEQ 0x040u
#define FQGPU_DEC_FORM_SNAP 0x100u
int fqgpu_ctx_decode_forms(const fqgpu_ctx *ctx, unsigned *forms, unsigned *qual_chains, unsigned *qual_strides, unsigned *n_cus);
int fqgpu_dblock_fetch(fqgpu_ctx *ctx, const fqgpu_dblock *b, uint8_t *seq_out, uint8_t *qual_out,
                       uint16_t *readlens_out, uint16_t *n_count_out, uint16_t *n_pos_out,
                       uint8_t *raw_out);
int fqgpu_ctx_set_index_stride(fqgpu_ctx *ctx, unsigned symbols);
int fqgpu_dblock_index_bytes(const fqgpu_dblock *b, int stream, size_t *bytes);
int fqgpu_dblock_fetch_index(fqgpu_ctx *ctx, const fqgpu_dblock *b, int stream, void *out, size_t cap);
int fqgpu_dblock_load_index(fqgpu_ctx *ctx, fqgpu_dblock *b, int stream, const void *data, size_t len);
int fqgpu_dblock_load_streams(fqgpu_ctx *ctx, fqgpu_dblock *b, const uint8_t *seq, size_t seq_len,
                              const uint8_t *qual, size_t qual_len, const uint16_t *n_count,
                              const uint16_t *n_pos, size_t n_pos_len);

typedef struct {
  float total_ms;
  float kernel_ms[32];
  int kernel_calls[32];
  const char *kernel_name[32];
  int n_kernels;
} fqgpu_timing;
int fqgpu_ctx_enable_timing(fqgpu_ctx *ctx, int on);
int fqgpu_ctx_last_timing(fqgpu_ctx *ctx, fqgpu_timing *out);
int fqgpu_ctx_timing_only(fqgpu_ctx *ctx, const char *name);

long fqgpu_parse_fastq(const uint8_t *raw, size_t len, fqgpu_rec *recs, size_t cap);
size_t fqgpu_synth_fastq(uint8_t *dst, size_t cap, int mode, uint64_t seed, uint64_t first_read_id,
                         uint64_t *n_reads_out);


typedef struct {
  const uint8_t *field_types;
  const char *separators;
  unsigned n_fields;
  const uint8_t *first_header;
  size_t first_header_len;
  const fqgpu_field_sizes *sizes;
  const uint8_t *const *streams;
} fqgpu_header_streams;
int fqgpu_decode_chunk(fqgpu_ctx *ctx, const fqgpu_header_streams *hdr, const uint16_t *readlens, size_t n_recs,
                       const uint8_t *seq, size_t seq_len, const uint8_t *qual, size_t qual_len,
                       const uint16_t *n_count, size_t n_count_len, const uint16_t *n_pos, size_t n_pos_len,
                       const uint8_t *seq_index, size_t seq_index_len, const uint8_t *qual_index, size_t qual_index_len,
                       uint8_t *raw_out, size_t raw_len, fqgpu_rec *recs_out, size_t *laid_out_len, size_t *bad_record);

int fqgpu_decode_chunk_indexing(fqgpu_ctx *ctx, const fqgpu_header_streams *hdr, const uint16_t *readlens, size_t n_recs,
                                const uint8_t *seq, size_t seq_len, const uint8_t *qual, size_t qual_len,
                                const uint16_t *n_count, size_t n_count_len, const uint16_t *n_pos, size_t n_pos_len,
                                uint8_t *raw_out, size_t raw_len, fqgpu_rec *recs_out, size_t *laid_out_len, size_t *bad_record);
int fqgpu_decode_index(fqgpu_ctx *ctx, int stream, uint8_t *out, size_t cap, size_t *len);

int fqgpu_decode_chunk_range(fqgpu_ctx *ctx, const fqgpu_header_streams *hdr, const uint16_t *readlens, size_t n_recs,
                             const uint8_t *seq, size_t seq_len, const uint8_t *qual, size_t qual_len,
                             const uint16_t *n_count, size_t n_count_len, const uint16_t *n_pos, size_t n_pos_len,
                             const uint8_t *seq_index, size_t seq_index_len, const uint8_t *qual_index, size_t qual_index_len,
                             size_t raw_len, size_t first, size_t end, uint8_t *out, size_t out_cap, size_t *out_len,
                             fqgpu_rec *recs_out, size_t *bad_record);

int fqgpu_decode_chunk_fasta(fqgpu_ctx *ctx, const fqgpu_header_streams *hdr, const uint16_t *readlens, size_t n_recs,
                             const uint8_t *seq, size_t seq_len,
                             const uint16_t *n_count, size_t n_count_len, const uint16_t *n_pos, size_t n_pos_len,
                             const uint8_t *seq_index, size_t seq_index_len,
                             size_t raw_len, size_t first, size_t end,
                             uint8_t *out, size_t out_cap, size_t *out_len, fqgpu_rec *recs_out, size_t *bad_record);

int fqgpu_chunk_crc32(fqgpu_ctx *ctx, uint32_t *crc, size_t *len);
int fqgpu_dblock_crc32(fqgpu_ctx *ctx, const fqgpu_dblock *b, uint32_t *crc, size_t *len);
uint32_t fqgpu_crc32_combine(uint32_t crc_a, uint32_t crc_b, uint64_t len_b);
int fqgpu_ctx_set_check_only(fqgpu_ctx *ctx, int on);

size_t fqgpu_stats_words(unsigned positions);
int fqgpu_chunk_stats(fqgpu_ctx *ctx, unsigned positions, uint64_t *out, size_t cap_words);
int fqgpu_dblock_stats(fqgpu_ctx *ctx, const fqgpu_dblock *b, unsigned positions, uint64_t *out, size_t cap_words);
int fqgpu_stats_merge(uint64_t *dst, size_t dst_words, const uint64_t *src, size_t src_words);

#define FQGPU_FILTER_NONE 0xFFFFFFFFu
// ... 139 lines not shown
```

Before: 131,400 MB/s.

## Pool short-segment contexts into shared walk wavefronts with pooled LDS tables

Groups consecutive quality contexts into pools whose coding tables together fit a fixed LDS budget, then packs contexts with fewer than 64 segments into shared 64-lane wavefronts instead of giving each context its own mostly idle wavefront. The layout kernel now computes per-pool lane and own-item bases with a wave-level scan, and the walk kernels binary-search the pool and context per lane and stage several tables at once. This is meant to cut the number of underfilled walk blocks for the 8192 quality contexts. In exchange it adds per-lane context lookups, divergent table access and larger LDS allocations, plus a diagnostic API to inspect the plan.

```diff
diff --git a/fqcomp28_amd/binding.py b/fqcomp28_amd/binding.py
--- a/fqcomp28_amd/binding.py
+++ b/fqcomp28_amd/binding.py
@@ -122,6 +122,8 @@
     "fqgpu_dblock_qual_segment_classes": (C.c_int, [C.c_void_p, C.c_void_p, C.POINTER(C.c_size_t)]),
     "fqgpu_dblock_qual_segments": (C.c_int, [C.c_void_p, C.c_void_p, C.c_void_p, C.c_void_p, C.c_void_p, C.c_size_t,
                                              C.POINTER(C.c_size_t)]),
+    "fqgpu_dblock_qual_walk_plan": (C.c_int, [C.c_void_p, C.c_void_p, C.c_void_p, C.c_void_p, C.c_void_p, C.c_size_t,
+                                              C.POINTER(C.c_size_t), C.POINTER(C.c_uint)]),
     "fqgpu_ctx_set_index_stride": (C.c_int, [C.c_void_p, C.c_uint]),
     "fqgpu_dblock_index_bytes": (C.c_int, [C.c_void_p, C.c_int, C.POINTER(C.c_size_t)]),
     "fqgpu_dblock_fetch_index": (C.c_int, [C.c_void_p, C.c_void_p, C.c_int, C.c_void_p, C.c_size_t]),
@@ -750,6 +752,18 @@
                    "dblock_qual_segments")
         return dict(cls=cls, anchor=anchor, ctx=ctx)
 
+    def qual_walk_plan(self):
+        n, items = C.c_size_t(0), C.c_uint(0)
+        rc = lib().fqgpu_dblock_qual_walk_plan(self.ctx.h, self.h, None, None, None, 0, C.byref(n), C.byref(items))
+        if rc != -1:
+            _check(rc, "dblock_qual_walk_plan")
+        first, base = np.zeros(n.value + 1, dtype=np.uint32), np.zeros(n.value + 1, dtype=np.uint32)
+        lanes = np.zeros(QUAL_MODELS, dtype=np.uint32)
+        if n.value:
+            _check(lib().fqgpu_dblock_qual_walk_plan(self.ctx.h, self.h, _p(first), _p(base), _p(lanes), n.value, C.byref(n),
+                                                     C.byref(items)), "dblock_qual_walk_plan")
+        return dict(pool_first=first, walk_base=base, lane_base=lanes, n_items=int(items.value))
+
     def fetch(self, raw=False):
         rc, st = self.status()
         _check(rc, "dblock_status")
diff --git a/fqcomp28_amd/csrc/api.hip b/fqcomp28_amd/csrc/api.hip
--- a/fqcomp28_amd/csrc/api.hip
+++ b/fqcomp28_amd/csrc/api.hip
@@ -1,4 +1,5 @@
 #include "fqgpu_internal.h"
+#include "enc_plan.h"
 
 #include <algorithm>
 #include <cstdio>
@@ -427,7 +428,7 @@
 }
 
 static void free_tables(DevTables &t) {
-  void *ps[] = {t.norm, t.logs, t.log_prefix, t.ct, t.ct_off, t.dt, t.dt_off, t.next1, t.next2, t.reset_mask,
+  void *ps[] = {t.norm, t.logs, t.log_prefix, t.ct, t.ct_off, t.dt, t.dt_off, t.next1, t.next2, t.reset_mask, t.pool_first, t.pool_of,
                 t.seq_pow[0], t.seq_pow[1], t.seq_pow[2], t.seq_pow[3]};
   for (void *p : ps) if (p) (void)hipFree(p);
   t = DevTables();
@@ -887,6 +888,28 @@
       for (uint32_t s = seg_base[c]; s < seg_base[c + 1] && s < n; s++) ctx_out[s] = c;
   free(seg_base);
   return he == hipSuccess ? FQGPU_OK : fq_hip_error(he, __FILE__, __LINE__);
+}
+
+extern "C" int fqgpu_dblock_qual_walk_plan(fqgpu_ctx *ctx, const fqgpu_dblock *b, uint32_t *pool_first_out, uint32_t *walk_base_out,
+                                           uint32_t *lane_base_out, size_t cap, size_t *n_pools_out, uint32_t *n_items_out) {
+  if (!ctx || !b || !n_pools_out || (cap && (!pool_first_out || !walk_base_out || !lane_base_out))) return FQGPU_E_ARG;
+  *n_pools_out = 0;
+  if (n_items_out) *n_items_out = 0;
+  const EncLane *lane = nullptr;
+  uint32_t n_segs = 0;
+  if (int rc = diag_lane(ctx, b, &lane, &n_segs)) return rc;
+  const DevTables &t = ctx->tab[1];
+  if (!lane->diag_walk_end || !lane->diag_walk_ctx || !t.pool_first || !t.n_pools) return FQGPU_E_ARG;
+  const size_t np = t.n_pools;
+  *n_pools_out = np;
+  if (n_items_out) FQ_HIP(hipMemcpy(n_items_out, lane->diag_walk_end + np - 1, 4, hipMemcpyDeviceToHost));
+  if (np > cap) return FQGPU_E_OVERFLOW;
+  FQ_HIP(hipMemcpy(pool_first_out, t.pool_first, (np + 1) * 4, hipMemcpyDeviceToHost));
+  walk_base_out[0] = 0;
+  FQ_HIP(hipMemcpy(walk_base_out + 1, lane->diag_walk_end, np * 4, hipMemcpyDeviceToHost));
+  FQ_HIP(hipMemcpy(lane_base_out, lane->diag_walk_ctx, (size_t)FQGPU_QUAL_MODELS * 4, hipMemcpyDeviceToHost));
+  for (size_t c = 0; c < FQGPU_QUAL_MODELS; c++) lane_base_out[c] &= (1u << WALK_LANE_BITS) - 1u;
+  return FQGPU_OK;
 }
 
 extern "C" int fqgpu_dblock_fetch(fqgpu_ctx *ctx, const fqgpu_dblock *b, uint8_t *seq_out, uint8_t *qual_out,
diff --git a/fqcomp28_amd/csrc/enc_chains_generic.h b/fqcomp28_amd/csrc/enc_chains_generic.h
--- a/fqcomp28_amd/csrc/enc_chains_generic.h
+++ b/fqcomp28_amd/csrc/enc_chains_generic.h
@@ -184,21 +184,21 @@
   return x;
 }
 
-template <class M, int PASS>
-__device__ __forceinline__ void seg_walk_role(uint32_t *lds, unsigned item, const uint8_t *__restrict__ sorted_sym,
-                                              uint16_t *__restrict__ out16, const uint32_t *__restrict__ arrays,
-                                              const uint32_t *__restrict__ ct, const uint32_t *__restrict__ ct_off,
-                                              uint16_t *__restrict__ final_state, unsigned S, const SegArrays &sa, StreamResult *res) {
-  constexpr unsigned B = M::B;
-  const uint32_t *ctx_count = arrays, *ctx_start = arrays + B, *seg_base = ctx_start + B + 1,
-                 *item_base = seg_base + B + 1;
-  if (item >= item_base[B]) return;
-  const unsigned c = seg_ctx_of<M>(item_base, item);
-  const unsigned n = ctx_count[c];
-  const unsigned nseg = seg_base[c + 1] - seg_base[c];
-  const unsigned k = (item - item_base[c]) * 64 + fq_lane();
-  const LdsCTable t = stage_ctable<M>(lds, ct + ct_off[c]);
-  if (k >= nseg) return;
+template <bool OWN>
+__device__ __forceinline__ unsigned walk_ctx_of(const uint32_t *__restrict__ plan, unsigned lo, unsigned hi, unsigned v) {
+  while (lo < hi) {
+    const unsigned mid = lo + ((hi - lo + 1) >> 1);
+    if ((OWN ? walk_own_base(plan[mid]) : walk_lane_base(plan[mid])) <= v) lo = mid; else hi = mid - 1;
+  }
+  return lo;
+}
+
+template <class M, int PASS, bool POOLED>
+__device__ __forceinline__ void seg_walk_lane(const LdsCTable &t, unsigned c, unsigned k, unsigned nseg, unsigned n,
+                                              const uint8_t *__restrict__ sorted_sym, uint16_t *__restrict__ out16,
+                                              const uint32_t *__restrict__ ctx_start, const uint32_t *__restrict__ seg_base,
+                                              uint16_t *__restrict__ final_state, unsigned S, const SegArrays &sa) {
+  if (!POOLED) c = (unsigned)__builtin_amdgcn_readfirstlane((int)c);
   const unsigned seg = seg_base[c] + k;
   const uint8_t *sym = sorted_sym + ctx_start[c];
   uint16_t *out = out16 + ctx_start[c];
@@ -217,7 +217,60 @@
   x = seg_walk_range<M>(t, sym, out, i0, i1, x);
   if (PASS == 1 && k + 1 < nseg) sa.entry_state[seg + 1] = (uint16_t)x;
   if (k == nseg - 1 && (PASS == 1 || !reset)) final_state[c] = (uint16_t)x;
-  if (PASS == 2 && fq_lane() == 0) atomicMax(&res->refixed, min(S, n));
+}
+
+template <class M, int PASS>
+__device__ __forceinline__ void seg_walk_role(uint32_t *lds, unsigned item, const uint8_t *__restrict__ sorted_sym,
+                                              uint16_t *__restrict__ out16, const uint32_t *__restrict__ arrays,
+                                              const uint32_t *__restrict__ ct, const uint32_t *__restrict__ ct_off,
+                                              uint16_t *__restrict__ final_state, unsigned S, const SegArrays &sa, StreamResult *res,
+                                              const WalkPlan &wp) {
+  constexpr unsigned B = M::B;
+  const uint32_t *ctx_count = arrays, *ctx_start = arrays + B, *seg_base = ctx_start + B + 1;
+  if (item >= wp.walk_end[wp.n_pools - 1]) return;
+  unsigned p = 0;
+  for (unsigned hi = wp.n_pools - 1; p < hi;) {
+    const unsigned mid = (p + hi) >> 1;
+    if (wp.walk_end[mid] > item) hi = mid; else p = mid + 1;
+  }
+  const unsigned first = wp.pool_first[p], last = wp.pool_first[p + 1] - 1;
+  const unsigned nseg_last = seg_base[last + 1] - seg_base[last];
+  const unsigned n_short = walk_lane_base(wp.ctx[last]) + (nseg_last < 64 ? nseg_last : 0u), n_pooled = (n_short + 63u) >> 6;
+  const unsigned j = item - (p ? wp.walk_end[p - 1] : 0u), lane = fq_lane();
+  if (j >= n_pooled) {
+    const unsigned c = walk_ctx_of<true>(wp.ctx, first, last, j - n_pooled);
+    const unsigned n = ctx_count[c];
+    const unsigned nseg = seg_base[c + 1] - seg_base[c];
+    const unsigned k = (j - n_pooled - walk_own_base(wp.ctx[c])) * 64 + lane;
+    const LdsCTable t = stage_ctable<M>(lds, ct + ct_off[c]);
+    if (k >= nseg) return;
+    seg_walk_lane<M, PASS, false>(t, c, k, nseg, n, sorted_sym, out16, ctx_start, seg_base, final_state, S, sa);
+    if (PASS == 2 && lane == 0) atomicMax(&res->refixed, min(S, n));
+    return;
+  }
+  const unsigned v = j * 64 + lane;
+  const bool active = v < n_short;
+  const unsigned c = walk_ctx_of<false>(wp.ctx, first, last, active ? v : n_short - 1);
+  const unsigned c_lo = (unsigned)__builtin_amdgcn_readfirstlane((int)c), c_hi = (unsigned)__builtin_amdgcn_readlane((int)c, 63);
+  const unsigned w0 = ct_off[c_lo];
+  const unsigned words = ct_off[c_hi] + 1u + (1u << ((ct[ct_off[c_hi]] & 0xFFFFu) - 1)) + 2u * M::A - w0;
+  for (unsigned i = lane; i < words; i += 64) lds[i] = ct[w0 + i];
+  __syncthreads();
+  const unsigned n = ctx_count[c];
+  if (PASS == 2) {
+    unsigned m = active ? min(S, n) : 0u;
+#pragma unroll
+    for (int d = 32; d > 0; d >>= 1) m = max(m, (unsigned)__shfl_xor((int)m, d));
+    if (lane == 0) atomicMax(&res->refixed, m);
+  }
+  if (!active) return;
+  const uint32_t *tbl = lds + (ct_off[c] - w0);
+  LdsCTable t;
+  t.log = tbl[0] & 0xFFFFu;
+  t.state_table = reinterpret_cast<const uint16_t *>(tbl) + 2;
+  t.tt = tbl + 1 + (1u << (t.log - 1));
+  seg_walk_lane<M, PASS, true>(t, c, v - walk_lane_base(wp.ctx[c]), seg_base[c + 1] - seg_base[c], n, sorted_sym, out16, ctx_start, seg_base,
+                               final_state, S, sa);
 }
 
 template <class M, int PASS>
@@ -225,9 +278,9 @@
 k_seg_walk(const uint8_t *__restrict__ sorted_sym, uint16_t *__restrict__ out16,
            const uint32_t *__restrict__ arrays, const uint32_t *__restrict__ ct,
            const uint32_t *__restrict__ ct_off, uint16_t *__restrict__ final_state, unsigned S,
-           SegArrays sa, StreamResult *res) {
+           SegArrays sa, StreamResult *res, WalkPlan wp) {
   extern __shared__ uint32_t lds[];
-  seg_walk_role<M, PASS>(lds, blockIdx.x, sorted_sym, out16, arrays, ct, ct_off, final_state, S, sa, res);
+  seg_walk_role<M, PASS>(lds, blockIdx.x, sorted_sym, out16, arrays, ct, ct_off, final_state, S, sa, res, wp);
 }
 
 template <class M>
@@ -455,11 +508,11 @@
 k_seg_stage1(const uint8_t *__restrict__ sorted_sym, uint16_t *__restrict__ out16, const uint32_t *__restrict__ arrays,
              const uint32_t *__restrict__ ct, const uint32_t *__restrict__ ct_off, uint16_t *__restrict__ final_state,
              unsigned S, unsigned n_walk, unsigned n_cand, unsigned pbase, unsigned fstride, SegArrays sa,
-             uint16_t *__restrict__ fbuf, StreamResult *res) {
+             uint16_t *__restrict__ fbuf, StreamResult *res, WalkPlan wp) {
   extern __shared__ uint32_t lds[];
   __shared__ SetsWaveLds L;
   if (blockIdx.x < n_walk)
-    seg_walk_role<M, 1>(lds, blockIdx.x, sorted_sym, out16, arrays, ct, ct_off, final_state, S, sa, res);
+    seg_walk_role<M, 1>(lds, blockIdx.x, sorted_sym, out16, arrays, ct, ct_off, final_state, S, sa, res, wp);
   else if (blockIdx.x < n_walk + n_cand)
     seg_cand_role<M, false>(lds, blockIdx.x - n_walk, n_cand, sorted_sym, arrays, ct, ct_off, S, fstride, sa, fbuf);
   else
diff --git a/fqcomp28_amd/csrc/enc_plan.h b/fqcomp28_amd/csrc/enc_plan.h
--- a/fqcomp28_amd/csrc/enc_plan.h
+++ b/fqcomp28_amd/csrc/enc_plan.h
@@ -24,6 +24,13 @@
 constexpr unsigned SEQ_ITEM_GROUPS = 64;
 constexpr unsigned SEG_MAX_CAND = 64;
 constexpr unsigned SEG_SLOT = 16;
+#ifndef FQ_SEG_POOL_TABLES
+#define FQ_SEG_POOL_TABLES 2
+#endif
+constexpr unsigned SEG_POOL_WORDS = FQ_SEG_POOL_TABLES * (1u + (1u << 10) + 2u * FQGPU_QUAL_ALPHA);
+constexpr unsigned WALK_LANE_BITS = 14;
+static_assert(SEG_POOL_WORDS / 25u * 63u < (1u << WALK_LANE_BITS), "lane_base fits its bits");
+static_assert((1u << 16) + SEG_POOL_WORDS / 25u < (1u << (32 - WALK_LANE_BITS)), "own_base fits its bits");
 
 struct EncSpan {
   size_t off = 0, bytes = 0;
@@ -118,9 +125,12 @@
   unsigned wpg = 0, Q = 0, gmin = 0, rounds = 0;
   unsigned max_fitems = 0, max_eitems = 0, max_citems = 0;
   unsigned lds_ct = 0;
+  unsigned lds_walk = 0;
+  unsigned max_walk_items = 0;
 
   EncSpan sa_anchor, sa_usym, sa_entry, sa_cand, sa_cls;
   EncSpan ia_has_g, ia_entry, ia_g;
+  EncSpan ss_final, ss_walk_ctx, ss_walk_end;
   EncSpan sp_fitem, sp_seg, sp_work, sp_entry;
   EncSpan cb_func, cb_item_entry;
   EncSpan cand0, cand;
@@ -152,10 +162,16 @@
     max_eitems = seq_max_segs / 64 + B + 1;
     max_citems = seq_max_segs / SEQ_ITEM_GROUPS + B + 1;
     lds_ct = (1u + (1u << (max_log - 1)) + 2u * in.A) * 4u;
+    lds_walk = std::max(lds_ct, SEG_POOL_WORDS * 4u);
+    max_walk_items = max_items;
 
     bytes.slot_of = tile_path ? lpos16_bytes : n_pad * 4;
     bytes.out16 = padded * 2;
-    bytes.seg_state = (size_t)B * 2 + (size_t)B * 8;
+    EncCarve ss;
+    ss_final = ss.take((size_t)B * 2);
+    ss_walk_ctx = ss.take((size_t)B * 4, 4);
+    ss_walk_end = ss.take((size_t)B * 4);
+    bytes.seg_state = ss.total;
     bytes.tile_bits = (size_t)n_ptiles * 4;
     bytes.tile_bit_base = (size_t)(n_ptiles + 1) * 8;
 
diff --git a/fqcomp28_amd/csrc/enc_records_hist.h b/fqcomp28_amd/csrc/enc_records_hist.h
--- a/fqcomp28_amd/csrc/enc_records_hist.h
+++ b/fqcomp28_amd/csrc/enc_records_hist.h
@@ -554,44 +554,114 @@
   ctx_count[c] = acc;
 }
 
+struct WalkPlan {
+  const uint32_t *pool_first, *pool_of;
+  unsigned n_pools;
+  uint32_t *walk_end;
+  uint32_t *ctx;
+};
+__device__ __forceinline__ unsigned walk_lane_base(unsigned w) { return w & ((1u << WALK_LANE_BITS) - 1u); }
+__device__ __forceinline__ unsigned walk_own_base(unsigned w) { return w >> WALK_LANE_BITS; }
+
+template <int N>
+__device__ __forceinline__ void layout_scan(unsigned (&v)[N], unsigned (*wsum)[16]) {
+  const unsigned lane = threadIdx.x & 63u, wave = threadIdx.x >> 6;
+  unsigned inc[N];
+#pragma unroll
+  for (int j = 0; j < N; j++) inc[j] = v[j];
+#pragma unroll
+  for (int d = 1; d < 64; d <<= 1) {
+#pragma unroll
+    for (int j = 0; j < N; j++) {
+      const unsigned o = (unsigned)__shfl_up((int)inc[j], d);
+      if (lane >= (unsigned)d) inc[j] += o;
+    }
+  }
+  if (lane == 63)
+    for (int j = 0; j < N; j++) wsum[j][wave] = inc[j];
+  __syncthreads();
+#pragma unroll
+  for (int j = 0; j < N; j++) {
+    unsigned off = 0;
+    for (unsigned w = 0; w < wave; w++) off += wsum[j][w];
+    v[j] = off + inc[j] - v[j];
+  }
+  __syncthreads();
+}
+
+constexpr unsigned LAYOUT_PER = 8;
 __global__ void __launch_bounds__(1024)
-k_ctx_layout(unsigned B, unsigned S, uint32_t *__restrict__ arrays, uint32_t *__restrict__ fill_none) {
+k_ctx_layout(unsigned B, unsigned S, uint32_t *__restrict__ arrays, uint32_t *__restrict__ fill_none, WalkPlan wp) {
   if (fill_none)
     for (unsigned c = threadIdx.x; c < B; c += blockDim.x) fill_none[c] = 0xFFFFFFFFu;
-  __shared__ unsigned part[3][1024];
+  __shared__ unsigned wsum[5][16];
+  __shared__ unsigned s_total[2];
   uint32_t *ctx_count = arrays, *ctx_start = arrays + B, *seg_base = ctx_start + B + 1,
            *item_base = seg_base + B + 1;
+  const bool walk = wp.ctx != nullptr;
   const unsigned per = (B + blockDim.x - 1) / blockDim.x;
   const unsigned c0 = threadIdx.x * per, c1 = min(c0 + per, B);
-  unsigned a0 = 0, a1 = 0, a2 = 0;
+  unsigned a[5] = {0, 0, 0, 0, 0};
   for (unsigned c = c0; c < c1; c++) {
     const unsigned n = ctx_count[c];
-    const unsigned nseg = (n + S - 1) / S;
-    a0 += (n + CTX_PAD - 1) & ~(CTX_PAD - 1);
-    a1 += nseg;
-    a2 += (nseg + 63) >> 6;
-  }
-  part[0][threadIdx.x] = a0; part[1][threadIdx.x] = a1; part[2][threadIdx.x] = a2;
-  __syncthreads();
-  if (threadIdx.x < 3) {
-    unsigned run = 0;
-    for (unsigned i = 0; i < blockDim.x; i++) {
-      const unsigned v = part[threadIdx.x][i];
-      part[threadIdx.x][i] = run;
-      run += v;
-    }
-  }
-  __syncthreads();
-  a0 = part[0][threadIdx.x]; a1 = part[1][threadIdx.x]; a2 = part[2][threadIdx.x];
+    const unsigned nseg = (n + S - 1) / S, items = (nseg + 63) >> 6;
+    a[0] += (n + CTX_PAD - 1) & ~(CTX_PAD - 1);
+    a[1] += nseg;
+    a[2] += items;
+    a[3] += nseg < 64 ? nseg : 0u;
+    a[4] += nseg < 64 ? 0u : items;
+  }
+  layout_scan<5>(a, wsum);
+  const unsigned short0 = a[3], own0 = a[4];
   for (unsigned c = c0; c < c1; c++) {
     const unsigned n = ctx_count[c];
-    const unsigned nseg = (n + S - 1) / S;
-    ctx_start[c] = a0; seg_base[c] = a1; item_base[c] = a2;
-    a0 += (n + CTX_PAD - 1) & ~(CTX_PAD - 1);
-    a1 += nseg;
-    a2 += (nseg + 63) >> 6;
-  }
-  if (c1 == B && c0 < B) { ctx_start[B] = a0; seg_base[B] = a1; item_base[B] = a2; }
+    const unsigned nseg = (n + S - 1) / S, items = (nseg + 63) >> 6;
+    ctx_start[c] = a[0]; seg_base[c] = a[1]; item_base[c] = a[2];
+    if (walk && wp.pool_first[wp.pool_of[c]] == c) { wp.walk_end[wp.pool_of[c]] = a[3]; wp.ctx[c] = a[4]; }
+    a[0] += (n + CTX_PAD - 1) & ~(CTX_PAD - 1);
+    a[1] += nseg;
+    a[2] += items;
+    a[3] += nseg < 64 ? nseg : 0u;
+    a[4] += nseg < 64 ? 0u : items;
+  }
+  if (c1 == B && c0 < B) {
+    ctx_start[B] = a[0]; seg_base[B] = a[1]; item_base[B] = a[2];
+    s_total[0] = a[3]; s_total[1] = a[4];
+  }
+  if (!walk) return;
+  __syncthreads();
+  unsigned run_short = short0, run_own = own0;
+  for (unsigned c = c0; c < c1; c++) {
+    const unsigned pool = wp.pool_of[c], f = wp.pool_first[pool];
+    if (f != c) wp.ctx[c] = (run_short - wp.walk_end[pool]) | ((run_own - wp.ctx[f]) << WALK_LANE_BITS);
+    const unsigned nseg = (ctx_count[c] + S - 1) / S;
+    run_short += nseg < 64 ? nseg : 0u;
+    run_own += nseg < 64 ? 0u : (nseg + 63) >> 6;
+  }
+  const unsigned p0 = threadIdx.x * per, p1 = min(p0 + per, wp.n_pools);
+  unsigned items_of[LAYOUT_PER], w[1] = {0};
+#pragma unroll
+  for (unsigned i = 0; i < LAYOUT_PER; i++) {
+    const unsigned p = p0 + i;
+    items_of[i] = 0;
+    if (p < p1) {
+      const unsigned f = wp.pool_first[p], l = wp.pool_first[p + 1];
+      const unsigned n_short = (l < B ? wp.walk_end[p + 1] : s_total[0]) - wp.walk_end[p];
+      const unsigned n_own = (l < B ? wp.ctx[l] : s_total[1]) - wp.ctx[f];
+      items_of[i] = ((n_short + 63u) >> 6) + n_own;
+    }
+    w[0] += items_of[i];
+  }
+  layout_scan<1>(w, wsum);
+#pragma unroll
+  for (unsigned i = 0; i < LAYOUT_PER; i++) {
+    const unsigned p = p0 + i;
+    if (p < p1) {
+      w[0] += items_of[i];
+      wp.walk_end[p] = w[0];
+      wp.ctx[wp.pool_first[p]] = 0;
+    }
+  }
 }
 
 template <class HT>
diff --git a/fqcomp28_amd/csrc/encode.hip b/fqcomp28_amd/csrc/encode.hip
--- a/fqcomp28_amd/csrc/encode.hip
+++ b/fqcomp28_amd/csrc/encode.hip
@@ -149,6 +149,7 @@
   const uint32_t *tile_first;
   SegArrays sa;
   ItemArrays ia;
+  WalkPlan wp;
   uint32_t *plan, *plan_work, *plan_seg_base;
   uint16_t *entry, *fbuf, *cbuf, *item_entry;
   SeqHandover hand;
@@ -201,6 +202,8 @@
     v.ia.has_g = at<uint32_t>(sc.seg_arrays, p.ia_has_g);
     v.ia.item_entry = at<uint16_t>(sc.seg_arrays, p.ia_entry);
     v.ia.g = at<uint16_t>(sc.seg_arrays, p.ia_g);
+    v.wp.ctx = at<uint32_t>(sc.seg_state, p.ss_walk_ctx);
+    v.wp.walk_end = at<uint32_t>(sc.seg_state, p.ss_walk_end);
   }
   return v;
 }
@@ -227,7 +230,7 @@
   });
 }
 
-static void launch_layout(EncScratch &sc, const EncShape &sh, bool tile_path, unsigned S, uint32_t *usym, hipStream_t st) {
+static void launch_layout(EncScratch &sc, const EncShape &sh, bool tile_path, unsigned S, uint32_t *usym, const WalkPlan &wp, hipStream_t st) {
   const unsigned B = sh.B;
   const dim3 grid((B + 255) / 256, sh.n_groups);
   uint32_t *arrays = at<uint32_t>(sc.ctx_arrays, sh.ctx_count), *group_sum = sc.group_sum.as<uint32_t>();
@@ -235,7 +238,7 @@
     using H = FQ_HIST_TYPE(h);
     hipLaunchKernelGGL(k_group_sum<H>, grid, dim3(256), 0, st, sc.tile_hist.as<H>(), sh.n_tiles, B, group_sum);
     hipLaunchKernelGGL(k_group_prefix, dim3((B + 255) / 256), dim3(256), 0, st, group_sum, sh.n_groups, B, arrays);
-    hipLaunchKernelGGL(k_ctx_layout, dim3(1), dim3(1024), 0, st, B, S, arrays, usym);
+    hipLaunchKernelGGL(k_ctx_layout, dim3(1), dim3(1024), 0, st, B, S, arrays, usym, wp);
     hipLaunchKernelGGL(k_tile_base<H>, grid, dim3(256), 0, st, sc.tile_hist.as<H>(), group_sum, at<uint32_t>(sc.ctx_arrays, sh.ctx_start),
                        sh.n_tiles, B, sc.tile_base.as<uint32_t>());
   });
@@ -322,8 +325,8 @@
     hipLaunchKernelGGL(k_seg_scan<M>, dim3((p.gen_max_segs + 3) / 4), dim3(256), 0, st, sym, v.arrays, tab.reset_mask, tab.norm, tab.logs, p.S, v.sa);
   if (EncStage s{ctx, st, FQ_SPAN("stage1"), mask, 8u, "stage1"}; !s.off)
     with_log_width(tab.max_log, [&](auto w) {
-      hipLaunchKernelGGL((k_seg_stage1<M, decltype(w)::value>), dim3(p.max_items + p.cand_grid + p.gen_pbase + B), dim3(64), p.lds_ct, st, sym, out16,
-                         v.arrays, tab.ct, tab.ct_off, v.final_state, p.S, p.max_items, p.cand_grid, p.gen_pbase, p.fstride, v.sa, v.fbuf, v.res);
+      hipLaunchKernelGGL((k_seg_stage1<M, decltype(w)::value>), dim3(p.max_walk_items + p.cand_grid + p.gen_pbase + B), dim3(64), p.lds_walk, st, sym, out16,
+                         v.arrays, tab.ct, tab.ct_off, v.final_state, p.S, p.max_walk_items, p.cand_grid, p.gen_pbase, p.fstride, v.sa, v.fbuf, v.res, v.wp);
     });
   if (EncStage s{ctx, st, FQ_SPAN("heads"), mask, 8u, "heads"}; !s.off)
     hipLaunchKernelGGL(k_seg_heads<M>, dim3(p.cand_grid), dim3(64), p.lds_ct, st, sym, v.arrays, tab.ct, tab.ct_off, p.S, p.fstride, v.sa, v.fbuf);
@@ -335,7 +338,7 @@
     hipLaunchKernelGGL(k_seg_resolve3<M>, dim3((p.max_items + 255) / 256), dim3(256), 0, st, v.arrays, tab.logs, v.fbuf, p.gen_pbase, p.fstride, v.sa, v.ia);
   }
   if (EncStage s{ctx, st, FQ_SPAN("walk2"), mask, 8u, "walk2"}; !s.off)
-    hipLaunchKernelGGL((k_seg_walk<M, 2>), dim3(p.max_items), dim3(64), p.lds_ct, st, sym, out16, v.arrays, tab.ct, tab.ct_off, v.final_state, p.S, v.sa, v.res);
+    hipLaunchKernelGGL((k_seg_walk<M, 2>), dim3(p.max_walk_items), dim3(64), p.lds_walk, st, sym, out16, v.arrays, tab.ct, tab.ct_off, v.final_state, p.S, v.sa, v.res, v.wp);
 }
 
 template <class M>
@@ -394,15 +397,18 @@
   if ((mask & 512u) && M::STREAM == 0) mask = 0;
   const bool fused = fused_k1(ctx);
   if (int rc = reserve(sc, p)) return rc;
-  const EncViews v = make_views<M>(lane, p, lp, b, fused);
+  EncViews v = make_views<M>(lane, p, lp, b, fused);
+  v.wp.pool_first = tab.pool_first; v.wp.pool_of = tab.pool_of; v.wp.n_pools = tab.n_pools;
   if (M::STREAM == 1) {
     lane.diag_cls = v.sa.cls;
     lane.diag_anchor = v.sa.anchor;
     lane.diag_n_segs = v.seg_base + M::B;
+    lane.diag_walk_end = v.wp.walk_end;
+    lane.diag_walk_ctx = v.wp.ctx;
   }
 
   if (EncStage s{ctx, st, FQ_SPAN("tile_hist"), mask, 1u}; !s.off && !fused) launch_hist<M>(sc, p, v, st, b);
-  if (EncStage s{ctx, st, FQ_SPAN("layout"), mask, 2u, M::STREAM ? "k2q" : "k2s"}; !s.off) launch_layout(sc, p, p.tile_path, p.S, v.sa.usym, st);
+  if (EncStage s{ctx, st, FQ_SPAN("layout"), mask, 2u, M::STREAM ? "k2q" : "k2s"}; !s.off) launch_layout(sc, p, p.tile_path, p.S, v.sa.usym, v.wp, st);
   if (EncStage s{ctx, st, FQ_SPAN("scatter"), mask, 4u, M::STREAM ? "k3q" : "k3s"}; !s.off) launch_partition<M>(ctx, sc, p, v, st, fused);
   if (p.serial_seq) launch_seq_chains(ctx, sc, p, v, st, mask);
   else launch_generic_chains<M>(ctx, sc, p, v, st, mask);
@@ -552,7 +558,7 @@
                        readlens.as<uint16_t>(), n_cnt32, lens32, (BlockResult *)nullptr);
     if ((rc = fq_scan_u32_to_u32(st, lens32, R, rec_start, lane.scan_tmp))) break;
     launch_hist2(lane, lp, st, raw_dev, recs_dev, R, n_sym, res);
-    launch_layout(sq, shq, true, S, nullptr, st);
+    launch_layout(sq, shq, true, S, nullptr, WalkPlan{}, st);
     launch_tile_partition<QualModel, true>(sq, shq, st, sq.keys.as<uint16_t>(), nullptr, sq.tile_sync.as<uint32_t>(), nullptr, nullptr, rec_start,
                                            at<uint8_t>(lane.first_sym, lp.first_sym_of[1]), lane.tile_first.as<uint32_t>());
     hipLaunchKernelGGL(k_hist_sorted_qual, dim3((max_segs + 3) / 4), dim3(256), 0, st, sq.sorted_sym.as<uint8_t>(), sq.ctx_arrays.as<uint32_t>(), S, counts_dev);
diff --git a/fqcomp28_amd/csrc/fqgpu_internal.h b/fqcomp28_amd/csrc/fqgpu_internal.h
--- a/fqcomp28_amd/csrc/fqgpu_internal.h
+++ b/fqcomp28_amd/csrc/fqgpu_internal.h
@@ -39,6 +39,9 @@
   uint16_t *next2 = nullptr;
   uint16_t *seq_pow[4] = {nullptr, nullptr, nullptr, nullptr};
   unsigned seq_pow_S[4] = {0, 0, 0, 0};
+  uint32_t *pool_first = nullptr;
+  uint32_t *pool_of = nullptr;
+  unsigned n_pools = 0;
   uint32_t max_log = 0;
   size_t ct_words = 0, dt_words = 0;
 };
@@ -186,8 +189,12 @@
   const uint8_t *diag_cls = nullptr;
   const uint32_t *diag_anchor = nullptr;
   const uint32_t *diag_n_segs = nullptr;
+  const uint32_t *diag_walk_end = nullptr, *diag_walk_ctx = nullptr;
   unsigned long long diag_stamp = 0;
-  void forget_diag() { diag_cls = nullptr; diag_anchor = nullptr; diag_n_segs = nullptr; diag_stamp = 0; }
+  void forget_diag() {
+    diag_cls = nullptr; diag_anchor = nullptr; diag_n_segs = nullptr; diag_walk_end = nullptr; diag_walk_ctx = nullptr;
+    diag_stamp = 0;
+  }
 };
 FQ_SCRATCH_BUFS(EncLane, FQ_B(EncLane, rec_start), FQ_B(EncLane, n_cnt32), FQ_B(EncLane, n_off), FQ_B(EncLane, first_sym),
                 FQ_B(EncLane, tile_first), FQ_B(EncLane, rscan), FQ_B(EncLane, scan_tmp))
diff --git a/fqcomp28_amd/csrc/tables.hip b/fqcomp28_amd/csrc/tables.hip
--- a/fqcomp28_amd/csrc/tables.hip
+++ b/fqcomp28_amd/csrc/tables.hip
@@ -1,4 +1,5 @@
 #include "fqgpu_internal.h"
+#include "enc_plan.h"
 
 namespace {
 
@@ -249,6 +250,24 @@
   if (c1 == B && c0 < B) prefix[B] = a;
 }
 
+__global__ void __launch_bounds__(64)
+k_pool_cut(const uint32_t *__restrict__ logs, const uint32_t *__restrict__ ct_off, unsigned B, unsigned A, unsigned budget,
+           uint32_t *__restrict__ pool_first, uint32_t *__restrict__ pool_of, uint32_t *__restrict__ n_pools) {
+  if (blockIdx.x || threadIdx.x) return;
+  unsigned np = 0, first = 0;
+  pool_first[0] = 0;
+  for (unsigned c = 0; c < B; c++) {
+    const unsigned end = ct_off[c] + 1u + (1u << (logs[c] - 1)) + 2u * A;
+    if (c > first && end - ct_off[first] > budget) {
+      first = c;
+      pool_first[++np] = c;
+    }
+    pool_of[c] = np;
+  }
+  pool_first[np + 1] = B;
+  *n_pools = np + 1;
+}
+
 template <int A, int ABITS>
 __global__ void __launch_bounds__(64)
 k_build_tables(const int16_t *__restrict__ norm, const uint32_t *__restrict__ logs,
@@ -477,15 +496,20 @@
   t.ct_off = fq_dev_alloc<uint32_t>(B);
   t.dt_off = fq_dev_alloc<uint32_t>(B);
   uint32_t *totals = fq_dev_alloc<uint32_t>(4);
-  if (!t.log_prefix || !t.ct_off || !t.dt_off || !totals) return FQGPU_E_NOMEM;
+  t.pool_first = fq_dev_alloc<uint32_t>(B + 1);
+  t.pool_of = fq_dev_alloc<uint32_t>(B);
+  if (!t.log_prefix || !t.ct_off || !t.dt_off || !totals || !t.pool_first || !t.pool_of) return FQGPU_E_NOMEM;
   hipLaunchKernelGGL(k_log_prefix, dim3(1), dim3(1024), 0, st, t.logs, B, t.log_prefix, t.ct_off, t.dt_off,
                      (unsigned)alpha, totals);
-  uint32_t h_tot[3];
+  hipLaunchKernelGGL(k_pool_cut, dim3(1), dim3(64), 0, st, t.logs, t.ct_off, B, (unsigned)alpha, SEG_POOL_WORDS, t.pool_first, t.pool_of,
+                     totals + 3);
+  uint32_t h_tot[4];
   FQ_HIP(hipMemcpyAsync(h_tot, totals, sizeof(h_tot), hipMemcpyDeviceToHost, st));
   FQ_HIP(hipStreamSynchronize(st));
   (void)hipFree(totals);
   t.ct_words = h_tot[1];
   t.dt_words = h_tot[2];
+  t.n_pools = h_tot[3];
   t.ct = fq_dev_alloc<uint32_t>(t.ct_words + 16);
   t.dt = fq_dev_alloc<uint32_t>(t.dt_words + 16);
   if (!t.ct || !t.dt) return FQGPU_E_NOMEM;
diff --git a/include/fqgpu.h b/include/fqgpu.h
--- a/include/fqgpu.h
+++ b/include/fqgpu.h
@@ -113,6 +113,8 @@
 int fqgpu_dblock_qual_segment_classes(fqgpu_ctx *ctx, const fqgpu_dblock *b, size_t counts[4]);
 int fqgpu_dblock_qual_segments(fqgpu_ctx *ctx, const fqgpu_dblock *b, uint8_t *cls_out, uint32_t *anchor_out, uint32_t *ctx_out,
                                size_t cap, size_t *n_out);
+int fqgpu_dblock_qual_walk_plan(fqgpu_ctx *ctx, const fqgpu_dblock *b, uint32_t *pool_first_out, uint32_t *walk_base_out,
+                                uint32_t *lane_base_out, size_t cap, size_t *n_pools_out, uint32_t *n_items_out);
 int fqgpu_ctx_fill_scratch(fqgpu_ctx *ctx, unsigned char byte, size_t *n_buffers, size_t *n_bytes);
 #define FQGPU_DEC_FORM_BOTH 0x001u
 #define FQGPU_DEC_FORM_QUAL_RESIDENT 0x002u
```

Result: no change. 131,500 MB/s, median of 6 (+0.1%).
